# CederGroupHub/chgnet

Hardware: AMD Instinct MI355X
Metric: structures/s (energy+force+stress) on batched ~50-atom crystals (higher is better)
Workload: dtype f32; 1 GPU; 1024 x LiMnO2 5x1x1 (40 atoms, sigma=0.01 frac perturbation) per GPU, task efs; structures_per_gpu=1024, atoms=40960, directed_bonds=3535504, angles=4125764, bond_graph_nodes=213755, weights=random-init 0.3.0 architecture (tests/golden/weights_seed0.npz), parallelism=structures sharded over 1 GPU(s), RCCL all-gather of energies only, process_group_ranks=1, energies_in_all_gather=1024, comm=none (single rank)

## Files before the change

### chgnet_amd/csrc/engine_internal.h

```cpp
#pragma once

#include "chgnet_hip.h"

#include <hip/hip_runtime.h>

#include <algorithm>
#include <cmath>
#include <cstdint>
#include <cstdio>
#include <cstdlib>
#include <cstring>
#include <functional>
#include <map>
#include <mutex>
#include <string>
#include <unordered_map>
#include <vector>

#include "mfma_tile.h"
#include "mfma_split.h"
#include "kernels_conv.h"
#include "kernels_angle_w.h"
#include "kernels_angle_blk.h"
#include "kernels_embed.h"

using namespace chg;

constexpr int MAX_CONV = 8;
constexpr float F16_OPERAND_LIMIT = 65504.0f;
constexpr int FWD_WAVES = 8;

struct ACW { const float *w_cn, *w_bond, *b1, *q_bias, *q_shift; GatedW g; const float *w2c_t, *w2g_t, *w_out, *b_out, *w_out_t, *w_cn_t, *w_bond_t; };
struct BCW { const float *w_bij, *w_ang, *w_ctr, *b1; GatedW g; const float *w2c_t, *w2g_t, *w_out, *b_out, *w_out_t, *w_bij_t, *w_ang_t, *w_ctr_t; };
struct AUW { const float *w_bij, *w_ang, *w_ctr, *b1; GatedW g; const float *w_bij_t, *w_ang_t, *w_ctr_t; };

struct Weights {
  const float *atomref, *emb, *freq_ag, *freq_bg, *freq_ang, *w_bond_emb, *w_wag, *w_wbg, *w_ang_emb;
  ACW ac[MAX_CONV];
  BCW bc[MAX_CONV];
  AUW au[MAX_CONV];
  const float *site_w, *site_b, *ro_ln_g, *ro_ln_b, *mlp_w0, *mlp_b0, *mlp_w1, *mlp_b1, *mlp_w2, *mlp_b2, *mlp_w3, *mlp_b3;
  const float *mlp_w0_t, *mlp_w1_t, *mlp_w2_t;
};

struct ErrText {
  static std::unordered_map<const ErrText*, std::string>& texts() {
    thread_local std::unordered_map<const ErrText*, std::string> t;
    return t;
  }
  std::string& slot() const { return texts()[this]; }
  ErrText& operator=(const std::string& v) { slot() = v; return *this; }
  ErrText& operator=(const char* v) { slot() = v; return *this; }
  operator std::string() const { return slot(); }
  const char* c_str() const { return slot().c_str(); }
  ~ErrText() { texts().erase(this); }
};
inline std::string operator+(const char* a, const ErrText& b) { return std::string(a) + std::string(b); }
inline std::string operator+(const std::string& a, const ErrText& b) { return a + std::string(b); }
inline std::string operator+(const ErrText& a, const char* b) { return std::string(a) + b; }
inline std::string operator+(const ErrText& a, const std::string& b) { return std::string(a) + b; }

struct ProfEntry { std::string label; int64_t launches = 0; double ms = 0.0; };
struct PendingEvent { int entry; hipEvent_t start, stop; };

struct chg_engine {
  int device = 0;
  hipStream_t stream = nullptr;
  chg_model_desc desc{};
  float* d_weights = nullptr;
  Weights w{};
  float* d_images = nullptr;
  const float* p_elem = nullptr;
  const float* img_ac_fwd[2][MAX_CONV] = {};
  const float* img_ac_bwd_rm[MAX_CONV] = {};
  const float* img_angle[2][2 * MAX_CONV] = {};
  ErrText err;
  hipEvent_t t0 = nullptr, t1 = nullptr;
  bool profiling = false;
  std::vector<ProfEntry> prof;
  std::map<std::string, int> prof_index;
  std::vector<PendingEvent> pending;
  std::vector<hipEvent_t> event_pool;
  hipStream_t copy_stream = nullptr;
  std::mutex pool_mu;
  std::vector<std::pair<char*, size_t>> arena_pool;
  std::vector<std::pair<char*, size_t>> work_pool;
  std::vector<int> work_kind;
  bool use_graphs = true;
  bool force_wide = false;
  char* scratch = nullptr;
  size_t scratch_bytes = 0, scratch_wanted = 0;
  char* h_stage = nullptr;
  size_t h_stage_bytes = 0;
  char* h_out = nullptr;
  size_t h_out_bytes = 0;
  int num_cus = 256;
  bool spec_builds = true;
  int last_N = 0, last_Ed = 0, last_A = 0, last_Eb = 0;
  double last_r_atom = 0.0, last_r_bond = 0.0;
  long n_spec_builds = 0, n_spec_overflows = 0, n_cell_builds = 0, n_cell_fallbacks = 0;
  int graph_search = 0;
  int cell_min_atoms = 2048;
  size_t memory_limit = 0;
};

struct Train2;

struct chg_batch {
  int B = 0, N = 0, Ed = 0, Eu = 0, A = 0, Eb = 0, L = 0;
  char* arena = nullptr;
  size_t arena_bytes = 0;
  int *z, *atom_owner, *atom_off, *e_center, *e_nbr, *e_d2u, *e_owner, *e_rev, *p_center, *p_nbr, *u_u2d, *u_bnode, *bn_und, *a_ctr, *a_b1c, *a_b2c, *a_d1, *a_d2;
  float *frac, *lattice, *e_image;
  float* cart;
  f32x4 *ev, *eu;
  float *hb0, *wag, *wbgc;
  float* atom[MAX_CONV + 1];
  float* hbc[MAX_CONV + 1];
  float* ang[MAX_CONV];
  float* Pl[MAX_CONV];
  float* Ql[MAX_CONV];
  float* Rl[2 * MAX_CONV];
  float* Sl[2 * MAX_CONV];
  float* agg_l[MAX_CONV];
  float* aggB_l[MAX_CONV];
  float* GP_l[MAX_CONV];
  float* GR_l[2 * MAX_CONV];
  float* GS_l[2 * MAX_CONV];
  float* zsave_l[2 * MAX_CONV] = {};
  float *energy, *site_energy, *site_raw, *magmom, *crystal_fea, *force, *virial, *volume;
  float *Ga, *GA, *Gb, *Gwag, *Gwbgc, *Gang, *GQ, *Gagg, *Grk, *Gu;
  WinIndex win{};
  int *win_tmp = nullptr, *win_scan = nullptr;
  int win_grid = 64;
  bool win_built = false;
  bool canonical = false;
  bool win_index_ready = false;
  int win_team = 0;
  int blk_cap = 0;
  bool blk_ready = false;
  int *blk_a = nullptr, *blk_b1c = nullptr, *blk_b2c = nullptr, *blk_ctr = nullptr, *blk_desc = nullptr, *blk_tiles = nullptr;
  bool win_pending = false;
  bool zsave_now = false;
  int32_t route[6] = {}, graph_route[6] = {};
  size_t addr_span = 0;
  int p_table_done = -1;
  float *zero1, *zero1_end, *zero2, *zero2_end;
  float* zero2_keep_end = nullptr;
  uint32_t last_task = 0;
  bool seed1_adjoints = false;
  hipGraphExec_t graph_exec = nullptr;
  uint32_t graph_task = 0;
  int eager_calls = 0;
  std::map<std::string, std::pair<const float*, size_t>> named;
  std::map<std::string, std::pair<const int*, size_t>> named_i32;
  char* train_arena = nullptr;
  size_t train_bytes = 0;
  std::vector<int> h_atom_off;
  std::vector<double> h_volume;
  char* t2_arena = nullptr;
  size_t t2_bytes = 0;
  struct Train2* t2 = nullptr;
  float* t_mcot = nullptr;
  float h_g_b3 = 0.f;
  bool q_tables = false;
  bool wide_range = false;
  bool t_has_mcot = false;
  float *t_grad = nullptr, *t_cot = nullptr, *t_tmp = nullptr , *t_dumpG = nullptr, *t_dumpH = nullptr, *t_dumpZ = nullptr, *t_Xb = nullptr, *t_Xa = nullptr,
        *t_ro = nullptr;
};

#define HIP_TRY(eng, expr)                                                                          \
  do {                                                                                              \
    hipError_t _e = (expr);                                                                         \
    if (_e != hipSuccess) {                                                                         \
      (eng)->err = std::string(#expr) + ": " + hipGetErrorString(_e);                               \
      return CHG_EHIP;                                                                              \
    }                                                                                               \
  } while (0)

#define TRY(x)                   \
  do {                           \
    int _s = (x);                \
    if (_s != CHG_OK) return _s; \
  } while (0)

namespace chgh {

int prof_entry(chg_engine* eng, const char* label);
hipEvent_t get_event(chg_engine* eng);
int collect_profile(chg_engine* eng);

struct LaunchScope {
  chg_engine* eng;
  PendingEvent pe{};
  bool on;
  LaunchScope(chg_engine* e, const char* label) : eng(e), on(e->profiling) {
    if (on) {
      pe.entry = prof_entry(eng, label);
      pe.start = get_event(eng);
      pe.stop = get_event(eng);
      hipEventRecord(pe.start, eng->stream);
    }
  }
  ~LaunchScope() {
    if (on) {
      hipEventRecord(pe.stop, eng->stream);
      eng->pending.push_back(pe);
    }
  }
};


struct Carver {
  char* base;
  size_t pos = 0;
  template <class T>
  T* take(size_t n) {
    pos = (pos + 255) & ~size_t(255);
    T* p = base ? reinterpret_cast<T*>(base + pos) : nullptr;
    pos += std::max<size_t>(n, 1) * sizeof(T);
    return p;
  }
};

inline dim3 g1(int64_t n, int b = 256) { return dim3((unsigned)std::max<int64_t>(1, (n + b - 1) / b)); }
inline int wave_grid(chg_engine* eng, int64_t items) {
  return (int)std::max<int64_t>(1, std::min<int64_t>((items + 3) / 4, 16 * (int64_t)eng->num_cus));
}

template <class T>
int h2d(chg_engine* eng, T* dst, const T* src, size_t n, hipStream_t stream = nullptr) {
  if (n == 0) return CHG_OK;
  if (!src) { eng->err = "chg_batch_upload: null host array"; return CHG_EINVAL; }
  HIP_TRY(eng, hipMemcpyAsync(dst, src, n * sizeof(T), hipMemcpyHostToDevice, stream ? stream : eng->stream));
  return CHG_OK;
}
template <class T>
int d2h(chg_engine* eng, T* dst, const T* src, size_t n) {
  if (n == 0 || !dst) return CHG_OK;
  HIP_TRY(eng, hipMemcpyAsync(dst, src, n * sizeof(T), hipMemcpyDeviceToHost, eng->stream));
  return CHG_OK;
}

template <class K>
int set_lds(chg_engine* eng, K kernel, size_t bytes) {
  HIP_TRY(eng, hipFuncSetAttribute(reinterpret_cast<const void*>(kernel), hipFuncAttributeMaxDynamicSharedMemorySize, (int)bytes));
  return CHG_OK;
}

size_t layout_weights(const float* base, int L, Weights& w);
int grid_for(int rows, int max_blocks, int block_rows = BLOCK_ROWS);
int tile_grid(chg_engine* eng, int rows, int block_rows = BLOCK_ROWS);
int rows_gemm(chg_engine* eng, const char* label, int K, int NOUT, const float* X, int ldx, const int* in_idx, const float* Wt,
              const float* bias, const float* resid, int ldr, float* Y, int ldy, const int* out_idx, int rows, int accumulate);
int rows_gemm_out2(chg_engine* eng, const char* label, const float* X, const int* in_idx, const float* Wt, const float* Wt2,
                   const float* bias, float* Y, int ldy, int rows);
int rows_gemm_in2(chg_engine* eng, const char* label, const float* X, int ldx, const float* Wt, const float* Wt2, float* Y,
                  const int* out_idx, int rows, int accumulate);
int zero(chg_engine* eng, void* p, size_t bytes);
int build_images(chg_engine* eng);
int predict_set_lds(chg_engine* eng);
int atomconv_q_table(chg_engine* eng, chg_batch* b, int l);
AtomConvArgs atomconv_args(chg_engine* eng, chg_batch* b, int l);
AngleArgs angle_args(chg_batch* b, int slot, const float* ang, const float* w_ang, const GatedW& g, float* out);
int angle_table_grads(chg_engine* eng, chg_batch* b, int slot, const float* w_bij_t, const float* w_ctr_t);
BondEmbedTArgs bond_embed_args(chg_engine* eng, chg_batch* b);
AngleEmbedTArgs angle_embed_args(chg_engine* eng, chg_batch* b);
int run_predict(chg_engine* eng, chg_batch* b, uint32_t task);
void carve(chg_batch* b, char* base, size_t& total);
int prepare_windows(chg_engine* eng, chg_batch* b);
inline long team_min_angles() {
  static const long v = [] { const char* e = std::getenv("CHGNET_TEAM_MIN_ANGLES"); return e ? std::atol(e) : 131072L; }();
  return v;
}
inline long blk_max_angles() {
  static const long v = [] { const char* e = std::getenv("CHGNET_BLK_MAX_ANGLES"); return e ? std::atol(e) : (1L << 22); }();
  return v;
}
inline size_t blk_tile_bound(size_t A, size_t Eb, size_t N) { return (A + 14 * Eb + 9 * N) / 16 + 1; }
inline int upload_blk_cap(size_t N, size_t A, size_t Eb) {
  return (A > 0 && N + 1 <= 8192 && (long)A <= blk_max_angles()) ? (int)blk_tile_bound(A, Eb, N) : 0;
}
bool decide_windows(chg_engine* eng, chg_batch* b);
int ensure_windows(chg_engine* eng, chg_batch* b);
void register_names(chg_batch* b);

int train_set_lds(chg_engine* eng);
void free_train2(chg_batch* b);
void release_workspace(chg_engine* eng, char* p, size_t bytes, int kind);
int backward_impl(chg_engine* eng, chg_batch* b, const float* energy_cotangent, const float* magmom_cotangent, const float* force_cotangent,
                  const float* stress_cotangent, chg_comm* comm, float* grad_blob);

size_t scan_scratch_ints(int n);
int exclusive_scan_with(chg_engine* eng, int* scratch, const int* in, int* out, int n);
int acquire_arena(chg_engine* eng, chg_batch* b, size_t total);
int build_batch_on_device(chg_engine* eng, const chg_structs_host* h, double r_atom, double r_bond, double numerical_tol, chg_batch** out);

}

namespace chgh_wide {
int run_predict(chg_engine* eng, chg_batch* b, uint32_t task);
int predict_set_lds(chg_engine* eng);
int backward_compute(chg_engine* eng, chg_batch* b, const float* energy_cotangent, const float* magmom_cotangent, const float* force_cotangent,
                     const float* stress_cotangent);
int train_set_lds(chg_engine* eng);
int hvp_compute(chg_engine* eng, chg_batch* b, const float* direction, const float* strain, float* hvp, float* hvp_strain);
}

using namespace chgh;
```

### chgnet_amd/csrc/engine_predict.hip

```cpp
#include "engine_internal.h"

#include "kernels_geom.h"
#include "kernels_angle_fa.h"
#include "kernels_chain.h"

namespace chgh {


struct Cursor {
  const float* base;
  size_t pos = 0;
  const float* take(size_t n) {
    pos += (4 - pos % 4) % 4;
    const float* p = base + pos;
    pos += n;
    return p;
  }
};

void take_gated_tail(Cursor& c, GatedW& g, const float*& w2c_t, const float*& w2g_t) {
  g.w2c = c.take(D * D); g.b2c = c.take(D); g.w2g = c.take(D * D); g.b2g = c.take(D);
  w2c_t = c.take(D * D); w2g_t = c.take(D * D);
}
void take_ln(Cursor& c, GatedW& g) {
// ... 109 lines not shown
}

int rows_gemm(chg_engine* eng, const char* label, int K, int NOUT, const float* X, int ldx, const int* in_idx, const float* Wt,
              const float* bias, const float* resid, int ldr, float* Y, int ldy, const int* out_idx, int rows, int accumulate) {
  RowsGemm p{X, ldx, in_idx, Wt, bias, resid, ldr, Y, ldy, out_idx, rows, accumulate, nullptr, 0, 0, 0, 0};
  if (rows <= SMALL_GEMM_ROWS && K == 64 && (NOUT == 64 || NOUT == 128)) return launch_rows_gemm_cols<64, 1>(eng, label, p, NOUT, NOUT);
  if (rows <= SMALL_GEMM_ROWS && K == 128 && NOUT == 64) return launch_rows_gemm_cols<128, 1>(eng, label, p, NOUT, NOUT);
  if (K == 64 && NOUT == 64) return launch_rows_gemm<64, 64>(eng, label, p);
  if (K == 64 && NOUT == 128) return launch_rows_gemm<64, 128>(eng, label, p);
  if (K == 128 && NOUT == 64) return launch_rows_gemm<128, 64>(eng, label, p);
  eng->err = "rows_gemm: unsupported shape";
  return CHG_EINVAL;
}

int rows_gemm_out2(chg_engine* eng, const char* label, const float* X, const int* in_idx, const float* Wt, const float* Wt2,
                   const float* bias, float* Y, int ldy, int rows) {
  RowsGemm p{X, D, in_idx, Wt, bias, nullptr, 0, Y, ldy, nullptr, rows, 0, Wt2, 0, 2 * D, 0, 0};
  if (rows <= SMALL_GEMM_ROWS) return launch_rows_gemm_cols<64, 1>(eng, label, p, 4 * D, 2 * D);
  return launch_rows_gemm<64, 128, 2>(eng, label, p);
}
int rows_gemm_in2(chg_engine* eng, const char* label, const float* X, int ldx, const float* Wt, const float* Wt2, float* Y,
                  const int* out_idx, int rows, int accumulate) {
  RowsGemm p{X, ldx, nullptr, Wt, nullptr, nullptr, 0, Y, D, out_idx, rows, accumulate, Wt2, 2 * D, 0, 0, 0};
  if (rows <= SMALL_GEMM_ROWS) return launch_rows_gemm_cols<128, 2>(eng, label, p, D, D);
  return launch_rows_gemm<128, 64, 2>(eng, label, p);
}

struct MultiGemm {
  RowsGemmN g{};
  int max_rows = 0;
  void add(RowsGemm p, int n_out, int n_out_first) {
    p.col_blocks = n_out / SMALL_GEMM_COLS; p.blocks1 = n_out_first / SMALL_GEMM_COLS;
    g.p[g.n++] = p;
    max_rows = std::max(max_rows, p.rows);
  }
};
template <int K>
int launch_rows_gemm_multi(chg_engine* eng, const char* label, const MultiGemm& m) {
  int blocks = 0;
  for (int i = 0; i < m.g.n; ++i) blocks += m.g.p[i].col_blocks;
  LaunchScope ls(eng, label);
  hipLaunchKernelGGL((k_rows_gemm_multi<K, SMALL_GEMM_COLS>), dim3(grid_for(m.max_rows, 4 * eng->num_cus), blocks), dim3(BLOCK),
                     (rows_gemm_lds<K, SMALL_GEMM_COLS, (K == 128 ? 2 : 1)>()), eng->stream, m.g);
  HIP_TRY(eng, hipGetLastError());
  return CHG_OK;
}
static bool small_rows(int rows) { return rows > 0 && rows <= SMALL_GEMM_ROWS; }

int zero(chg_engine* eng, void* p, size_t bytes) {
  if (bytes == 0) return CHG_OK;
  LaunchScope ls(eng, "memset");
  HIP_TRY(eng, hipMemsetAsync(p, 0, bytes, eng->stream));
  return CHG_OK;
}





static bool addr32_mode(const chg_batch* b) {
  constexpr size_t HARD = (size_t)1 << 32;
  static const int forced = [] { const char* e = std::getenv("CHGNET_ADDR_MODE"); return e ? std::atoi(e) : 0; }();
  static const size_t limit = [] { const char* e = std::getenv("CHGNET_ADDR32_MAX_BYTES"); return e ? (size_t)std::strtoull(e, nullptr, 10) : HARD; }();
  if (b->addr_span == 0 || b->addr_span >= HARD || forced == 64) return false;
  return forced == 32 || b->addr_span < limit;
}

int build_images(chg_engine* eng) {
  const int L = eng->desc.n_conv;
  constexpr size_t AF = ac_fwd_image_floats(), AB = ac_bwd_rm_image_floats();
  constexpr size_t BF = AngleLds<true, false>::tiles, BB = AngleLds<true, true>::tiles, UF = AngleLds<false, false>::tiles,
                   UB = AngleLds<false, true>::tiles;
  static_assert(AF % 4 == 0 && AB % 4 == 0 && BF % 4 == 0 && BB % 4 == 0 && UF % 4 == 0 && UB % 4 == 0, "images are copied in 16-byte units");
  constexpr size_t PE = (size_t)94 * 4 * D;
  const size_t total = (size_t)L * (2 * AF + AB) + (size_t)(L - 1) * (BF + BB + UF + UB) + PE;
  if (!eng->d_images) {
    HIP_TRY(eng, hipMalloc(&eng->d_images, total * sizeof(float)));
    HIP_TRY(eng, hipMemsetAsync(eng->d_images, 0, total * sizeof(float), eng->stream));
  }
  float* at = eng->d_images;
  auto take = [&](size_t n) { float* p = at; at += n; return p; };
  for (int l = 0; l < L; ++l) {
    AtomConvArgs a{};
    a.gw = eng->w.ac[l].g; a.w_bond = eng->w.ac[l].w_bond;
    for (int qb = 0; qb < 2; ++qb) {
      a.q_bias = qb ? eng->w.ac[l].q_bias : nullptr;
      float* img = take(AF);
      eng->img_ac_fwd[qb][l] = img;
      hipLaunchKernelGGL(k_atomconv_image<>, dim3(1), dim3(BLOCK), 0, eng->stream, a, img);
    }
    float* img = take(AB);
    eng->img_ac_bwd_rm[l] = img;
    hipLaunchKernelGGL(k_atomconv_image_rm, dim3(1), dim3(BLOCK), 0, eng->stream, a, img);
  }
  for (int l = 0; l + 1 < L; ++l) {
    const BCW& bc = eng->w.bc[l];
    const AUW& au = eng->w.au[l];
    float* img;
    eng->img_angle[0][l] = img = take(BF);
    hipLaunchKernelGGL((k_angle_image<true, false>), dim3(1), dim3(BLOCK), 0, eng->stream, bc.w_ang, bc.g, img);
    eng->img_angle[1][l] = img = take(BB);
    hipLaunchKernelGGL((k_angle_image<true, true>), dim3(1), dim3(BLOCK), 0, eng->stream, bc.w_ang, bc.g, img);
    eng->img_angle[0][L + l] = img = take(UF);
    hipLaunchKernelGGL((k_angle_image<false, false>), dim3(1), dim3(BLOCK), 0, eng->stream, au.w_ang, au.g, img);
    eng->img_angle[1][L + l] = img = take(UB);
    hipLaunchKernelGGL((k_angle_image<false, true>), dim3(1), dim3(BLOCK), 0, eng->stream, au.w_ang, au.g, img);
  }
  {
    float* tab = take(PE);
    eng->p_elem = tab;
    const ACW& w0 = eng->w.ac[0];
    TRY(rows_gemm_out2(eng, "gemm_Pelem", eng->w.emb, nullptr, w0.w_cn, w0.w_cn + 2 * D * D, w0.b1, tab, 4 * D, 94));
  }
  HIP_TRY(eng, hipGetLastError());
  return CHG_OK;
}

static bool tiny_batch(const chg_batch* b) {
  static const bool on = [] { const char* e = std::getenv("CHGNET_TINY_FUSE"); return !e || std::atoi(e) != 0; }();
  return on && b->N <= SMALL_GEMM_ROWS && b->Ed <= (1 << 18) && b->A <= (1 << 19);
}

static RowsGemm atomconv_p_problem(chg_engine* eng, chg_batch* b, int l) {
  const ACW& w = eng->w.ac[l];
  return RowsGemm{b->atom[l], D, nullptr, w.w_cn, w.b1, nullptr, 0, b->Pl[l], 4 * D, nullptr, b->N, 0, w.w_cn + 2 * D * D, 0, 2 * D, 0, 0};
}

int atomconv_tables(chg_engine* eng, chg_batch* b, int l) {
  const ACW& w = eng->w.ac[l];
  if (b->p_table_done == l) return CHG_OK;
  return rows_gemm_out2(eng, "gemm_P", b->atom[l], nullptr, w.w_cn, w.w_cn + 2 * D * D, w.b1, b->Pl[l], 4 * D, b->N);
}

int atomconv_q_table(chg_engine* eng, chg_batch* b, int l) {
  const ACW& w = eng->w.ac[l];
  float* Q = b->Ql[l];
  if (b->Eu == 0) return CHG_OK;
  TRY(rows_gemm(eng, "gemm_Q", 64, 128, b->hb0, D, nullptr, w.w_bond, b->A > 0 ? w.q_bias : nullptr, nullptr, 0, Q, 2 * D, nullptr, b->Eu, 0));
  if (b->Eb > 0 && b->hbc[l] != b->hbc[0])
    TRY(rows_gemm(eng, "gemm_Qnode", 64, 128, b->hbc[l], D, nullptr, w.w_bond, nullptr, nullptr, 0, Q, 2 * D, b->bn_und, b->Eb, 0));
  return CHG_OK;
}

AtomConvArgs atomconv_args(chg_engine* eng, chg_batch* b, int l) {
  AtomConvArgs a{};
  a.P = b->Pl[l]; a.Q = b->Ql[l]; a.wag = b->wag;
  a.e_center = b->e_center; a.e_nbr = b->e_nbr; a.e_d2u = b->e_d2u; a.n_edges = b->Ed;
  a.gw = eng->w.ac[l].g;
  a.agg = b->agg_l[l]; a.GA = b->GA; a.GP = b->GP_l[l]; a.GQ = b->GQ; a.Gwag = b->Gwag;
  a.first_wag = l == b->L - 1;
  a.hb0 = b->hb0;
  a.hbc = (b->Eb > 0 && b->hbc[l] != b->hbc[0]) ? b->hbc[l] : nullptr;
  a.u_bnode = b->u_bnode;
  a.w_bond = eng->w.ac[l].w_bond;
  a.q_bias = b->A > 0 ? eng->w.ac[l].q_bias : nullptr;
  return a;
}

int atomconv_fwd_kernel(chg_engine* eng, chg_batch* b, int l, bool keep_q) {
  {
    LaunchScope ls(eng, "atomconv_fwd");
    const size_t lds = atomconv_lds<FWD_WAVES, false, true>();
    AtomConvArgs a = atomconv_args(eng, b, l);
    a.e_center = b->p_center;
    a.image = eng->img_ac_fwd[a.q_bias ? 1 : 0][l];
    a.e_nbr = b->p_nbr;
    a.Qout = keep_q ? b->Ql[l] : nullptr;
    if (addr32_mode(b)) hipLaunchKernelGGL((k_atomconv_fwd<FWD_WAVES, true>), dim3(tile_grid(eng, b->Ed, TILE_ROWS * FWD_WAVES)), dim3(64 * FWD_WAVES), lds, eng->stream, a);
    else hipLaunchKernelGGL((k_atomconv_fwd<FWD_WAVES>), dim3(tile_grid(eng, b->Ed, TILE_ROWS * FWD_WAVES)), dim3(64 * FWD_WAVES), lds, eng->stream, a);
    HIP_TRY(eng, hipGetLastError());
  }
  return CHG_OK;
}

int atomconv_fwd(chg_engine* eng, chg_batch* b, int l, bool keep_q) {
  const ACW& w = eng->w.ac[l];
  if (b->Ed > 0) {
    TRY(atomconv_tables(eng, b, l));
    TRY(atomconv_fwd_kernel(eng, b, l, keep_q));
  }
  return rows_gemm(eng, "gemm_out", 64, 64, b->agg_l[l], D, nullptr, w.w_out, w.b_out, b->atom[l], D, b->atom[l + 1], D, nullptr, b->N, 0);
}

constexpr size_t acb_fused_lds() { return sizeof(float) * ((size_t)ac_bwd_rm_image_floats() + WAVES * TILE_FLOATS); }

int atomconv_bwd_kernel(chg_engine* eng, chg_batch* b, int l) {
  {
    AtomConvArgs a = atomconv_args(eng, b, l);
    a.e_center = b->p_center;
    a.e_nbr = b->p_nbr;
    a.image = eng->img_ac_bwd_rm[l];
    a.Gb = b->Gb;
    a.gb_accumulate = l == b->L - 1 ? 0 : 1;
    LaunchScope ls(eng, "atomconv_bwd");
    if (addr32_mode(b)) hipLaunchKernelGGL((k_atomconv_bwd<false, true>), dim3(tile_grid(eng, b->Ed)), dim3(BLOCK), acb_fused_lds(), eng->stream, a);
    else hipLaunchKernelGGL(k_atomconv_bwd<false>, dim3(tile_grid(eng, b->Ed)), dim3(BLOCK), acb_fused_lds(), eng->stream, a);
    HIP_TRY(eng, hipGetLastError());
  }
  return CHG_OK;
}

int atomconv_bwd(chg_engine* eng, chg_batch* b, int l) {
  const ACW& w = eng->w.ac[l];
  if (b->Ed == 0) return CHG_OK;
  TRY(rows_gemm(eng, "gemm_Gagg", 64, 64, b->Ga, D, nullptr, w.w_out_t, nullptr, nullptr, 0, b->GA, D, nullptr, b->N, 0));
  TRY(atomconv_bwd_kernel(eng, b, l));
  if (l > 0) TRY(rows_gemm_in2(eng, "gemm_GP", b->GP_l[l], 4 * D, w.w_cn_t, w.w_cn_t + 2 * D * D, b->Ga, nullptr, b->N, 1));
  return CHG_OK;
}

int angle_tables(chg_engine* eng, chg_batch* b, int slot, const float* atom, const float* hbc, const float* w_bij, const float* w_ctr, const float* b1,
                 int p_layer = -1) {
  float *S = b->Sl[slot], *R = b->Rl[slot];
  if (small_rows(b->N) && small_rows(b->Eb)) {
    MultiGemm m;
    m.add(RowsGemm{atom, D, nullptr, w_ctr, b1, nullptr, 0, S, 2 * D, nullptr, b->N, 0, nullptr, 0, 0, 0, 0}, 2 * D, 2 * D);
    m.add(RowsGemm{hbc, D, nullptr, w_bij, nullptr, nullptr, 0, R, 4 * D, nullptr, b->Eb, 0, w_bij + 2 * D * D, 0, 2 * D, 0, 0}, 4 * D, 2 * D);
    if (p_layer >= 0 && b->Ed > 0) {
      m.add(atomconv_p_problem(eng, b, p_layer), 4 * D, 2 * D);
      b->p_table_done = p_layer;
    }
    return launch_rows_gemm_multi<64>(eng, m.g.n == 3 ? "gemm_SRP" : "gemm_SR", m);
  }
  TRY(rows_gemm(eng, "gemm_S", 64, 128, atom, D, nullptr, w_ctr, b1, nullptr, 0, S, 2 * D, nullptr, b->N, 0));
  return rows_gemm_out2(eng, "gemm_R", hbc, nullptr, w_bij, w_bij + 2 * D * D, nullptr, R, 4 * D, b->Eb);
}

AngleArgs angle_args(chg_batch* b, int slot, const float* ang, const float* w_ang, const GatedW& g, float* out) {
  AngleArgs a{};
  a.R = b->Rl[slot]; a.S = b->Sl[slot]; a.ang = ang; a.wbgc = b->wbgc;
  a.a_ctr = b->a_ctr; a.a_b1c = b->a_b1c; a.a_b2c = b->a_b2c; a.n_angles = b->A;
  a.w_ang = w_ang; a.gw = g; a.out = out; a.slot = slot;
  a.Gagg = b->Gagg; a.Gang = b->Gang; a.GR = b->GR_l[slot]; a.GS = b->GS_l[slot]; a.Gwbgc = b->Gwbgc;
  a.first_gang = slot == b->L - 2;
  a.skip_flag = b->win.flag;
  a.zsave = (b->zsave_now && (b->win_built || b->win_team > 0)) ? b->zsave_l[slot] : nullptr;
  return a;
}

static bool per_atom_forward() {
  static const bool on = [] { const char* e = std::getenv("CHGNET_PER_ATOM_FWD"); return !e || std::atoi(e) != 0; }();
  return on;
}

template <bool HIDDEN, bool BWD, int NW = WAVES>
int launch_angle(chg_engine* eng, const char* label, chg_batch* b, const AngleArgs& a) {
  LaunchScope ls(eng, label);
  AngleArgs plain = a;
  const bool index_from_builder = b->canonical && (b->win_index_ready || b->blk_ready);
  const bool a32 = addr32_mode(b);
  if (!BWD && !HIDDEN && b->win_built && per_atom_forward()) {
    AngleWArgs w{};
    w.a = a; w.w = b->win;
    w.a.image = eng->img_angle[0][a.slot];
    if (a32) hipLaunchKernelGGL(k_angleupd_fwd_a<true>, dim3(b->win_grid), dim3(BLOCK), angle_fa_lds(), eng->stream, w);
    else hipLaunchKernelGGL(k_angleupd_fwd_a<>, dim3(b->win_grid), dim3(BLOCK), angle_fa_lds(), eng->stream, w);
    HIP_TRY(eng, hipGetLastError());
    if (index_from_builder) return CHG_OK;
  } else if (BWD && b->blk_cap > 0) {
    AngleBlkArgs w{};
    w.a = a; w.a.image = eng->img_angle[1][a.slot];
    w.x.tiles = b->blk_tiles; w.x.a = b->blk_a; w.x.b1c = b->blk_b1c; w.x.b2c = b->blk_b2c; w.x.ctr = b->blk_ctr; w.x.desc = b->blk_desc;
    w.x.flag = b->canonical ? nullptr : b->win.flag;
    const int grid = std::max(1, std::min(eng->num_cus, (b->blk_cap + WAVES - 1) / WAVES));
    hipLaunchKernelGGL((k_angle_bwd_blk<HIDDEN>), dim3(grid), dim3(BLOCK), angle_blk_lds<HIDDEN>(), eng->stream, w);
    HIP_TRY(eng, hipGetLastError());
    if (index_from_builder) return CHG_OK;
  } else if (BWD && b->win_team > 0) {
    AngleBwdWArgs w = angle_bwd_w_args(a, b->win, b->N);
    w.image = eng->img_angle[1][a.slot];
    if (HIDDEN && w.zsave) hipLaunchKernelGGL((k_angle_bwd_w<HIDDEN, true, HIDDEN>), dim3(b->win_grid), dim3(BLOCK), angle_w_lds<HIDDEN>(), eng->stream, w);
    else
    hipLaunchKernelGGL((k_angle_bwd_w<HIDDEN, true>), dim3(b->win_grid), dim3(BLOCK), angle_w_lds<HIDDEN>(), eng->stream, w);
    HIP_TRY(eng, hipGetLastError());
    if (index_from_builder) return CHG_OK;
  } else if (BWD && b->win_built) {
    AngleBwdWArgs w = angle_bwd_w_args(a, b->win, b->N);
    w.image = eng->img_angle[1][a.slot];
    if (HIDDEN && w.zsave) {
      if (a32) hipLaunchKernelGGL((k_angle_bwd_w<HIDDEN, false, HIDDEN, true>), dim3(b->win_grid), dim3(BLOCK), angle_w_lds<HIDDEN>(), eng->stream, w);
      else hipLaunchKernelGGL((k_angle_bwd_w<HIDDEN, false, HIDDEN>), dim3(b->win_grid), dim3(BLOCK), angle_w_lds<HIDDEN>(), eng->stream, w);
    } else {
      if (a32) hipLaunchKernelGGL((k_angle_bwd_w<HIDDEN, false, false, true>), dim3(b->win_grid), dim3(BLOCK), angle_w_lds<HIDDEN>(), eng->stream, w);
      else hipLaunchKernelGGL((k_angle_bwd_w<HIDDEN>), dim3(b->win_grid), dim3(BLOCK), angle_w_lds<HIDDEN>(), eng->stream, w);
    }
    HIP_TRY(eng, hipGetLastError());
    if (index_from_builder) return CHG_OK;
  } else {
    plain.skip_flag = nullptr;
  }
  plain.image = eng->img_angle[BWD ? 1 : 0][a.slot];
  const size_t lds = angle_lds<HIDDEN, NW, BWD>();
  if (HIDDEN && !BWD && a32) hipLaunchKernelGGL((k_angle<HIDDEN, BWD, NW, false, HIDDEN && !BWD>), dim3(tile_grid(eng, b->A, TILE_ROWS * NW)), dim3(64 * NW), lds, eng->stream, plain);
  else hipLaunchKernelGGL((k_angle<HIDDEN, BWD, NW>), dim3(tile_grid(eng, b->A, TILE_ROWS * NW)), dim3(64 * NW), lds, eng->stream, plain);
  HIP_TRY(eng, hipGetLastError());
  return CHG_OK;
}

int bondconv_fwd(chg_engine* eng, chg_batch* b, int l) {
  const BCW& w = eng->w.bc[l];
  TRY(angle_tables(eng, b, l, b->atom[l + 1], b->hbc[l], w.w_bij, w.w_ctr, w.b1, l + 1));
  TRY((launch_angle<true, false>(eng, "bondconv_fwd", b, angle_args(b, l, b->ang[l], w.w_ang, w.g, b->aggB_l[l]))));
  return rows_gemm(eng, "gemm_out", 64, 64, b->aggB_l[l], D, nullptr, w.w_out, w.b_out, b->hbc[l], D, b->hbc[l + 1], D, nullptr, b->Eb, 0);
}

int angleupd_fwd(chg_engine* eng, chg_batch* b, int l) {
  const AUW& w = eng->w.au[l];
  TRY(angle_tables(eng, b, b->L + l, b->atom[l + 1], b->hbc[l + 1], w.w_bij, w.w_ctr, w.b1));
  return launch_angle<false, false, FWD_WAVES>(eng, "angleupd_fwd", b, angle_args(b, b->L + l, b->ang[l], w.w_ang, w.g, b->ang[l + 1]));
}

int angle_table_grads(chg_engine* eng, chg_batch* b, int slot, const float* w_bij_t, const float* w_ctr_t) {
  if (small_rows(b->N) && small_rows(b->Eb)) {
    MultiGemm m;
    m.add(RowsGemm{b->GR_l[slot], 4 * D, nullptr, w_bij_t, nullptr, nullptr, 0, b->Gb, D, b->bn_und, b->Eb, 1, w_bij_t + 2 * D * D, 2 * D, 0, 0, 0}, D, D);
    m.add(RowsGemm{b->GS_l[slot], 2 * D, nullptr, w_ctr_t, nullptr, nullptr, 0, b->Ga, D, nullptr, b->N, 1, nullptr, 0, 0, 0, 0}, D, D);
    return launch_rows_gemm_multi<128>(eng, "gemm_GRS", m);
  }
  TRY(rows_gemm_in2(eng, "gemm_GR", b->GR_l[slot], 4 * D, w_bij_t, w_bij_t + 2 * D * D, b->Gb, b->bn_und, b->Eb, 1));
  return rows_gemm(eng, "gemm_GS", 128, 64, b->GS_l[slot], 2 * D, nullptr, w_ctr_t, nullptr, nullptr, 0, b->Ga, D, nullptr, b->N, 1);
}

int bondconv_bwd(chg_engine* eng, chg_batch* b, int l) {
  const BCW& w = eng->w.bc[l];
  TRY(rows_gemm(eng, "gemm_Gagg", 64, 64, b->Gb, D, b->bn_und, w.w_out_t, nullptr, nullptr, 0, b->Gagg, D, nullptr, b->Eb, 0));
  TRY((launch_angle<true, true>(eng, "bondconv_bwd", b, angle_args(b, l, b->ang[l], w.w_ang, w.g, nullptr))));
  return angle_table_grads(eng, b, l, w.w_bij_t, w.w_ctr_t);
}

int angleupd_bwd(chg_engine* eng, chg_batch* b, int l) {
  const AUW& w = eng->w.au[l];
  TRY((launch_angle<false, true>(eng, "angleupd_bwd", b, angle_args(b, b->L + l, b->ang[l], w.w_ang, w.g, nullptr))));
  return angle_table_grads(eng, b, b->L + l, w.w_bij_t, w.w_ctr_t);
}

BondEmbedTArgs bond_embed_args(chg_engine* eng, chg_batch* b) {
  const Weights& w = eng->w;
  BondEmbedTArgs a{};
  a.ev = b->ev; a.u_u2d = b->u_u2d; a.u_bnode = b->u_bnode; a.n_und = b->Eu; a.bn_und = b->bn_und; a.n_nodes = b->Eb;
  a.freq_ag = w.freq_ag; a.freq_bg = w.freq_bg; a.w_emb = w.w_bond_emb; a.w_ag = w.w_wag; a.w_bg = w.w_wbg;
  a.rc_ag = eng->desc.atom_graph_cutoff; a.rc_bg = eng->desc.bond_graph_cutoff;
  const double p = eng->desc.cutoff_coeff;
  a.env = Envelope{(float)(-(p + 1) * (p + 2) / 2), (float)(p * (p + 2)), (float)(-p * (p + 1) / 2), eng->desc.cutoff_coeff};
  a.hb0 = b->hb0; a.wag = b->wag; a.wbgc = b->wbgc;
  a.hbc0 = b->Eb > 0 ? b->hbc[0] : nullptr;
  a.Gb = b->Gb; a.Gwag = b->Gwag; a.Gwbgc = b->Gwbgc; a.Grk = b->Grk;
  return a;
}

AngleEmbedTArgs angle_embed_args(chg_engine* eng, chg_batch* b) {
  AngleEmbedTArgs a{};
  a.eu = b->eu; a.a_d1 = b->a_d1; a.a_d2 = b->a_d2; a.n_angles = b->A;
  a.freq = eng->w.freq_ang; a.w_emb = eng->w.w_ang_emb;
  a.ang0 = b->ang[0]; a.Gang = b->Gang; a.Gu = b->Gu;
  return a;
}

struct ChainBuilder {
  ChainArgs a{};
  int max_rows = 0;
  ChainProb& add(int rows) {
    ChainProb& p = a.p[a.n++];
    p = ChainProb{};
    p.rows = rows;
    max_rows = std::max(max_rows, rows);
    return p;
  }
  static void term(ChainProb& p, const float* X, int ldx, const int* idx, const float* W, int K) { p.t[p.nterms++] = ChainTerm{X, idx, W, ldx, K}; }
  static void out(ChainProb& p, const float* W, const float* bias, float* Y, int ldy, int ncols) { p.o[p.nouts++] = ChainOut{W, bias, Y, ldy, ncols}; }
};
int launch_chain(chg_engine* eng, const char* label, ChainBuilder& cb) {
  int blocks = 0;
  for (int i = 0; i < cb.a.n; ++i) {
    ChainProb& p = cb.a.p[i];
    p.col_blocks = 0;
    for (int o = 0; o < p.nouts; ++o) p.col_blocks += p.o[o].ncols / D;
    p.serial_outs = (p.Y1 && p.Y1 == p.add) ? 1 : 0;
    if (p.serial_outs) {
      if (p.nouts > 1 || (p.nouts == 1 && p.o[0].ncols != D)) { eng->err = "launch_chain: an in-place problem takes one 64-column output"; return CHG_EINVAL; }
      p.col_blocks = 1;
    }
    p.col_blocks = std::max(1, p.col_blocks);
    blocks += p.col_blocks;
  }
  if (cb.max_rows <= 0 || blocks == 0) return CHG_OK;
  int row_blocks = 1;
  for (int i = 0; i < cb.a.n; ++i) {
    const int rows_per_wg = chain_tiles_per_wg(cb.a.p[i].nterms) * TILE_ROWS;
    row_blocks = std::max(row_blocks, (cb.a.p[i].rows + rows_per_wg - 1) / rows_per_wg);
  }
  LaunchScope ls(eng, label);
  hipLaunchKernelGGL(k_rows_chain, dim3(row_blocks, blocks), dim3(BLOCK), chain_lds(), eng->stream, cb.a);
  HIP_TRY(eng, hipGetLastError());
  return CHG_OK;
}

int forward_tiny(chg_engine* eng, chg_batch* b, bool want_grad, bool want_m) {
  const Weights& w = eng->w;
  const int L = b->L;
// ... 127 lines not shown
  if (b->A > 0 && !(tiny && b->Ed > 0)) {
    LaunchScope ls(eng, "angle_embed_fwd");
    hipLaunchKernelGGL((k_angle_embed_fwd_o4<0>), dim3(grid_for(b->A, EMBED_GRID_MULT * eng->num_cus)), dim3(BLOCK), angle_embed_lds(), st, angle_embed_args(eng, b));
  }
  if (!tiny) { LaunchScope ls(eng, "atom_embed");
    hipLaunchKernelGGL(k_atom_embed, g1((int64_t)b->N * (D / 4)), dim3(256), 0, st, b->z, w.emb, b->atom[0], b->N); }
  HIP_TRY(eng, hipGetLastError());

  if (!tiny) TRY(zero(eng, b->zero1, zero_bytes));
  static const bool chain_on = [] { const char* e = std::getenv("CHGNET_TINY_CHAIN"); return !e || std::atoi(e) != 0; }();
  const bool chained = tiny && chain_on && L >= 2 && b->Ed > 0 && b->A > 0 && b->Eb > 0 && b->p_table_done == 0;
  b->route[0] = tiny;
  b->route[1] = chained;
  b->route[2] = want_grad && b->zsave_l[0] && (b->win_built || b->win_team > 0);
  b->route[3] = b->win_built;
  b->route[4] = b->win_team > 0;
  b->route[5] = addr32_mode(b);
  if (chained) {
    TRY(forward_tiny(eng, b, want_grad, want_m));
  } else {
  for (int l = 0; l < L - 1; ++l) {
    TRY(atomconv_fwd(eng, b, l, want_grad));
    if (b->A > 0) {
      TRY(bondconv_fwd(eng, b, l));
      if (l < L - 2) TRY(angleupd_fwd(eng, b, l));
    }
  }
  if (want_m) {
    LaunchScope ls(eng, "magmom");
    hipLaunchKernelGGL(k_magmom, dim3(wave_grid(eng, b->N)), dim3(256), 0, st, b->atom[L - 1], w.site_w, w.site_b, b->magmom, b->N);
  }
  TRY(atomconv_fwd(eng, b, L - 1, want_grad));
  }

  {
    ReadoutArgs r{};
    r.atom = b->atom[L]; r.atom_owner = b->atom_owner; r.z = b->z; r.n_atoms = b->N;
    r.ln_g = w.ro_ln_g; r.ln_b = w.ro_ln_b; r.w0 = w.mlp_w0; r.b0 = w.mlp_b0; r.w1 = w.mlp_w1; r.b1 = w.mlp_b1;
    r.w2 = w.mlp_w2; r.b2 = w.mlp_b2; r.w3 = w.mlp_w3; r.b3 = w.mlp_b3; r.atomref = w.atomref;
    r.has_composition = eng->desc.has_composition; r.n_hidden = eng->desc.n_mlp_hidden;
    r.site_energy = b->site_energy; r.site_raw = b->site_raw; r.crystal_fea = b->crystal_fea;
    r.Ga = want_grad ? b->Ga : nullptr;
    const int tiles16 = (b->N + TILE_ROWS - 1) / TILE_ROWS;
    r.wpb = std::max(1, std::min(WAVES, (tiles16 + eng->num_cus - 1) / eng->num_cus));
    LaunchScope ls(eng, "readout");
    hipLaunchKernelGGL(k_readout<false>, dim3(grid_for(b->N, eng->num_cus, r.wpb * TILE_ROWS)), dim3(BLOCK), readout_lds(), st, r);
    HIP_TRY(eng, hipGetLastError());
  }

  if (want_grad) {
    if (chained) {
      TRY(reverse_tiny(eng, b));
    } else {
    TRY(atomconv_bwd(eng, b, L - 1));
    for (int l = L - 2; l >= 0; --l) {
      if (b->A > 0) {
        if (l < L - 2) TRY(angleupd_bwd(eng, b, l));
        TRY(bondconv_bwd(eng, b, l));
      }
      TRY(atomconv_bwd(eng, b, l));
    }
    }
    if (b->Ed > 0) {
      if (tiny) {
        EmbedAllArgs ea{bond_embed_args(eng, b), angle_embed_args(eng, b), grid_for(b->Eu, 2 * eng->num_cus),
                        b->Eb > 0 ? grid_for(b->Eb, 2 * eng->num_cus) : 0, b->A > 0 ? grid_for(b->A, EMBED_GRID_MULT * eng->num_cus) : 0};
        LaunchScope ls(eng, "embed_bwd");
        hipLaunchKernelGGL(k_embed_all<true>, dim3(ea.g_bond1 + ea.g_bond2 + ea.g_angle), dim3(BLOCK), bond_embed_lds(), st, ea);
      } else { LaunchScope ls(eng, "bond_embed_bwd");
        hipLaunchKernelGGL((k_bond_embed_t<true, false, 1>), dim3(grid_for(b->Eu, 2 * eng->num_cus)), dim3(BLOCK), bond_embed_lds(), st, bond_embed_args(eng, b));
        if (b->Eb > 0)
          hipLaunchKernelGGL((k_bond_embed_t<true, false, 2>), dim3(grid_for(b->Eb, 2 * eng->num_cus)), dim3(BLOCK), bond_embed_lds(), st, bond_embed_args(eng, b)); }
      if (b->A > 0 && !tiny) {
        LaunchScope ls(eng, "angle_embed_bwd");
        hipLaunchKernelGGL((k_angle_embed_t<true>), dim3(grid_for(b->A, EMBED_GRID_MULT * eng->num_cus)), dim3(BLOCK), angle_embed_lds(), st, angle_embed_args(eng, b));
      }
      ForceArgs f{};
      f.ev = b->ev; f.eu = b->eu; f.Gu = b->Gu; f.Grk = b->Grk;
      f.e_center = b->e_center; f.e_d2u = b->e_d2u; f.e_owner = b->e_owner; f.e_rev = b->e_rev; f.u_u2d = b->u_u2d;
      f.n_edges = b->Ed; f.force = b->force; f.virial = b->virial;
      LaunchScope ls(eng, "edge_force");
      hipLaunchKernelGGL(k_edge_force, g1(b->Ed, EF_EDGES_PER_BLOCK), dim3(256), 0, st, f);
    }
    HIP_TRY(eng, hipGetLastError());
  }
  {
    FinalizeArgs f{};
    f.lattice = b->lattice; f.atom_off = b->atom_off; f.n_struct = b->B;
    f.is_intensive = eng->desc.is_intensive; f.has_composition = eng->desc.has_composition; f.want_stress = want_s;
    f.site_raw = b->site_raw; f.z = b->z; f.atomref = eng->w.atomref; f.energy_out = b->energy; f.virial = b->virial; f.volume = b->volume;
    LaunchScope ls(eng, "finalize");
    hipLaunchKernelGGL(k_finalize, g1((int64_t)b->B * 64), dim3(256), 0, st, f);
    HIP_TRY(eng, hipGetLastError());
  }
  b->last_task = task;
  b->seed1_adjoints = want_grad;
  b->q_tables = want_grad;
  return CHG_OK;
}


void carve(chg_batch* b, char* base, size_t& total) {
  Carver c{base};
  const size_t B = b->B, N = b->N, Ed = b->Ed, Eu = b->Eu, A = b->A, Eb = b->Eb;
  const int L = b->L;
  b->z = c.take<int>(N); b->atom_owner = c.take<int>(N); b->atom_off = c.take<int>(B + 1);
  b->e_center = c.take<int>(Ed); b->e_nbr = c.take<int>(Ed); b->e_d2u = c.take<int>(Ed); b->e_owner = c.take<int>(Ed);
  b->e_rev = c.take<int>(Ed); b->p_center = c.take<int>(Ed); b->p_nbr = c.take<int>(Ed);
  b->u_u2d = c.take<int>(Eu); b->u_bnode = c.take<int>(Eu); b->bn_und = c.take<int>(Eb);
  b->a_ctr = c.take<int>(A); b->a_b1c = c.take<int>(A); b->a_b2c = c.take<int>(A); b->a_d1 = c.take<int>(A); b->a_d2 = c.take<int>(A);
  b->frac = c.take<float>(3 * N); b->lattice = c.take<float>(9 * B); b->e_image = c.take<float>(3 * Ed);
  b->cart = c.take<float>(3 * N); b->ev = c.take<f32x4>(Ed); b->eu = c.take<f32x4>(Ed);
  b->hb0 = c.take<float>(Eu * D); b->wag = c.take<float>(Eu * D); b->wbgc = c.take<float>(Eb * D);
  for (int l = 0; l <= L; ++l) b->atom[l] = c.take<float>(N * D);
  for (int l = 0; l < L; ++l) b->hbc[l] = (A > 0 || l == 0) ? c.take<float>(Eb * D) : nullptr;
  for (int l = 0; l < L - 1; ++l) b->ang[l] = c.take<float>(A * D);
  for (int l = 0; l < L; ++l) { b->Pl[l] = c.take<float>(N * 4 * D); b->Ql[l] = c.take<float>(Eu * 2 * D); }
  for (int t = 0; t < 2 * L; ++t) { b->Rl[t] = c.take<float>(Eb * 4 * D); b->Sl[t] = c.take<float>(N * 2 * D); }
  static const bool zsave_on = [] { const char* e = std::getenv("CHGNET_ZSAVE"); return !e || std::atoi(e) != 0; }();
  for (int t = 0; t < 2 * L; ++t)
    b->zsave_l[t] = (zsave_on && t < L - 1 && A > ((size_t)1 << 19)) ? c.take<float>((A + TILE_ROWS) * 2 * D) : nullptr;
  b->site_energy = c.take<float>(N); b->site_raw = c.take<float>(N); b->volume = c.take<float>(B);
  b->zero1 = c.take<float>(0);
  for (int l = 0; l < L; ++l) b->agg_l[l] = c.take<float>(N * D);
  for (int l = 0; l < L - 1; ++l) b->aggB_l[l] = c.take<float>(Eb * D);
  b->crystal_fea = c.take<float>(B * D);
  b->zero1_end = c.take<float>(0);
  b->zero2 = c.take<float>(0);
  b->force = c.take<float>(3 * N); b->virial = c.take<float>(9 * B); b->energy = c.take<float>(B); b->magmom = c.take<float>(N);
  b->zero2_keep_end = c.take<float>(0);
  b->Gwbgc = c.take<float>(Eb * D);
  b->Gu = c.take<float>(4 * Ed);
  b->Grk = c.take<float>(Eu);
  for (int l = 0; l < L; ++l) b->GP_l[l] = c.take<float>(N * 4 * D);
  for (int t = 0; t < 2 * L; ++t) {
    const bool used = (t < L - 1) || (t >= L && t < 2 * L - 2);
    b->GR_l[t] = used ? c.take<float>(Eb * 4 * D) : nullptr;
    b->GS_l[t] = used ? c.take<float>(N * 2 * D) : nullptr;
  }
  b->zero2_end = c.take<float>(0);
  b->Gb = c.take<float>(Eu * D); b->Gwag = c.take<float>(Eu * D); b->Gang = c.take<float>(A * D);
  b->Ga = c.take<float>(N * D); b->GA = c.take<float>(N * D);
  b->GQ = c.take<float>(Eu * 2 * D);
  b->Gagg = c.take<float>(Eb * D);
  {
    WinIndex& w = b->win;
    w.flag = c.take<int>(4); w.na = c.take<int>(N + 1); w.boff = c.take<int>(N + 1); w.aoff = c.take<int>(N + 1); w.toff = c.take<int>(N + 1); w.toff4 = c.take<int>(N + 1);
    w.head = c.take<int>(Ed); w.rank = c.take<int>(Ed); w.list = c.take<int>(A ? N * WIN_LIST : 0);
    w.q_a = c.take<int>(A); w.q_ctr = c.take<int>(A); w.q_b1c = c.take<int>(A); w.q_b2c = c.take<int>(A); w.q_ab1 = c.take<int>(A); w.q_ab2 = c.take<int>(A);
    w.abbond = c.take<int>(2 * Eb);
    w.rows = c.take<int4>(A); w.atoms = c.take<int4>(A ? N : 0);
    w.wave_head = c.take<int>(A ? WIN_MAX_GRID * WAVES : 0); w.next_atom = c.take<int>(A ? N : 0); w.xatom = c.take<int>(WIN_MAX_GRID / 8 + 1);
    b->win_tmp = c.take<int>(N + 1);
    b->win_scan = c.take<int>(scan_scratch_ints((int)N + 1));
  }
  {
    const size_t slots = (size_t)b->blk_cap * TILE_ROWS;
    b->blk_a = c.take<int>(slots); b->blk_b1c = c.take<int>(slots); b->blk_b2c = c.take<int>(slots); b->blk_ctr = c.take<int>(slots);
    b->blk_desc = c.take<int>(b->blk_cap);
    b->blk_tiles = c.take<int>(b->blk_cap ? 4 : 0);
  }
  if (A == 0) for (int l = 1; l < L; ++l) b->hbc[l] = b->hbc[0];
  {
    auto tab = [](size_t rows, size_t ld) { return rows * ld * sizeof(float); };
    size_t span = std::max({tab(N, 4 * D) , tab(Eu, 2 * D) , tab(Eb, 4 * D) , tab(A, D) ,
                            b->zsave_l[0] ? tab(A + TILE_ROWS, 2 * D) : 0 ,
                            A * sizeof(int4) });
    for (int l = 0; l < L; ++l) {
      if (!b->hbc[l]) continue;
      span = b->hbc[l] < b->hb0 ? ~size_t(0) : std::max(span, (size_t)(b->hbc[l] - b->hb0) * sizeof(float) + tab(Eb, D));
    }
    b->addr_span = span;
  }
  total = (c.pos + 255) & ~size_t(255);
}

int ensure_windows(chg_engine* eng, chg_batch* b) {
  if (!b->win_pending) return CHG_OK;
  b->win_pending = false;
  return prepare_windows(eng, b);
}

bool decide_windows(chg_engine* eng, chg_batch* b) {
  b->win_built = false;
  b->win_team = 0;
  b->win_grid = std::max(64, std::min(eng->num_cus / 64 * 64, WIN_MAX_GRID));
  const char* min_env = std::getenv("CHGNET_WIN_MIN_ATOMS_PER_WAVE");
  const long min_atoms = min_env ? std::atol(min_env) : WIN_MIN_ATOMS_PER_WAVE;
  if (b->A == 0) return false;
  if ((long)b->N < min_atoms * b->win_grid * WAVES) {
    const long team_min = team_min_angles();
    if (team_min < 0 || b->A < team_min || b->N + 1 > 8192) return false;
    const int cus = std::max(1, std::min(eng->num_cus, WIN_MAX_GRID));
    const long tiles_max = (long)b->A / TILE_ROWS + b->N;
    b->win_team = WAVES;
    b->win_grid = (int)std::max<long>(1, std::min<long>(cus, (tiles_max + WAVES - 1) / WAVES));
    return true;
  }
  if (scan_scratch_ints(b->N + 1) > (size_t)(1u << 17)) return false;
  b->win_built = true;
  return true;
}

int prepare_windows(chg_engine* eng, chg_batch* b) {
  hipStream_t st = eng->stream;
  WinIndex& w = b->win;
  if (b->blk_cap > 0) {
    b->win_built = false; b->win_team = 0;
    if (b->blk_ready) return CHG_OK;
    b->win_grid = std::max(1, std::min(eng->num_cus, WIN_MAX_GRID));
    hipLaunchKernelGGL(k_win_clear, g1(std::max(b->Ed, b->N + 1)), dim3(256), 0, st, w, b->N, b->Ed, b->win_grid);
    hipLaunchKernelGGL(k_win_heads, g1(b->A), dim3(256), 0, st, b->a_d1, b->a_ctr, b->A, b->Ed, b->N, w);
    hipLaunchKernelGGL(k_win_scan2, dim3(1), dim3(1024), 0, st, b->N, w);
    hipLaunchKernelGGL(k_win_ranks, g1(b->A), dim3(256), 0, st, b->a_d1, b->a_ctr, b->a_b1c, b->A, b->N, w);
    hipLaunchKernelGGL(k_win_rows, g1(b->A), dim3(256), 0, st, b->a_ctr, b->a_b1c, b->a_b2c, b->a_d1, b->a_d2, b->A, b->N, b->Ed, w);
    const size_t slots = (size_t)b->blk_cap * TILE_ROWS;
    HIP_TRY(eng, hipMemsetAsync(b->blk_a, 0xFF, sizeof(int) * slots, st));
    HIP_TRY(eng, hipMemsetAsync(b->blk_b1c, 0, (size_t)((char*)(b->blk_ctr + slots) - (char*)b->blk_b1c), st));
    hipLaunchKernelGGL(k_blk_from_q, g1(b->A), dim3(256), 0, st, b->A, b->N, w, b->blk_a, b->blk_b1c, b->blk_b2c, b->blk_ctr, b->blk_desc, b->blk_tiles, b->blk_cap);
    HIP_TRY(eng, hipGetLastError());
    b->blk_ready = true;
    return CHG_OK;
  }
  const bool ready = b->win_index_ready;
  if (!ready && !decide_windows(eng, b)) return CHG_OK;
  if (b->win_team > 0) {
    if (ready) return CHG_OK;
    hipLaunchKernelGGL(k_win_clear, g1(std::max(b->Ed, b->N + 1)), dim3(256), 0, st, w, b->N, b->Ed, b->win_grid);
    hipLaunchKernelGGL(k_win_heads, g1(b->A), dim3(256), 0, st, b->a_d1, b->a_ctr, b->A, b->Ed, b->N, w);
    hipLaunchKernelGGL(k_win_scan2, dim3(1), dim3(1024), 0, st, b->N, w);
    hipLaunchKernelGGL(k_win_ranks, g1(b->A), dim3(256), 0, st, b->a_d1, b->a_ctr, b->a_b1c, b->A, b->N, w);
    hipLaunchKernelGGL(k_win_rows, g1(b->A), dim3(256), 0, st, b->a_ctr, b->a_b1c, b->a_b2c, b->a_d1, b->a_d2, b->A, b->N, b->Ed, w);
    HIP_TRY(eng, hipGetLastError());
    return CHG_OK;
  }
  if (!ready) {
    HIP_TRY(eng, hipMemsetAsync(w.flag, 0, sizeof(int) * 4, st));
    HIP_TRY(eng, hipMemsetAsync(w.na, 0, sizeof(int) * ((size_t)b->N + 1), st));
    HIP_TRY(eng, hipMemsetAsync(w.head, 0xFF, sizeof(int) * (size_t)b->Ed, st));
    HIP_TRY(eng, hipMemsetAsync(w.rank, 0xFF, sizeof(int) * (size_t)b->Ed, st));
    hipLaunchKernelGGL(k_win_init, dim3(1), dim3(1), 0, st, w, b->win_grid);
    hipLaunchKernelGGL(k_win_heads, g1(b->A), dim3(256), 0, st, b->a_d1, b->a_ctr, b->A, b->Ed, b->N, w);
    TRY(exclusive_scan_with(eng, b->win_scan, w.na, w.boff, b->N + 1));
    hipLaunchKernelGGL(k_win_counts, g1((int64_t)b->N + 1), dim3(256), 0, st, b->N, w, b->win_tmp);
    TRY(exclusive_scan_with(eng, b->win_scan, b->win_tmp, w.aoff, b->N + 1));
    hipLaunchKernelGGL(k_win_ranks, g1(b->A), dim3(256), 0, st, b->a_d1, b->a_ctr, b->a_b1c, b->A, b->N, w);
    hipLaunchKernelGGL(k_win_rows, g1(b->A), dim3(256), 0, st, b->a_ctr, b->a_b1c, b->a_b2c, b->a_d1, b->a_d2, b->A, b->N, b->Ed, w);
  }
  hipLaunchKernelGGL(k_win_groups, g1(b->win_grid / 8 + 1), dim3(256), 0, st, b->N, b->A, b->win_grid / 8, w);
  hipLaunchKernelGGL(k_win_schedule, dim3(b->win_grid / 8), dim3(64), 0, st, b->win_grid, w);
  hipLaunchKernelGGL(k_win_atoms, g1(b->N), dim3(256), 0, st, b->N, w);
  if (ready) hipLaunchKernelGGL(k_win_pack, g1(b->A), dim3(256), 0, st, b->A, w);
  HIP_TRY(eng, hipGetLastError());
  return CHG_OK;
}

void register_names(chg_batch* b) {
  auto& m = b->named;
  m.clear();
  const size_t N = b->N, Ed = b->Ed, Eu = b->Eu, A = b->A, Eb = b->Eb, B = b->B;
  m["cart"] = {b->cart, 3 * N};
  m["ev"] = {reinterpret_cast<const float*>(b->ev), 4 * Ed};
  m["eu"] = {reinterpret_cast<const float*>(b->eu), 4 * Ed};
  m["hb0"] = {b->hb0, Eu * D}; m["wag"] = {b->wag, Eu * D}; m["wbgc"] = {b->wbgc, Eb * D};
  for (int l = 0; l <= b->L; ++l) m["atom" + std::to_string(l)] = {b->atom[l], N * D};
  for (int l = 0; l < b->L; ++l) m["hbc" + std::to_string(l)] = {b->hbc[l], Eb * D};
  for (int l = 0; l < b->L - 1; ++l) m["ang" + std::to_string(l)] = {b->ang[l], A * D};
  for (int l = 0; l < b->L; ++l) { m["P" + std::to_string(l)] = {b->Pl[l], N * 4 * D}; m["Q" + std::to_string(l)] = {b->Ql[l], Eu * 2 * D}; }
  m["agg"] = {b->agg_l[b->L - 1], N * D}; m["aggB"] = {b->aggB_l[0], Eb * D};
  m["Ga"] = {b->Ga, N * D}; m["GA"] = {b->GA, N * D}; m["Gb"] = {b->Gb, Eu * D}; m["Gwag"] = {b->Gwag, Eu * D};
  m["Gwbgc"] = {b->Gwbgc, Eb * D}; m["Gang"] = {b->Gang, A * D}; m["GP"] = {b->GP_l[0], N * 4 * D}; m["GQ"] = {b->GQ, Eu * 2 * D};
  m["GR"] = {b->GR_l[0], Eb * 4 * D}; m["GS"] = {b->GS_l[0], N * 2 * D}; m["Grk"] = {b->Grk, Eu}; m["Gu"] = {b->Gu, 4 * Ed};
  m["virial"] = {b->virial, 9 * B}; m["volume"] = {b->volume, B};
  m["frac"] = {b->frac, 3 * N}; m["lattice"] = {b->lattice, 9 * B}; m["e_image"] = {b->e_image, 3 * Ed};
  auto& mi = b->named_i32;
  mi.clear();
  mi["z"] = {b->z, N}; mi["atom_owner"] = {b->atom_owner, N}; mi["atom_off"] = {b->atom_off, B + 1};
  mi["e_center"] = {b->e_center, Ed}; mi["e_nbr"] = {b->e_nbr, Ed}; mi["e_d2u"] = {b->e_d2u, Ed}; mi["e_owner"] = {b->e_owner, Ed};
  mi["e_rev"] = {b->e_rev, Ed}; mi["p_center"] = {b->p_center, Ed}; mi["p_nbr"] = {b->p_nbr, Ed};
  mi["u_u2d"] = {b->u_u2d, Eu}; mi["u_bnode"] = {b->u_bnode, Eu}; mi["bn_und"] = {b->bn_und, Eb};
  mi["a_ctr"] = {b->a_ctr, A}; mi["a_b1c"] = {b->a_b1c, A}; mi["a_b2c"] = {b->a_b2c, A}; mi["a_d1"] = {b->a_d1, A}; mi["a_d2"] = {b->a_d2, A};
  mi["win_flag"] = {b->win.flag, 4}; mi["win_q_a"] = {b->win.q_a, A}; mi["win_q_ctr"] = {b->win.q_ctr, A}; mi["win_na"] = {b->win.na, N + 1};
  mi["win_aoff"] = {b->win.aoff, N + 1}; mi["win_q_ab1"] = {b->win.q_ab1, A}; mi["win_q_ab2"] = {b->win.q_ab2, A};
  mi["win_next_atom"] = {b->win.next_atom, A ? N : 0};
  mi["blk_tiles"] = {b->blk_tiles, b->blk_cap ? (size_t)1 : 0}; mi["blk_a"] = {b->blk_a, (size_t)b->blk_cap * TILE_ROWS};
  mi["blk_b1c"] = {b->blk_b1c, (size_t)b->blk_cap * TILE_ROWS}; mi["blk_b2c"] = {b->blk_b2c, (size_t)b->blk_cap * TILE_ROWS};
  mi["blk_ctr"] = {b->blk_ctr, (size_t)b->blk_cap * TILE_ROWS}; mi["blk_desc"] = {b->blk_desc, (size_t)b->blk_cap};
  mi["win_wave_head"] = {b->win.wave_head, A ? (size_t)WIN_MAX_GRID * WAVES : 0}; mi["win_xatom"] = {b->win.xatom, (size_t)WIN_MAX_GRID / 8 + 1};
}


int predict_set_lds(chg_engine* eng) {
  int s;
  if ((s = set_lds(eng, k_rows_gemm<64, 64>, rows_gemm_lds<64, 64>()))) return s;
  if ((s = set_lds(eng, k_rows_gemm<64, 128>, rows_gemm_lds<64, 128>()))) return s;
  if ((s = set_lds(eng, k_rows_gemm<128, 64>, rows_gemm_lds<128, 64>()))) return s;
  if ((s = set_lds(eng, k_rows_gemm<64, SMALL_GEMM_COLS, 1>, (rows_gemm_lds<64, SMALL_GEMM_COLS, 1>())))) return s;
  if ((s = set_lds(eng, k_rows_gemm_multi<64, SMALL_GEMM_COLS>, (rows_gemm_lds<64, SMALL_GEMM_COLS, 1>())))) return s;
  if ((s = set_lds(eng, k_rows_gemm_multi<128, SMALL_GEMM_COLS>, (rows_gemm_lds<128, SMALL_GEMM_COLS, 2>())))) return s;
  if ((s = set_lds(eng, k_rows_gemm<128, SMALL_GEMM_COLS, 1>, (rows_gemm_lds<128, SMALL_GEMM_COLS, 1>())))) return s;
  if ((s = set_lds(eng, k_rows_gemm<128, SMALL_GEMM_COLS, 2>, (rows_gemm_lds<128, SMALL_GEMM_COLS, 2>())))) return s;
  if ((s = set_lds(eng, (k_rows_gemm<64, 128, 2>), (rows_gemm_lds<64, 128, 2>())))) return s;
  if ((s = set_lds(eng, (k_rows_gemm<128, 64, 2>), (rows_gemm_lds<128, 64, 2>())))) return s;
  if ((s = set_lds(eng, k_atomconv_fwd<FWD_WAVES>, (atomconv_lds<FWD_WAVES, false, true>())))) return s;
  if ((s = set_lds(eng, k_atomconv_bwd<false>, acb_fused_lds()))) return s;
  if ((s = set_lds(eng, k_angleupd_fwd_a<>, angle_fa_lds()))) return s;
  if ((s = set_lds(eng, (k_atomconv_fwd<FWD_WAVES, true>), (atomconv_lds<FWD_WAVES, false, true>())))) return s;
  if ((s = set_lds(eng, (k_atomconv_bwd<false, true>), acb_fused_lds()))) return s;
  if ((s = set_lds(eng, k_angleupd_fwd_a<true>, angle_fa_lds()))) return s;
  if ((s = set_lds(eng, (k_angle_bwd_w<true, false, false, true>), angle_w_lds<true>()))) return s;
  if ((s = set_lds(eng, (k_angle_bwd_w<true, false, true, true>), angle_w_lds<true>()))) return s;
  if ((s = set_lds(eng, (k_angle_bwd_w<false, false, false, true>), angle_w_lds<false>()))) return s;
  if ((s = set_lds(eng, (k_angle<true, false, WAVES, false, true>), angle_lds<true>()))) return s;
  if ((s = set_lds(eng, k_angle_bwd_blk<true>, angle_blk_lds<true>()))) return s;
  if ((s = set_lds(eng, k_angle_bwd_blk<false>, angle_blk_lds<false>()))) return s;
  if ((s = set_lds(eng, k_angle_bwd_w<true>, angle_w_lds<true>()))) return s;
  if ((s = set_lds(eng, k_angle_bwd_w<false>, angle_w_lds<false>()))) return s;
  if ((s = set_lds(eng, (k_angle_bwd_w<true, true>), angle_w_lds<true>()))) return s;
  if ((s = set_lds(eng, (k_angle_bwd_w<true, false, true>), angle_w_lds<true>()))) return s;
  if ((s = set_lds(eng, (k_angle_bwd_w<true, true, true>), angle_w_lds<true>()))) return s;
  if ((s = set_lds(eng, (k_angle_bwd_w<false, true>), angle_w_lds<false>()))) return s;
  if ((s = set_lds(eng, k_angle<true, false>, angle_lds<true>()))) return s;
  if ((s = set_lds(eng, k_angle<true, true>, (angle_lds<true, WAVES, true>())))) return s;
  if ((s = set_lds(eng, k_angle<false, true>, (angle_lds<false, WAVES, true>())))) return s;
  if ((s = set_lds(eng, k_angle<false, false, FWD_WAVES>, (angle_lds<false, FWD_WAVES>())))) return s;
  if ((s = set_lds(eng, k_readout<false>, readout_lds()))) return s;
  if ((s = set_lds(eng, (k_bond_embed_t<false, false, 2>), bond_embed_lds()))) return s;
  if ((s = set_lds(eng, (k_bond_embed_t<true, false, 1>), bond_embed_lds()))) return s;
  if ((s = set_lds(eng, (k_bond_embed_t<true, false, 2>), bond_embed_lds()))) return s;
  if ((s = set_lds(eng, k_angle_embed_fwd_o4<0>, angle_embed_lds()))) return s;
  if ((s = set_lds(eng, k_bond_embed_fwd_o4<1>, bond_embed_lds()))) return s;
  if ((s = set_lds(eng, k_angle_embed_t<true>, angle_embed_lds()))) return s;
  if ((s = set_lds(eng, k_rows_chain, chain_lds()))) return s;
  if ((s = set_lds(eng, k_embed_all<false>, bond_embed_lds()))) return s;
  if ((s = set_lds(eng, k_embed_all<true>, bond_embed_lds()))) return s;
  return CHG_OK;
}


}
```

### chgnet_amd/csrc/kernels_angle_fa.h

```cpp
#pragma once

#include "kernels_angle_w.h"

namespace chg {

constexpr int FA_NSL = 15;
constexpr int FA_RS = 4 * D + 4;
constexpr size_t angle_fa_lds() { return sizeof(float) * (size_t)(AngleLds<false, false>::tiles + WAVES * FA_NSL * FA_RS); }

struct FaRows { f32x4 r[FA_NSL]; f32x4 s; };

template <bool A32 = false>
__device__ __forceinline__ void fa_request(FaRows& q, const AngleArgs& p, int c, int n, int bkv, int lane) {
#pragma unroll
  for (int k = 0; k < FA_NSL; ++k)
    if (k < n) q.r[k] = *grow<f32x4, A32>(p.R, (unsigned)__builtin_amdgcn_readlane(bkv, k), 4 * D, 4 * lane);
  q.s = lane < 32 ? *grow<f32x4, A32>(p.S, (unsigned)c, 2 * D, 4 * lane) : zero4();
}
__device__ __forceinline__ void fa_commit(const FaRows& q, float* tab, int n, int lane) {
#pragma unroll
  for (int k = 0; k < FA_NSL; ++k)
    if (k < n) *reinterpret_cast<f32x4*>(tab + k * FA_RS + 4 * lane) = q.r[k] + q.s;
}

template <bool A32 = false>
__global__ __launch_bounds__(BLOCK) CHG_TWO_WAVES void k_angleupd_fwd_a(AngleWArgs pw) {
  const AngleArgs& p = pw.a;
  const WinIndex& w = pw.w;
  if (w.flag[0] != 1) return;
  extern __shared__ __attribute__((aligned(16))) float smem[];
  using L = AngleLds<false, false>;
  const h16x8* Wang = reinterpret_cast<const h16x8*>(smem);
  const float* vecs = smem + L::vecs;
  const int tid = threadIdx.x, lane = tid & 63, j = lane & 15, g = lane >> 4;
  const int wave = __builtin_amdgcn_readfirstlane(tid >> 6);
  float* tab = smem + L::tiles + wave * (FA_NSL * FA_RS);

  int c_cur = w.wave_head[blockIdx.x * WAVES + wave];
  int n_raw = 0, ab_raw = 0, r_raw = 0, c_nx = -1;
  if (c_cur >= 0) { n_raw = w.na[c_cur]; ab_raw = w.boff[c_cur]; r_raw = w.aoff[c_cur]; c_nx = w.next_atom[c_cur]; }
  stage_image<L::tiles / 4, BLOCK>(smem, p.image, tid);
  __syncthreads();
  if (c_cur < 0) return;
  int n_nraw = 0, ab_nraw = 0, r_nraw = 0, c_n2 = -1;
  if (c_nx >= 0) { n_nraw = w.na[c_nx]; ab_nraw = w.boff[c_nx]; r_nraw = w.aoff[c_nx]; c_n2 = w.next_atom[c_nx]; }
  FaRows rows;
  int aA, q1A, q2A;
  V64 xn;
  {
    const int c = __builtin_amdgcn_readfirstlane(c_cur), n = __builtin_amdgcn_readfirstlane(n_raw);
    const int ab0 = __builtin_amdgcn_readfirstlane(ab_raw), r0 = __builtin_amdgcn_readfirstlane(r_raw);
    const int bkv = w.abbond[ab0 + min(lane, n - 1)];
    const int ra = min(r0 + j, r0 + n * (n - 1) - 1);
    aA = w.q_a[ra]; q1A = w.q_ab1[ra]; q2A = w.q_ab2[ra];
    fa_request<A32>(rows, p, c, min(n, FA_NSL), bkv, lane);
    read_dl_g<VT, A32>(p.ang, (unsigned)aA, D, g, xn.t);
  }
  V64 y_prev;
  CHG_EV(ft) y_prev.t[ft] = zero4();
  int a_prev = 0, nvalid_prev = 0;

  for (int c = __builtin_amdgcn_readfirstlane(c_cur); c >= 0; c = __builtin_amdgcn_readfirstlane(c_cur)) {
    const int n = __builtin_amdgcn_readfirstlane(n_raw), ab0 = __builtin_amdgcn_readfirstlane(ab_raw);
    const int r_begin = __builtin_amdgcn_readfirstlane(r_raw), r_end = r_begin + n * (n - 1);
    __builtin_amdgcn_wave_barrier();
    fa_commit(rows, tab, min(n, FA_NSL), lane);
    __builtin_amdgcn_wave_barrier();
    const int c_next = __builtin_amdgcn_readfirstlane(c_nx);
    int bkv_n = 0, aA_n = 0, q1A_n = 0, q2A_n = -1;
    int n1 = 0, ab1 = 0, rb1 = 0;
    int n_n2raw = 0, ab_n2raw = 0, r_n2raw = 0, c_n3 = -1;
    if (c_next >= 0) {
      n1 = __builtin_amdgcn_readfirstlane(n_nraw); ab1 = __builtin_amdgcn_readfirstlane(ab_nraw); rb1 = __builtin_amdgcn_readfirstlane(r_nraw);
      bkv_n = w.abbond[ab1 + min(lane, n1 - 1)];
      const int ra = min(rb1 + j, rb1 + n1 * (n1 - 1) - 1);
      aA_n = w.q_a[ra]; q1A_n = w.q_ab1[ra]; q2A_n = w.q_ab2[ra];
      if (c_n2 >= 0) { n_n2raw = w.na[c_n2]; ab_n2raw = w.boff[c_n2]; r_n2raw = w.aoff[c_n2]; c_n3 = w.next_atom[c_n2]; }
    }
    int a_t = aA, q1_t = q1A, q2_t = q2A;
    int a_n, q1_n, q2_n;
    {
      const int rr = min(r_begin + TILE_ROWS + j, r_end - 1);
      a_n = w.q_a[rr]; q1_n = w.q_ab1[rr]; q2_n = w.q_ab2[rr];
    }
    for (int row0 = r_begin; row0 < r_end; row0 += TILE_ROWS) {
      const int nvalid = min(TILE_ROWS, r_end - row0);
      asm volatile("" ::: "memory");
      const V64 x = xn;
      const int a = a_t, r1 = q1_t - ab0, r2 = q2_t < 0 ? -1 : q2_t - ab0;
      const bool last = row0 + TILE_ROWS >= r_end;
      const int a_ld = last ? (c_next >= 0 ? aA_n : a) : a_n;
      read_dl_g<VT, A32>(p.ang, (unsigned)a_ld, D, g, xn.t);
      const int rr2 = min(row0 + 2 * TILE_ROWS + j, r_end - 1);
      const int a_n2 = w.q_a[rr2], q1_n2 = w.q_ab1[rr2], q2_n2 = w.q_ab2[rr2];
      f32x4 z[2 * VT];
#pragma unroll
      for (int fo = 0; fo < 2 * VT; ++fo) z[fo] = zero4();
      gemm_split<VT, 2 * VT, false, true>(z, Wang, 2 * D, x.t, j, g);
      asm volatile("" ::: "memory");
      if (j < nvalid_prev) write_dl_g<VT, A32>(p.out, (unsigned)a_prev, D, g, y_prev.t);
      asm volatile("" ::: "memory");
      const bool in_lds = r1 < FA_NSL && r2 >= 0 && r2 < FA_NSL;
      if (__builtin_amdgcn_ballot_w64(!in_lds) == 0) {
        const float* t1 = tab + r1 * FA_RS + 4 * g;
        const float* t2 = tab + r2 * FA_RS + 2 * D + 4 * g;
#pragma unroll
        for (int fo = 0; fo < 2 * VT; ++fo)
          z[fo] += *reinterpret_cast<const f32x4*>(t1 + 16 * fo) + *reinterpret_cast<const f32x4*>(t2 + 16 * fo);
      } else {
        const int row = min(row0 + j, r_end - 1);
        const float* g1 = grow<float, A32>(p.R, (unsigned)w.q_b1c[row], 4 * D, 4 * g);
        const float* g2 = grow<float, A32>(p.R, (unsigned)w.q_b2c[row], 4 * D, 2 * D + 4 * g);
        const float* gs = grow<float, A32>(p.S, (unsigned)c, 2 * D, 4 * g);
#pragma unroll
        for (int fo = 0; fo < 2 * VT; ++fo)
          z[fo] += (*reinterpret_cast<const f32x4*>(g1 + 16 * fo) + *reinterpret_cast<const f32x4*>(gs + 16 * fo)) +
                   *reinterpret_cast<const f32x4*>(g2 + 16 * fo);
      }
      if (row0 == r_begin && c_next >= 0) fa_request<A32>(rows, p, c_next, min(n1, FA_NSL), bkv_n, lane);
      V64 zc{{z[0], z[1], z[2], z[3]}}, zg{{z[4], z[5], z[6], z[7]}};
      GatedState st;
      V64 y;
      gated_forward<false, false, false, 1>(zc, zg, nullptr, nullptr, vecs, j, g, st, y);
      CHG_EV(ft) y_prev.t[ft] = y.t[ft] + x.t[ft];
      a_prev = a; nvalid_prev = nvalid;
      a_t = a_n; q1_t = q1_n; q2_t = q2_n; a_n = a_n2; q1_n = q1_n2; q2_n = q2_n2;
    }
    c_cur = c_next; n_raw = n_nraw; ab_raw = ab_nraw; r_raw = r_nraw;
    c_nx = c_n2; n_nraw = n_n2raw; ab_nraw = ab_n2raw; r_nraw = r_n2raw; c_n2 = c_n3;
    aA = aA_n; q1A = q1A_n; q2A = q2A_n;
  }
  if (j < nvalid_prev) write_dl_g<VT, A32>(p.out, (unsigned)a_prev, D, g, y_prev.t);
}

}
```

### chgnet_amd/csrc/kernels_angle_w.h

```cpp
#pragma once

#include "blk_shape.h"
#include "kernels_conv.h"

namespace chg {

constexpr int TS64 = D + PAD;
constexpr int TILE64_FLOATS = TILE_ROWS * TS64;
constexpr int WIN_LIST = 32;
constexpr int WIN_MAX_GRID = 1024;
constexpr int WIN_MIN_ATOMS_PER_WAVE = 3;

struct WinIndex {
  int* flag;
  int *wave_head, *next_atom;
  int* xatom;
  int *na, *boff, *aoff;
  int* toff;
  int* toff4;
  int *head, *rank;
  int* list;
  int *q_a, *q_ctr, *q_b1c, *q_b2c, *q_ab1, *q_ab2;
  int* abbond;
  int4* rows;
// ... 46 lines not shown
  const int h = w.head[d1];
  if (h < 0 || a_ctr[h] != c) { w.flag[0] = 0; return; }
  const int n = w.na[c], q = a - h, r = w.rank[d1];
  const long row = (long)w.aoff[c] + (long)r * (n - 1) + q;
  if (q < 0 || q >= n - 1 || row < 0 || row >= A) { w.flag[0] = 0; return; }
  int r2 = -1;
  if (d2 >= 0 && d2 < Ed) {
    const int h2 = w.head[d2];
    if (h2 >= 0 && a_ctr[h2] == c) r2 = w.rank[d2];
  }
  w.q_a[row] = a; w.q_ctr[row] = c; w.q_b1c[row] = a_b1c[a]; w.q_b2c[row] = a_b2c[a];
  w.q_ab1[row] = w.boff[c] + r;
  w.q_ab2[row] = r2 >= 0 ? w.boff[c] + r2 : -1;
  w.rows[row] = make_int4(a, a_b1c[a], a_b2c[a], r2);
}

static __global__ void k_win_pack(int A, WinIndex w) {
  const int row = blockIdx.x * blockDim.x + threadIdx.x;
  if (row >= A) return;
  const int ab2 = w.q_ab2[row];
  w.rows[row] = make_int4(w.q_a[row], w.q_b1c[row], w.q_b2c[row], ab2 < 0 ? -1 : ab2 - w.boff[w.q_ctr[row]]);
}

static __global__ void k_win_clear(WinIndex w, int N, int Ed, int grid) {
  const int i = blockIdx.x * blockDim.x + threadIdx.x, stride = gridDim.x * blockDim.x;
  for (int k = i; k <= N; k += stride) w.na[k] = 0;
  for (int k = i; k < Ed; k += stride) { w.head[k] = -1; w.rank[k] = -1; }
  if (i == 0) { w.flag[0] = 1; w.flag[1] = 0; w.flag[2] = 0; w.flag[3] = grid; }
}

static __global__ __launch_bounds__(1024) void k_win_scan2(int N, WinIndex w) {
  __shared__ int tot_b[16], tot_a[16], tot_t[16], tot_4[16];
  const int tid = threadIdx.x, lane = tid & 63, wave = tid >> 6;
  const int n = N + 1, per = (n + 1023) / 1024;
  const int b = min(tid * per, n), e = min(b + per, n);
  int sb = 0, sa = 0, st = 0, s4 = 0;
  for (int k = b; k < e; ++k) {
    const int v = k < N ? w.na[k] : 0;
    int ps, qs;
    sb += v; sa += v * (v - 1); st += (v * (v - 1) + TILE_ROWS - 1) / TILE_ROWS; s4 += blk_shape_of(v, ps, qs);
  }
  int ib = sb, ia = sa, it = st, i4 = s4;
#pragma unroll
  for (int off = 1; off < 64; off <<= 1) {
    const int ub = __shfl_up(ib, off), ua = __shfl_up(ia, off), ut = __shfl_up(it, off), u4 = __shfl_up(i4, off);
    if (lane >= off) { ib += ub; ia += ua; it += ut; i4 += u4; }
  }
  if (lane == 63) { tot_b[wave] = ib; tot_a[wave] = ia; tot_t[wave] = it; tot_4[wave] = i4; }
  __syncthreads();
  int rb = ib - sb, ra = ia - sa, rt = it - st, r4 = i4 - s4;
  for (int q = 0; q < wave; ++q) { rb += tot_b[q]; ra += tot_a[q]; rt += tot_t[q]; r4 += tot_4[q]; }
  for (int k = b; k < e; ++k) {
    const int v = k < N ? w.na[k] : 0;
    int ps, qs;
    w.boff[k] = rb; w.aoff[k] = ra; w.toff[k] = rt; w.toff4[k] = r4;
    rb += v; ra += v * (v - 1); rt += (v * (v - 1) + TILE_ROWS - 1) / TILE_ROWS; r4 += blk_shape_of(v, ps, qs);
  }
}

constexpr int WIN_GROUP_WAVES = 64;

static __global__ void k_win_groups(int N, int A, int ngroups, WinIndex w) {
  const int i = blockIdx.x * blockDim.x + threadIdx.x;
  if (i > ngroups) return;
  if (i == ngroups) { w.xatom[i] = N; return; }
  const long target = (long)A * i / ngroups;
  int lo = 0, hi = N;
  while (lo < hi) {
    const int mid = (lo + hi) >> 1;
    if (w.aoff[mid + 1] > target) hi = mid; else lo = mid + 1;
  }
  w.xatom[i] = lo;
}

__device__ __forceinline__ unsigned wave_min_u32(unsigned v) {
#define CHG_DPP_MIN(ctrl) v = min(v, (unsigned)__builtin_amdgcn_update_dpp((int)v, (int)v, (ctrl), 0xF, 0xF, false))
  CHG_DPP_MIN(0xB1);
  CHG_DPP_MIN(0x4E);
  CHG_DPP_MIN(0x141);
  CHG_DPP_MIN(0x140);
#undef CHG_DPP_MIN
  const auto r = __builtin_amdgcn_permlane16_swap(v, v, false, false);
  const unsigned s = min((unsigned)r[0], (unsigned)r[1]);
  const auto q = __builtin_amdgcn_permlane32_swap(s, s, false, false);
  return min((unsigned)q[0], (unsigned)q[1]);
}

static __global__ __launch_bounds__(64) void k_win_schedule(int grid, WinIndex w) {
  const int gi = blockIdx.x, lane = threadIdx.x;
  const int spx = grid >> 6;
  const int x = gi / spx, sub = gi - x * spx;
  const int head_slot = ((((sub << 3) + (lane / WAVES)) << 3) + x) * WAVES + (lane % WAVES);
  if (w.flag[0] != 1) { w.wave_head[head_slot] = -1; return; }
  const int c0 = w.xatom[gi], c1 = w.xatom[gi + 1];
  unsigned load = 0;
  int head = -1, tail = -1;
  for (int cb = c0; cb < c1; cb += 64) {
    const int nn = w.na[min(cb + lane, c1 - 1)];
    const int m = min(64, c1 - cb);
    for (int i = 0; i < m; ++i) {
      const int n = __builtin_amdgcn_readlane(nn, i);
      if (n < 2) continue;
      const unsigned cost = (unsigned)(n * (n - 1) + TILE_ROWS - 1) / TILE_ROWS + 1;
      const unsigned best = wave_min_u32((load << 6) | (unsigned)lane);
      if ((int)(best & 63u) == lane) {
        const int c = cb + i;
        load += cost;
        w.next_atom[c] = -1;
        if (tail < 0) head = c; else w.next_atom[tail] = c;
        tail = c;
      }
    }
  }
  w.wave_head[head_slot] = head;
}

static __global__ void k_win_atoms(int N, WinIndex w) {
  const int c = blockIdx.x * blockDim.x + threadIdx.x;
  if (c < N) w.atoms[c] = make_int4(w.na[c], w.aoff[c], w.boff[c], w.next_atom[c]);
}

struct AngleWArgs {
  AngleArgs a;
  WinIndex w;
  int n_atoms;
};

struct AngleBwdWArgs {
  const int* flag;
  const float* image;
  const float* w_ang;
  GatedW gw;
  const float *R, *S, *ang, *wbgc, *Gagg, *zsave;
  float *Gang, *GR, *GS, *Gwbgc;
  int first_gang;
  const int4* rows;
  const int* abbond;
  const int4* atoms;
  const int* wave_head;
  const int *toff, *na, *aoff, *boff, *q_a, *q_b1c, *q_b2c, *q_ab2;
  int n_atoms;
};
inline AngleBwdWArgs angle_bwd_w_args(const AngleArgs& a, const WinIndex& w, int n_atoms) {
  AngleBwdWArgs k{};
  k.flag = w.flag; k.image = a.image; k.w_ang = a.w_ang; k.gw = a.gw;
  k.R = a.R; k.S = a.S; k.ang = a.ang; k.wbgc = a.wbgc; k.Gagg = a.Gagg; k.zsave = a.zsave;
  k.Gang = a.Gang; k.GR = a.GR; k.GS = a.GS; k.Gwbgc = a.Gwbgc; k.first_gang = a.first_gang;
  k.rows = w.rows; k.abbond = w.abbond; k.atoms = w.atoms; k.wave_head = w.wave_head;
  k.toff = w.toff; k.na = w.na; k.aoff = w.aoff; k.boff = w.boff; k.q_a = w.q_a; k.q_b1c = w.q_b1c; k.q_b2c = w.q_b2c; k.q_ab2 = w.q_ab2;
  k.n_atoms = n_atoms;
  return k;
}

template <class T, bool A32 = false>
__device__ __forceinline__ T index_load(const T* __restrict__ base, int i) {
  if constexpr (A32) return *reinterpret_cast<const T*>(reinterpret_cast<const char*>(base) + (unsigned)i * (unsigned)sizeof(T));
  else return base[i];
}
__device__ __forceinline__ int4 index_load_uniform(const int4* base, int i) {
#if defined(__HIP_DEVICE_COMPILE__)
  typedef const int __attribute__((address_space(4))) * ConstInt;
  ConstInt q = (ConstInt)(unsigned long long)(base + i);
  return make_int4(q[0], q[1], q[2], q[3]);
#else
  return base[i];
#endif
}

template <bool HIDDEN> constexpr int win_ns() { return HIDDEN ? 13 : 14; }
template <bool HIDDEN> constexpr int win_pst() { return 2 * D; }
constexpr size_t WIN_RM_ANG = rm_image_bytes(2 * D, D), WIN_RM_W2 = rm_image_bytes(D, D);

template <bool HIDDEN>
constexpr size_t angle_w_lds() {
  const size_t weights = HIDDEN ? WIN_RM_ANG + 2 * WIN_RM_W2 : 16 * (size_t)(2 * IMG128);
  return weights + sizeof(float) * (VEC_SLOTS * D + WAVES * TILE64_FLOATS + WAVES * win_ns<HIDDEN>() * win_pst<HIDDEN>());
}

struct Gather64 { f32x4 a[TILE_ROWS / 4], b[TILE_ROWS / 4], c[TILE_ROWS / 4]; };
template <bool A32 = false>
__device__ __forceinline__ void gather64_issue(Gather64& gr, const float* __restrict__ t0, int i0, int ld0, const float* __restrict__ t1, int i1,
                                               int ld1, const float* __restrict__ t2, int i2, int ld2, int lane, int c0 = 0, int c1 = 0, int c2 = 0) {
  const int sub = lane >> 4, t = lane & 15;
  int r0[TILE_ROWS / 4], r1[TILE_ROWS / 4], r2[TILE_ROWS / 4];
#pragma unroll
  for (int it = 0; it < TILE_ROWS / 4; ++it) {
    const int rr = 4 * it + sub;
    r0[it] = __shfl(i0, rr); r1[it] = __shfl(i1, rr); r2[it] = __shfl(i2, rr);
  }
#pragma unroll
  for (int it = 0; it < TILE_ROWS / 4; ++it) {
    gr.a[it] = *grow<f32x4, A32>(t0, (unsigned)r0[it], ld0, c0 + 4 * t);
    gr.b[it] = *grow<f32x4, A32>(t1, (unsigned)r1[it], ld1, c1 + 4 * t);
    gr.c[it] = *grow<f32x4, A32>(t2, (unsigned)r2[it], ld2, c2 + 4 * t);
  }
}
__device__ __forceinline__ void gather64_commit(const Gather64& gr, float* tile, int lane) {
  const int sub = lane >> 4, t = lane & 15;
#pragma unroll
  for (int it = 0; it < TILE_ROWS / 4; ++it)
    *reinterpret_cast<f32x4*>(tile + (4 * it + sub) * TS64 + 4 * t) = (gr.a[it] + gr.b[it]) + gr.c[it];
}

struct Cols64 { float v[TILE_ROWS]; };
__device__ __forceinline__ void to_columns(const V64& x, float* T, float* Trow, int g, int lane, Cols64& c) {
  write_dl<VT>(Trow, g, x.t);
  __builtin_amdgcn_wave_barrier();
#pragma unroll
  for (int rr = 0; rr < TILE_ROWS; ++rr) c.v[rr] = T[rr * TS64 + lane];
  __builtin_amdgcn_wave_barrier();
}
__device__ __forceinline__ int fresh_uniform(int v) {
  asm volatile("" : "+s"(v));
  return v;
}
__device__ __forceinline__ unsigned run_starts64(int key, int cur, int nvalid, int lane) {
  const int prev = __builtin_amdgcn_update_dpp(cur, key, 0x111 , 0xF, 0xF, false);
  return (unsigned)__builtin_amdgcn_ballot_w64(key != prev && lane < nvalid);
}
template <int NB, bool A32 = false>
__device__ __forceinline__ void run_sum64(const Cols64 (&c)[NB], int nvalid, int key, unsigned starts, float (&sum)[NB], int& cur, float* __restrict__ dst,
                                          int ld, int col) {
  nvalid = fresh_uniform(nvalid);
#pragma unroll
  for (int rr = 0; rr < TILE_ROWS; ++rr) {
    if (rr < nvalid) {
      if (starts & (1u << rr)) {
        if (cur >= 0) {
          float* d = grow<float, A32>(dst, (unsigned)cur, ld, col);
#pragma unroll
          for (int q = 0; q < NB; ++q) atomicAdd(d + q * D, sum[q]);
        }
#pragma unroll
        for (int q = 0; q < NB; ++q) sum[q] = 0.f;
        cur = __builtin_amdgcn_readlane(key, rr);
      }
#pragma unroll
      for (int q = 0; q < NB; ++q) sum[q] += c[q].v[rr];
    }
  }
}
template <int NB, bool A32 = false>
__device__ __forceinline__ void run_flush64(float (&sum)[NB], int& cur, float* __restrict__ dst, int ld, int col) {
  if (cur >= 0) {
    float* d = grow<float, A32>(dst, (unsigned)cur, ld, col);
#pragma unroll
    for (int q = 0; q < NB; ++q) atomicAdd(d + q * D, sum[q]);
  }
#pragma unroll
  for (int q = 0; q < NB; ++q) sum[q] = 0.f;
  cur = -1;
}
template <bool A32 = false>
__device__ __forceinline__ void row_add64(const Cols64& c, int nvalid, float* __restrict__ base, int row, int ld, int lane) {
  nvalid = fresh_uniform(nvalid);
#pragma unroll
  for (int rr = 0; rr < TILE_ROWS; ++rr)
    if (rr < nvalid) atomicAdd(grow<float, A32>(base, (unsigned)__builtin_amdgcn_readlane(row, rr), ld, lane), c.v[rr]);
}
template <int NB>
__device__ __forceinline__ void private_add(const Cols64 (&c)[NB], int nvalid, int slot, float* pacc, float* dump, int lane) {
  nvalid = fresh_uniform(nvalid);
#pragma unroll
  for (int rr = 0; rr < TILE_ROWS; rr += 2) {
    const int sa = __builtin_amdgcn_readlane(slot, rr), sb = __builtin_amdgcn_readlane(slot, rr + 1);
    float* pa = (rr < nvalid && sa >= 0) ? pacc + sa * (NB * D) : dump;
    float* pb = (rr + 1 < nvalid && sb >= 0) ? pacc + sb * (NB * D) : dump + NB * D;
    float a[NB], b[NB];
#pragma unroll
    for (int q = 0; q < NB; ++q) { a[q] = pa[q * D + lane]; b[q] = pb[q * D + lane]; }
#pragma unroll
    for (int q = 0; q < NB; ++q) { pa[q * D + lane] = a[q] + c[q].v[rr]; pb[q * D + lane] = b[q] + c[q].v[rr + 1]; }
  }
}

template <bool HIDDEN, bool TEAM = false, bool ZS = false, bool A32 = false>
__global__ __launch_bounds__(BLOCK) CHG_TWO_WAVES void k_angle_bwd_w(AngleBwdWArgs pw) {
  const AngleBwdWArgs& p = pw;
  const AngleBwdWArgs& w = pw;
  if (w.flag[0] != 1) return;
  extern __shared__ __attribute__((aligned(16))) float smem[];
  constexpr int NS = win_ns<HIDDEN>(), PST = win_pst<HIDDEN>();
  constexpr int MODE = HIDDEN ? 2 : 1;
  float* Wang = smem;
  float* WangT = HIDDEN ? Wang : Wang + 4 * IMG128;
  float* W2c = HIDDEN ? Wang + WIN_RM_ANG / 4 : WangT + 4 * IMG128;
  float* W2g = W2c + (HIDDEN ? WIN_RM_W2 / 4 : 0);
  float* vecs = W2g + (HIDDEN ? WIN_RM_W2 / 4 : 0);
  float* tiles = vecs + VEC_SLOTS * D;
  float* paccs = tiles + WAVES * TILE64_FLOATS;
  const int tid = threadIdx.x, lane = tid & 63, j = lane & 15, g = lane >> 4;
  const int wave = __builtin_amdgcn_readfirstlane(tid >> 6);
  static_assert((size_t)AngleLds<HIDDEN, true>::tiles * sizeof(float) == (HIDDEN ? WIN_RM_ANG + 2 * WIN_RM_W2 : 16 * (size_t)(2 * IMG128)) + sizeof(float) * VEC_SLOTS * D,
                "the per-atom adjoints share the weight image of k_angle<HIDDEN, true>");
  if (p.image) {
    stage_image<AngleLds<HIDDEN, true>::tiles / 4, BLOCK>(smem, p.image, tid);
  } else if (HIDDEN) {
    stage_rm(reinterpret_cast<_Float16*>(Wang), p.w_ang, 2 * D, D, tid, BLOCK);
    stage_rm(reinterpret_cast<_Float16*>(W2c), p.gw.w2c, D, D, tid, BLOCK);
    stage_rm(reinterpret_cast<_Float16*>(W2g), p.gw.w2g, D, D, tid, BLOCK);
    stage_gated_vecs(vecs, p.gw, HIDDEN, tid);
  } else {
    stage_split<false>(reinterpret_cast<h16x8*>(Wang), p.w_ang, 2 * D, D, tid, BLOCK);
    stage_split<true>(reinterpret_cast<h16x8*>(WangT), p.w_ang, 2 * D, D, tid, BLOCK);
    stage_gated_vecs(vecs, p.gw, HIDDEN, tid);
  }
  for (int q = tid; q < WAVES * NS * PST; q += BLOCK) paccs[q] = 0.f;
  __syncthreads();
  float* T = tiles + wave * TILE64_FLOATS;
  float* Trow = T + j * TS64;
  float* pacc = paccs + wave * NS * PST;
// ... 219 lines not shown
```

### chgnet_amd/csrc/kernels_conv.h

```cpp
#pragma once

#include "mfma_tile.h"
#include "mfma_split.h"

namespace chg {

constexpr int TS = 2 * D + PAD;
constexpr int WS = D + PAD;
constexpr int TILE_FLOATS = TILE_ROWS * TS;
constexpr int VEC_SLOTS = 6;
constexpr int IMG64 = 1024, IMG128 = 2048;
constexpr int angle_split(bool hidden, bool bwd) { return (hidden && bwd) ? 2 : 1; }

struct GatedW {
  const float *w2c, *b2c, *w2g, *b2g, *ln1_g, *ln1_b, *ln2_g, *ln2_b;
};

__device__ __forceinline__ void stage_gated_vecs(float* vecs, const GatedW& gw, bool hidden, int tid) {
  if (hidden) {
    stage_vector(vecs + 0 * D, gw.b2c, D, tid);
    stage_vector(vecs + 1 * D, gw.b2g, D, tid);
  }
  stage_vector(vecs + 2 * D, gw.ln1_g, D, tid);
  stage_vector(vecs + 3 * D, gw.ln1_b, D, tid);
// ... 225 lines not shown
      rows_of(tb, nvalid_n, in_n, out_n);
      if (nvalid_n > 0) issue_x(in_n, vn);
    }
    for (int tile = tb; tile < te; ++tile) {
      const int nvalid = nvalid_n, out_row = out_n;
      if (nvalid <= 0) break;
#pragma unroll
      for (int it = 0; it < NV; ++it) *reinterpret_cast<f32x4*>(T + (RPS * it + subx) * XS + 4 * tx) = vn[it];
      __builtin_amdgcn_wave_barrier();
      f32x4 x[KT];
      read_dl<KT>(T + j * XS, g, x);
      __builtin_amdgcn_wave_barrier();
      if (tile + 1 < te) {
        rows_of(tile + 1, nvalid_n, in_n, out_n);
        if (nvalid_n > 0) issue_x(in_n, vn);
      } else {
        nvalid_n = 0;
      }
      const bool rmw = p.accumulate || p.resid;
      f32x4 old[NO];
      if (rmw) {
#pragma unroll
        for (int it = 0; it < NO; ++it) {
          const int r = __shfl(out_row, RPO * it + suby);
          old[it] = zero4();
          if (RPO * it + suby < nvalid) {
            if (p.accumulate) old[it] = *reinterpret_cast<const f32x4*>(p.Y + (size_t)r * p.ldy + 4 * ty);
            if (p.resid) old[it] += *reinterpret_cast<const f32x4*>(p.resid + (size_t)r * p.ldr + 4 * ty);
          }
        }
      }
      f32x4 acc[NFT];
      read_dl<NFT>(bias, g, acc);
      contract(acc, 0, x);
      write_dl<NFT>(T + j * XS, g, acc);
      __builtin_amdgcn_wave_barrier();
      f32x4 ov[NO];
      int orow[NO];
#pragma unroll
      for (int it = 0; it < NO; ++it) {
        const int rr = RPO * it + suby;
        orow[it] = __shfl(out_row, rr);
        ov[it] = *reinterpret_cast<const f32x4*>(T + rr * XS + 4 * ty);
        if (rmw) ov[it] += old[it];
      }
#pragma unroll
      for (int it = 0; it < NO; ++it) asm volatile("" : "+v"(ov[it]));
#pragma unroll
      for (int it = 0; it < NO; ++it)
        if (RPO * it + suby < nvalid) *reinterpret_cast<f32x4*>(p.Y + (size_t)orow[it] * p.ldy + 4 * ty) = ov[it];
      __builtin_amdgcn_wave_barrier();
    }
    return;
  }
  for (int tile = tb; tile < te; ++tile) {
    const int row0 = tile * BLOCK_ROWS + wave * TILE_ROWS;
    const int nvalid = min(TILE_ROWS, p.rows - row0);
    if (nvalid <= 0) continue;
    const int rr_ = row0 + (j < nvalid ? j : 0);
    const int in_row = p.in_idx ? p.in_idx[rr_] : rr_;
    const int out_row = p.out_idx ? p.out_idx[rr_] : rr_;
    constexpr int LPR = K / 4, RPS = 64 / LPR;
    constexpr int LPO = NOUT / 4, RPO = 64 / LPO;
    f32x4 x[KT];
    f32x4 acc[NFT];
    read_dl<NFT>(bias, g, acc);
#pragma unroll
    for (int part = 0; part < PARTS; ++part) {
      if (part == 0 || split_in) {
        const float* X = p.X + (part ? p.x2_off : 0);
        const int sub = lane / LPR, t = lane % LPR;
        f32x4 v[TILE_ROWS / RPS];
#pragma unroll
        for (int it = 0; it < TILE_ROWS / RPS; ++it) {
          const int r = __shfl(in_row, RPS * it + sub);
          v[it] = *reinterpret_cast<const f32x4*>(X + (size_t)r * p.ldx + 4 * t);
        }
#pragma unroll
        for (int it = 0; it < TILE_ROWS / RPS; ++it) *reinterpret_cast<f32x4*>(T + (RPS * it + sub) * XS + 4 * t) = v[it];
        __builtin_amdgcn_wave_barrier();
        read_dl<KT>(T + j * XS, g, x);
        __builtin_amdgcn_wave_barrier();
      }
      if (part == 1 && !split_in) {
#pragma unroll
        for (int ft = 0; ft < NFT; ++ft) acc[ft] = zero4();
      }
      contract(acc, part, x);
      if (part == PARTS - 1 || !split_in) {
        write_dl<NFT>(T + j * XS, g, acc);
        __builtin_amdgcn_wave_barrier();
        float* Y = p.Y + (part ? p.y2_off : 0);
        const int sub = lane / LPO, t = lane % LPO;
        constexpr int NOI = TILE_ROWS / RPO;
        f32x4 ov[NOI];
        f32x4* odst[NOI];
#pragma unroll
        for (int it = 0; it < NOI; ++it) {
          const int r = __shfl(out_row, RPO * it + sub);
          odst[it] = reinterpret_cast<f32x4*>(Y + (size_t)r * p.ldy + 4 * t);
          ov[it] = zero4();
          if (p.resid) ov[it] = *reinterpret_cast<const f32x4*>(p.resid + (size_t)r * p.ldr + 4 * t);
          if (p.accumulate) ov[it] += *odst[it];
        }
#pragma unroll
        for (int it = 0; it < NOI; ++it) {
          ov[it] += *reinterpret_cast<const f32x4*>(T + (RPO * it + sub) * XS + 4 * t);
          asm volatile("" : "+v"(ov[it]));
        }
#pragma unroll
        for (int it = 0; it < NOI; ++it)
          if (RPO * it + sub < nvalid) *odst[it] = ov[it];
        __builtin_amdgcn_wave_barrier();
      }
    }
  }
}

template <int K, int NOUT, int PARTS = 1>
__global__ __launch_bounds__(BLOCK) CHG_TWO_WAVES void k_rows_gemm(RowsGemm p) {
  rows_gemm_body<K, NOUT, PARTS>(p, blockIdx.y);
}

struct RowsGemmN { RowsGemm p[3]; int n; };
template <int K, int NOUT>
__global__ __launch_bounds__(BLOCK) CHG_TWO_WAVES void k_rows_gemm_multi(RowsGemmN g) {
  int y = blockIdx.y;
#pragma unroll
  for (int i = 0; i < 3; ++i) {
    if (i >= g.n) return;
    if (y < g.p[i].col_blocks) {
      if (K == 128 && g.p[i].x2_off > 0) rows_gemm_body<K, NOUT, (K == 128 ? 2 : 1)>(g.p[i], y);
      else rows_gemm_body<K, NOUT, 1>(g.p[i], y);
      return;
    }
    y -= g.p[i].col_blocks;
  }
}

template <int K, int NOUT, int PARTS = 1>
constexpr size_t rows_gemm_lds() {
  return sizeof(float) * (PARTS * NOUT * (K + PAD) + NOUT + WAVES * TILE_ROWS * ((K > NOUT ? K : NOUT) + PAD));
}

struct AtomConvArgs {
  const float* P;
  const float* Q;
  const float* wag;
  const int *e_center, *e_nbr, *e_d2u;
  int n_edges;
  GatedW gw;
  const float *hb0, *hbc;
  const int* u_bnode;
  const float *w_bond, *q_bias;
  float* Qout;
  const float* image;
  float* agg;
  const float* GA;
  float* GP;
  float* GQ;
  float* Gwag;
  int first_wag;
  float* Gb;
  int gb_accumulate;
  float* dumpG;
  float* dumpH;
  float* g_ln;
};

constexpr int AC_VEC_SLOTS = VEC_SLOTS + 2;
template <int NW = WAVES, bool BWD = false, bool FUSEQ = false>
constexpr size_t atomconv_lds() {
  if (FUSEQ) return 16 * (size_t)(2 * IMG64 + IMG128) + sizeof(float) * (AC_VEC_SLOTS * D + NW * TILE_FLOATS);
  return 16 * (size_t)(BWD ? 4 : 2) * IMG64 + sizeof(float) * (VEC_SLOTS * D + NW * TILE_FLOATS);
}

constexpr int ac_fwd_image_floats() { return 4 * (2 * IMG64 + IMG128) + AC_VEC_SLOTS * D; }
__device__ __forceinline__ void atomconv_fwd_stage(float* base, const AtomConvArgs& p, int tid, int nthreads) {
  h16x8* I2c = reinterpret_cast<h16x8*>(base);
  h16x8* I2g = I2c + IMG64;
  h16x8* Ib = I2g + IMG64;
  float* vecs = reinterpret_cast<float*>(Ib + IMG128);
  stage_split<false>(I2c, p.gw.w2c, D, D, tid, nthreads);
  stage_split<false>(I2g, p.gw.w2g, D, D, tid, nthreads);
  stage_split<false>(Ib, p.w_bond, 2 * D, D, tid, nthreads);
  stage_gated_vecs(vecs, p.gw, true, tid);
  for (int q = tid; q < 2 * D; q += nthreads) vecs[VEC_SLOTS * D + q] = p.q_bias ? p.q_bias[q] : 0.f;
}
__device__ __forceinline__ void atomconv_bwd_stage(float* base, const AtomConvArgs& p, int tid, int nthreads) {
  h16x8* I2c = reinterpret_cast<h16x8*>(base);
  h16x8* I2g = I2c + IMG64;
  h16x8* I2cT = I2g + IMG64;
  h16x8* I2gT = I2cT + IMG64;
  float* vecs = reinterpret_cast<float*>(I2gT + IMG64);
  stage_split<false>(I2c, p.gw.w2c, D, D, tid, nthreads);
  stage_split<false>(I2g, p.gw.w2g, D, D, tid, nthreads);
  stage_split<true>(I2cT, p.gw.w2c, D, D, tid, nthreads);
  stage_split<true>(I2gT, p.gw.w2g, D, D, tid, nthreads);
  stage_gated_vecs(vecs, p.gw, true, tid);
}
constexpr int AC_RM_IMG = (int)(rm_image_bytes(D, D) / 4);
constexpr int ac_bwd_rm_image_floats() { return 2 * AC_RM_IMG + VEC_SLOTS * D + 4 * IMG128; }
__device__ __forceinline__ void atomconv_bwd_stage_rm(float* base, const AtomConvArgs& p, int tid, int nthreads) {
  stage_rm(reinterpret_cast<_Float16*>(base), p.gw.w2c, D, D, tid, nthreads);
  stage_rm(reinterpret_cast<_Float16*>(base + AC_RM_IMG), p.gw.w2g, D, D, tid, nthreads);
  float* vecs = base + 2 * AC_RM_IMG;
  stage_gated_vecs(vecs, p.gw, true, tid);
  stage_split<true>(reinterpret_cast<h16x8*>(vecs + VEC_SLOTS * D), p.w_bond, 2 * D, D, tid, nthreads);
}
template <int UNUSED = 0>
__global__ __launch_bounds__(BLOCK) void k_atomconv_image(AtomConvArgs p, float* out) { atomconv_fwd_stage(out, p, threadIdx.x, BLOCK); }
static __global__ __launch_bounds__(BLOCK) void k_atomconv_image_rm(AtomConvArgs p, float* out) { atomconv_bwd_stage_rm(out, p, threadIdx.x, BLOCK); }

__device__ __forceinline__ int bond_node(const AtomConvArgs& p, int k) { return p.hbc ? p.u_bnode[k] : -1; }
template <bool A32 = false>
__device__ __forceinline__ long bond_row_offset(const AtomConvArgs& p, int k, int bn) {
  if constexpr (A32) return (long)(bn >= 0 ? (unsigned)(p.hbc - p.hb0) + (unsigned)bn * D : (unsigned)k * D);
  else return bn >= 0 ? (p.hbc - p.hb0) + (long)bn * D : (long)k * D;
}

template <int NW, bool A32 = false>
__global__ __launch_bounds__(64 * NW) CHG_TWO_WAVES void k_atomconv_fwd(AtomConvArgs p) {
  extern __shared__ __attribute__((aligned(16))) float smem[];
  h16x8* I2c = reinterpret_cast<h16x8*>(smem);
  h16x8* I2g = I2c + IMG64;
  h16x8* Ib = I2g + IMG64;
  float* vecs = reinterpret_cast<float*>(Ib + IMG128);
  float* tiles = vecs + AC_VEC_SLOTS * D;
  const float* W2c = reinterpret_cast<const float*>(I2c);
  const float* W2g = reinterpret_cast<const float*>(I2g);
  const int tid = threadIdx.x, wave = tid >> 6, lane = tid & 63, j = lane & 15, g = lane >> 4;
  float* T = tiles + wave * TILE_FLOATS;
  float* Trow = T + j * TS;
  const int ntiles = (p.n_edges + TILE_ROWS - 1) / TILE_ROWS;
  const TileSeq ts = wave_tile_seq<true>(ntiles, NW, wave);
  const int tstride = TILE_ROWS;
  auto row_of = [&](int v) { return max(0, min(ts.at(v) * tstride + j, p.n_edges - 1)); };
  GatherPH gr;
  V64 wv_nx;
  int c_nx = 0, n_nx = 0, c_n2 = 0, n_n2 = 0;
  int bn_nx = -1, bn_n2 = -1;
  if (ts.count > 0) {
    const int r0 = row_of(0);
    c_nx = p.e_center[r0]; n_nx = p.e_nbr[r0];
    bn_nx = bond_node(p, r0 >> 1);
    gather_issue_ph<A32>(gr, p.P, c_nx, p.P + 2 * D, n_nx, 4 * D, 4 * D, p.hb0, bond_row_offset<A32>(p, r0 >> 1, bn_nx), lane);
    read_dl_g<VT, A32>(p.wag, (unsigned)(r0 >> 1), D, g, wv_nx.t);
    const int r1 = row_of(1);
    c_n2 = p.e_center[r1]; n_n2 = p.e_nbr[r1];
    bn_n2 = bond_node(p, r1 >> 1);
  }
  stage_image<ac_fwd_image_floats() / 4, 64 * NW>(smem, p.image, tid);
  __syncthreads();
  for (int v = 0; v < ts.count; ++v) {
    const int row0 = ts.at(v) * tstride;
    const int nvalid = min(TILE_ROWS, p.n_edges - row0);
    const int c = c_nx;
    const bool node = bn_nx >= 0;
    const V64 wv = wv_nx;
    gather_commit_h(gr, T, TS, lane);
    __builtin_amdgcn_wave_barrier();
    V64 x;
    read_dl<VT>(Trow, g, x.t);
    __builtin_amdgcn_wave_barrier();
    gather_commit_p(gr, T, TS, lane);
    __builtin_amdgcn_wave_barrier();
    c_nx = c_n2; n_nx = n_n2; bn_nx = bn_n2;
    if (v + 1 < ts.count) {
      const int r1 = row_of(v + 1);
      gather_issue_ph<A32>(gr, p.P, c_nx, p.P + 2 * D, n_nx, 4 * D, 4 * D, p.hb0, bond_row_offset<A32>(p, r1 >> 1, bn_nx), lane);
      read_dl_g<VT, A32>(p.wag, (unsigned)(r1 >> 1), D, g, wv_nx.t);
      const int r2 = row_of(v + 2);
      c_n2 = p.e_center[r2]; n_n2 = p.e_nbr[r2];
      bn_n2 = bond_node(p, r2 >> 1);
    }
    f32x4 z[2 * VT];
    if (!node) {
      read_dl<2 * VT>(vecs + VEC_SLOTS * D, g, z);
    } else {
#pragma unroll
      for (int ft = 0; ft < 2 * VT; ++ft) z[ft] = f32x4{0.f, 0.f, 0.f, 0.f};
    }
    gemm_split<VT, 2 * VT, false, true>(z, Ib, 2 * D, x.t, j, g);
    if (p.Qout && !(j & 1) && j < nvalid) {
      write_dl_g<2 * VT, A32>(p.Qout, (unsigned)((row0 + j) >> 1), 2 * D, g, z);
    }
    {
      f32x4 ps[2 * VT];
      read_dl<2 * VT>(Trow, g, ps);
#pragma unroll
      for (int ft = 0; ft < 2 * VT; ++ft) z[ft] += ps[ft];
    }
    V64 zc{{z[0], z[1], z[2], z[3]}}, zg{{z[4], z[5], z[6], z[7]}};
    GatedState s;
    V64 y;
    gated_forward<true, false, false, 1, true>(zc, zg, W2c, W2g, vecs, j, g, s, y);
    gather_take(gr);
    asm volatile("" : "+v"(c_n2), "+v"(n_n2), "+v"(bn_n2));
    CHG_EV(ft) asm volatile("" : "+v"(wv_nx.t[ft]));
    __builtin_amdgcn_wave_barrier();
    V64 m;
    CHG_EV(ft) m.t[ft] = y.t[ft] * wv.t[ft];
    write_dl<VT>(Trow, g, m.t);
    __builtin_amdgcn_wave_barrier();
    {
      float acc1 = 0.f, acc2 = 0.f;
      int cur1 = __builtin_amdgcn_readlane(c, 0), cur2 = __builtin_amdgcn_readlane(c, 1);
#pragma unroll
      for (int b = 0; b < TILE_ROWS / 2; ++b) {
        if (2 * b < nvalid) {
          const int c1 = __builtin_amdgcn_readlane(c, 2 * b), c2 = __builtin_amdgcn_readlane(c, 2 * b + 1);
          if (c1 != cur1) {
            tile_atomic_add(grow<float, A32>(p.agg, (unsigned)cur1, D, lane), acc1);
            acc1 = 0.f;
            cur1 = c1;
          }
          if (c2 != cur2) {
            tile_atomic_add(grow<float, A32>(p.agg, (unsigned)cur2, D, lane), acc2);
            acc2 = 0.f;
            cur2 = c2;
          }
          acc1 += T[(2 * b) * TS + lane];
          acc2 += T[(2 * b + 1) * TS + lane];
        }
      }
      tile_atomic_add(grow<float, A32>(p.agg, (unsigned)cur1, D, lane), acc1);
      tile_atomic_add(grow<float, A32>(p.agg, (unsigned)cur2, D, lane), acc2);
    }
    __builtin_amdgcn_wave_barrier();
  }
}

template <bool STORE_GQ = true, bool A32 = false>
__device__ __forceinline__ void acbwd_scatter(const float* T, int c, int nvalid, int k0, const AtomConvArgs& p, int lane) {
  float a1[4] = {0.f, 0.f, 0.f, 0.f}, a2[4] = {0.f, 0.f, 0.f, 0.f};
  int cur1 = __builtin_amdgcn_readlane(c, 0), cur2 = __builtin_amdgcn_readlane(c, 1);
#pragma unroll
  for (int b = 0; b < TILE_ROWS / 2; ++b) {
    if (2 * b < nvalid) {
      const float e0 = T[(2 * b) * TS + lane], e1 = T[(2 * b) * TS + 64 + lane];
      const float o0 = T[(2 * b + 1) * TS + lane], o1 = T[(2 * b + 1) * TS + 64 + lane];
      if (STORE_GQ) {
        float* q = p.GQ + (size_t)(k0 + b) * 2 * D + lane;
        q[0] = e0 + o0;
        q[64] = e1 + o1;
      }
      const int c1 = __builtin_amdgcn_readlane(c, 2 * b), c2 = __builtin_amdgcn_readlane(c, 2 * b + 1);
      if (c1 != cur1) {
        float* d = grow<float, A32>(p.GP, (unsigned)cur1, 4 * D, lane);
        tile_atomic_add(d, a1[0]); tile_atomic_add(d + 64, a1[1]); tile_atomic_add(d + 128, a1[2]); tile_atomic_add(d + 192, a1[3]);
        a1[0] = a1[1] = a1[2] = a1[3] = 0.f;
        cur1 = c1;
      }
      if (c2 != cur2) {
        float* d = grow<float, A32>(p.GP, (unsigned)cur2, 4 * D, lane);
        tile_atomic_add(d, a2[0]); tile_atomic_add(d + 64, a2[1]); tile_atomic_add(d + 128, a2[2]); tile_atomic_add(d + 192, a2[3]);
        a2[0] = a2[1] = a2[2] = a2[3] = 0.f;
        cur2 = c2;
      }
      a1[0] += e0; a1[1] += e1; a1[2] += o0; a1[3] += o1;
      a2[0] += o0; a2[1] += o1; a2[2] += e0; a2[3] += e1;
    }
  }
  float* d1 = grow<float, A32>(p.GP, (unsigned)cur1, 4 * D, lane);
  tile_atomic_add(d1, a1[0]); tile_atomic_add(d1 + 64, a1[1]); tile_atomic_add(d1 + 128, a1[2]); tile_atomic_add(d1 + 192, a1[3]);
  float* d2 = grow<float, A32>(p.GP, (unsigned)cur2, 4 * D, lane);
  tile_atomic_add(d2, a2[0]); tile_atomic_add(d2 + 64, a2[1]); tile_atomic_add(d2 + 128, a2[2]); tile_atomic_add(d2 + 192, a2[3]);
}

template <bool TRAIN, bool A32 = false>
__global__ __launch_bounds__(BLOCK) CHG_TWO_WAVES void k_atomconv_bwd(AtomConvArgs p) {
  constexpr bool FUSE_GQ = !TRAIN;
  constexpr int NW = WAVES;
  constexpr bool RM = FUSE_GQ;
  extern __shared__ __attribute__((aligned(16))) float smem[];
  constexpr int HMODE = RM ? 2 : 1;
  float* vecs = RM ? smem + 2 * AC_RM_IMG : smem + 4 * 4 * IMG64;
  const h16x8* IbT = reinterpret_cast<const h16x8*>(vecs + VEC_SLOTS * D);
  float* tiles = vecs + VEC_SLOTS * D + (FUSE_GQ ? 4 * IMG128 : 0);
  const float* W2c = smem;
  const float* W2g = RM ? smem + AC_RM_IMG : smem + 4 * IMG64;
  const float* W2cT = RM ? W2c : smem + 2 * 4 * IMG64;
  const float* W2gT = RM ? W2g : smem + 3 * 4 * IMG64;
  const int tid = threadIdx.x, lane = tid & 63, j = lane & 15, g = lane >> 4;
  const int wave = __builtin_amdgcn_readfirstlane(tid >> 6);
  float* T = tiles + wave * TILE_FLOATS;
  float* Trow = T + j * TS;
  const int ntiles = (p.n_edges + TILE_ROWS - 1) / TILE_ROWS;
  const TileSeq ts = wave_tile_seq<!TRAIN>(ntiles, NW, wave);
  const int last_row = p.n_edges - 1;
  int c, n, k;
  {
    const int row = max(0, min(ts.at(0) * TILE_ROWS + j, last_row));
    c = p.e_center[row]; n = p.e_nbr[row]; k = row >> 1;
    GatherRegs gr;
    gather_issue128<A32>(gr, p.P, c, p.P + 2 * D, n, p.Q, k, 4 * D, 4 * D, 2 * D, lane);
    if (TRAIN) atomconv_bwd_stage(smem, p, tid, 64 * NW);
    else stage_image<ac_bwd_rm_image_floats() / 4, 64 * NW>(smem, p.image, tid);
    gather_commit128(gr, T, TS, lane);
  }
  __syncthreads();
  TrainTile tt{};
  tt.T = T; tt.lane = lane;
  for (int v = 0; v < ts.count; ++v) {
    const int row0 = ts.at(v) * TILE_ROWS;
    const int nvalid = min(TILE_ROWS, p.n_edges - row0);
    if (TRAIN) {
      tt.nvalid = nvalid;
      tt.hrow = j < nvalid ? p.dumpH + (size_t)(row0 + j) * 2 * D : nullptr;
      tt.grow = j < nvalid ? p.dumpG + (size_t)(row0 + j) * 2 * D : nullptr;
    }
    int cn, nn, kn;
    {
      const int row = max(0, min(ts.at(v + 1) * TILE_ROWS + j, last_row));
      cn = p.e_center[row]; nn = p.e_nbr[row]; kn = row >> 1;
    }
    V64 wv, gm;
    read_dl_g<VT, A32>(p.wag, (unsigned)k, D, g, wv.t);
    read_dl_g<VT, A32>(p.GA, (unsigned)c, D, g, gm.t);
    const int k0 = row0 >> 1, nb = nvalid >> 1;
    float* gwag_rows = grow<float, A32>(p.Gwag, (unsigned)k0, D, lane);
    float prev[TILE_ROWS / 2];
#pragma unroll
    for (int b = 0; b < TILE_ROWS / 2; ++b) prev[b] = p.first_wag ? 0.f : gwag_rows[(size_t)min(b, nb - 1) * D];
    __builtin_amdgcn_wave_barrier();
    V64 zc, zg;
    read_dl<VT>(Trow, g, zc.t);
    read_dl<VT>(Trow + D, g, zg.t);
    GatedState s;
    V64 y;
    gated_forward<true, false, TRAIN, HMODE>(zc, zg, W2c, W2g, vecs, j, g, s, y, &tt);
    asm volatile("" : "+v"(cn), "+v"(nn));
    V64 gy, gw, gzc, gzg;
    CHG_EV(ft) {
      gw.t[ft] = gm.t[ft] * y.t[ft];
      gy.t[ft] = gm.t[ft] * wv.t[ft];
    }
    __builtin_amdgcn_wave_barrier();
    write_dl<VT>(Trow, g, gw.t);
    __builtin_amdgcn_wave_barrier();
    {
      float* dst = gwag_rows;
#pragma unroll
      for (int b = 0; b < TILE_ROWS / 2; ++b) prev[b] += T[(2 * b) * TS + lane] + T[(2 * b + 1) * TS + lane];
      if (nvalid == TILE_ROWS) {
#pragma unroll
        for (int b = 0; b < TILE_ROWS / 2; ++b) dst[(size_t)b * D] = prev[b];
      } else {
#pragma unroll
        for (int b = 0; b < TILE_ROWS / 2; ++b)
          if (b < nb) dst[(size_t)b * D] = prev[b];
      }
    }
    gated_backward<true, false, TRAIN, HMODE>(gy, zc, zg, W2cT, W2gT, vecs, j, g, s, gzc, gzg, &tt);
    if (FUSE_GQ) {
      float* gb_row = grow<float, A32>(p.Gb, (unsigned)(k0 + (j >> 1)), D, 4 * g);
      const bool owner = !(j & 1) && j < nvalid;
      V64 old = zero64();
      if (p.gb_accumulate && owner) {
        CHG_EV(ft) old.t[ft] = *reinterpret_cast<const f32x4*>(gb_row + 16 * ft);
      }
      f32x4 gz[2 * VT] = {gzc.t[0], gzc.t[1], gzc.t[2], gzc.t[3], gzg.t[0], gzg.t[1], gzg.t[2], gzg.t[3]};
      V64 gq = zero64();
      gemm_split<2 * VT, VT, true>(gq.t, IbT, D, gz, j, g);
      CHG_EW(ft, r) gq.t[ft][r] += __shfl_xor(gq.t[ft][r], 1);
      CHG_EV(ft) gq.t[ft] += old.t[ft];
      CHG_EV(ft) asm volatile("" : "+v"(gq.t[ft]));
      if (owner) {
        CHG_EV(ft) *reinterpret_cast<f32x4*>(gb_row + 16 * ft) = gq.t[ft];
      }
    }
    __builtin_amdgcn_wave_barrier();
    write_dl<VT>(Trow, g, gzc.t);
    write_dl<VT>(Trow + D, g, gzg.t);
    __builtin_amdgcn_wave_barrier();
    if (v + 1 < ts.count) {
      GatherRegs gr;
      gather_issue128<A32>(gr, p.P, cn, p.P + 2 * D, nn, p.Q, kn, 4 * D, 4 * D, 2 * D, lane);
      acbwd_scatter<!FUSE_GQ, A32>(T, c, nvalid, k0, p, lane);
      __builtin_amdgcn_wave_barrier();
      gather_commit128(gr, T, TS, lane);
    } else {
      acbwd_scatter<!FUSE_GQ, A32>(T, c, nvalid, k0, p, lane);
    }
    c = cn; n = nn; k = kn;
  }
  if (TRAIN) {
#pragma unroll
    for (int q = 0; q < 4; ++q) atomicAdd(p.g_ln + q * D + lane, tt.ln[q]);
  }
}

struct AngleArgs {
  const float* R;
  const float* S;
  const float* ang;
  const float* wbgc;
  const int *a_ctr, *a_b1c, *a_b2c;
  int n_angles;
  const float* w_ang;
  GatedW gw;
  const float* image;
  int slot;
  float* out;
  const float* Gagg;
  float* Gang;
  float* GR;
  float* GS;
  float* Gwbgc;
  int first_gang;
  const int* skip_flag;
  float* zsave;
  float* dumpG;
  float* dumpH;
  float* dumpZ;
  float* g_ln;
};

template <bool HIDDEN, int NW = WAVES, bool BWD = false>
constexpr size_t angle_lds() {
  if (angle_split(HIDDEN, BWD) == 2) return rm_image_bytes(2 * D, D) + 2 * rm_image_bytes(D, D) + sizeof(float) * (VEC_SLOTS * D + NW * TILE_FLOATS);
  return 16 * (size_t)((BWD ? 2 : 1) * IMG128 + (HIDDEN ? 2 * IMG64 : 0)) + sizeof(float) * (VEC_SLOTS * D + NW * TILE_FLOATS);
}


template <bool HIDDEN, bool BWD>
struct AngleLds {
  static constexpr int SPLIT = angle_split(HIDDEN, BWD);
  static constexpr int wangT = SPLIT == 2 ? 0 : 4 * IMG128;
  static constexpr int w2c = SPLIT == 2 ? (int)(rm_image_bytes(2 * D, D) / 4) : wangT + (BWD ? 4 * IMG128 : 0);
  static constexpr int w2 = HIDDEN ? (SPLIT == 2 ? (int)(rm_image_bytes(D, D) / 4) : 4 * IMG64) : 0;
  static constexpr int w2g = w2c + w2;
  static constexpr int vecs = w2g + w2;
  static constexpr int tiles = vecs + VEC_SLOTS * D;
};
template <bool HIDDEN, bool BWD>
__device__ __forceinline__ void angle_stage(float* base, const float* __restrict__ w_ang, const GatedW& gw, int tid, int nthreads) {
  using L = AngleLds<HIDDEN, BWD>;
  float* Wang = base;
  float* WangT = base + L::wangT;
  float* W2c = base + L::w2c;
  float* W2g = base + L::w2g;
  if (L::SPLIT == 2) {
    stage_rm(reinterpret_cast<_Float16*>(Wang), w_ang, 2 * D, D, tid, nthreads);
    stage_rm(reinterpret_cast<_Float16*>(W2c), gw.w2c, D, D, tid, nthreads);
    stage_rm(reinterpret_cast<_Float16*>(W2g), gw.w2g, D, D, tid, nthreads);
  } else {
    stage_split<false>(reinterpret_cast<h16x8*>(Wang), w_ang, 2 * D, D, tid, nthreads);
    if (BWD) stage_split<true>(reinterpret_cast<h16x8*>(WangT), w_ang, 2 * D, D, tid, nthreads);
    if (HIDDEN) {
      stage_split<false>(reinterpret_cast<h16x8*>(W2c), gw.w2c, D, D, tid, nthreads);
      stage_split<false>(reinterpret_cast<h16x8*>(W2g), gw.w2g, D, D, tid, nthreads);
    }
  }
  stage_gated_vecs(base + L::vecs, gw, HIDDEN, tid);
}
template <bool HIDDEN, bool BWD>
__global__ __launch_bounds__(BLOCK) void k_angle_image(const float* w_ang, GatedW gw, float* out) {
  angle_stage<HIDDEN, BWD>(out, w_ang, gw, threadIdx.x, BLOCK);
}

template <bool HIDDEN, bool BWD, int NW = WAVES, bool TRAIN = false, bool A32 = false>
__global__ __launch_bounds__(64 * NW) CHG_TWO_WAVES void k_angle(AngleArgs p) {
  static_assert(!TRAIN || BWD, "TRAIN is a variant of the adjoint kernels");
  if (!TRAIN && p.skip_flag && *p.skip_flag == 1) return;
  extern __shared__ __attribute__((aligned(16))) float smem[];
  constexpr int SPLIT = angle_split(HIDDEN, BWD);
  using L = AngleLds<HIDDEN, BWD>;
  float* Wang = smem;
  float* WangT = smem + L::wangT;
  float* W2c = smem + L::w2c;
  float* W2g = smem + L::w2g;
  float* vecs = smem + L::vecs;
  float* tiles = smem + L::tiles;
  const int tid = threadIdx.x, wave = tid >> 6, lane = tid & 63, j = lane & 15, g = lane >> 4;
  float* T = tiles + wave * TILE_FLOATS;
  float* Trow = T + j * TS;
  const int ntiles = (p.n_angles + TILE_ROWS - 1) / TILE_ROWS;
  const TileSeq ts = wave_tile_seq<!TRAIN>(ntiles, NW, wave);
  const int tstride = TILE_ROWS;
  auto row_of = [&](int v) { return max(0, min(ts.at(v) * tstride + j, p.n_angles - 1)); };
  constexpr bool PIPE = !BWD;
  int ctr_nx, b1_nx, b2_nx;
  int ctr_n2 = 0, b1_n2 = 0, b2_n2 = 0;
  GatherRegs gr_p;
  V64 x_p;
  {
    const int a0 = row_of(0);
    ctr_nx = p.a_ctr[a0]; b1_nx = p.a_b1c[a0]; b2_nx = p.a_b2c[a0];
    if (PIPE) {
      gather_issue128<A32>(gr_p, p.R, b1_nx, p.R + 2 * D, b2_nx, p.S, ctr_nx, 4 * D, 4 * D, 2 * D, lane);
      read_dl_g<VT, A32>(p.ang, (unsigned)a0, D, g, x_p.t);
      if (1 < ts.count) {
        const int a1 = row_of(1);
        ctr_n2 = p.a_ctr[a1]; b1_n2 = p.a_b1c[a1]; b2_n2 = p.a_b2c[a1];
      }
    }
  }
  if (TRAIN) angle_stage<HIDDEN, BWD>(smem, p.w_ang, p.gw, tid, 64 * NW);
  else stage_image<L::tiles / 4, 64 * NW>(smem, p.image, tid);
  __syncthreads();
  TrainTile tt{};
  tt.T = T; tt.lane = lane;
  for (int v = 0; v < ts.count; ++v) {
    int lane_t = lane;
    if (BWD && HIDDEN) asm volatile("" : "+v"(lane_t));
    const int row0 = ts.at(v) * tstride;
    const int nvalid = min(TILE_ROWS, p.n_angles - row0);
    const int ctr = ctr_nx, b1 = b1_nx, b2 = b2_nx;
    if (TRAIN) {
      tt.nvalid = nvalid;
      tt.hrow = (HIDDEN && j < nvalid) ? p.dumpH + (size_t)(row0 + j) * 2 * D : nullptr;
      tt.grow = j < nvalid ? p.dumpG + (size_t)(row0 + j) * 2 * D : nullptr;
    }
    if (!PIPE && v + 1 < ts.count) {
      const int a1 = row_of(v + 1);
      ctr_nx = p.a_ctr[a1]; b1_nx = p.a_b1c[a1]; b2_nx = p.a_b2c[a1];
    }
    if (nvalid <= 0) continue;
    const bool valid = j < nvalid;
    const int a = row0 + (valid ? j : 0);
    V64 x;
    f32x4 z[2 * VT];
    if (PIPE) {
      gather_commit128(gr_p, T, TS, lane_t);
      x = x_p;
      __builtin_amdgcn_wave_barrier();
      read_dl<2 * VT>(Trow, g, z);
      if (v + 1 < ts.count) {
        const int a1 = row_of(v + 1);
        gather_issue128<A32>(gr_p, p.R, b1_n2, p.R + 2 * D, b2_n2, p.S, ctr_n2, 4 * D, 4 * D, 2 * D, lane_t);
        int lane_here;
        asm volatile("v_mbcnt_lo_u32_b32 %0, -1, 0\n\tv_mbcnt_hi_u32_b32 %0, -1, %0" : "=v"(lane_here));
        read_dl_g<VT, A32>(p.ang, (unsigned)a1, D, lane_here >> 4, x_p.t);
        ctr_nx = ctr_n2; b1_nx = b1_n2; b2_nx = b2_n2;
        if (v + 2 < ts.count) {
          const int a2 = max(0, min(ts.at(v + 2) * tstride + (lane_here & 15), p.n_angles - 1));
          ctr_n2 = p.a_ctr[a2]; b1_n2 = p.a_b1c[a2]; b2_n2 = p.a_b2c[a2];
        }
      }
    } else {
      gather_rows64<A32>(T, TS, p.ang, a, lane_t);
      __builtin_amdgcn_wave_barrier();
      read_dl<VT>(Trow, g, x.t);
      __builtin_amdgcn_wave_barrier();
      gather_sum128<A32>(T, TS, p.R, b1, p.R + 2 * D, b2, p.S, ctr, 4 * D, 4 * D, 2 * D, lane_t);
      __builtin_amdgcn_wave_barrier();
      read_dl<2 * VT>(Trow, g, z);
    }
    Rows64 gy_rows;
    if (BWD && !HIDDEN) rows64_issue<A32>(gy_rows, p.Gang, a, lane_t);
    if (SPLIT == 2) gemm_rm<VT, 2 * VT, false, false>(z, reinterpret_cast<const _Float16*>(Wang), 2 * D, D, x.t, j, g, lane_t);
    else gemm_split<VT, 2 * VT, false, !BWD>(z, reinterpret_cast<const h16x8*>(Wang), 2 * D, x.t, j, g);
    if (BWD && !HIDDEN) {
      __builtin_amdgcn_sched_group_barrier(0x020, 4, 0);
      __builtin_amdgcn_sched_group_barrier(0x008, 128, 0);
    }
    if (!BWD && p.zsave) write_dl_g_nt<2 * VT, A32>(p.zsave, (unsigned)(valid ? a : p.n_angles + j), 2 * D, g, z);
    V64 zc{{z[0], z[1], z[2], z[3]}}, zg{{z[4], z[5], z[6], z[7]}};
    GatedState s;
    V64 y;
    constexpr bool SLIM = HIDDEN && BWD;
    gated_forward<HIDDEN, SLIM, TRAIN, SPLIT, !BWD>(zc, zg, W2c, W2g, vecs, j, g, s, y, &tt);
    __builtin_amdgcn_wave_barrier();
    V64 w1, w2;
    if (HIDDEN) {
      read_dl_g<VT, A32>(p.wbgc, (unsigned)b1, D, g, w1.t);
      read_dl_g<VT, A32>(p.wbgc, (unsigned)b2, D, g, w2.t);
    }
    if (!BWD) {
      CHG_EV(ft) {
        if (HIDDEN) y.t[ft] = y.t[ft] * (w1.t[ft] * w2.t[ft]);
        else y.t[ft] = y.t[ft] + x.t[ft];
      }
      write_dl<VT>(Trow, g, y.t);
      __builtin_amdgcn_wave_barrier();
      if (HIDDEN) seg_colsum_atomic<D, A32>(T, TS, valid ? b1 : -1, nvalid, p.out, D, lane_t);
      else scatter_rows64<false, A32>(T, TS, p.out, a, nvalid, lane_t);
    } else {
      V64 gy, gzc, gzg;
      if (HIDDEN) {
        V64 g1, g2, gu;
        read_dl_g<VT, A32>(p.Gagg, (unsigned)b1, D, g, gu.t);
        CHG_EV(ft) {
          const f32x4 gyu = gu.t[ft] * y.t[ft];
          g1.t[ft] = gyu * w2.t[ft];
          g2.t[ft] = gyu * w1.t[ft];
          gy.t[ft] = gu.t[ft] * w1.t[ft] * w2.t[ft];
        }
        write_dl<VT>(Trow, g, g1.t);
        write_dl<VT>(Trow + D, g, g2.t);
        __builtin_amdgcn_wave_barrier();
        seg_colsum_atomic<D, A32>(T, TS, valid ? b1 : -1, nvalid, p.Gwbgc, D, lane_t);
        row_atomic_add<D, A32>(T + D, TS, valid ? b2 : -1, nvalid, p.Gwbgc, D, lane_t);
      } else {
        rows64_commit(gy_rows, T, TS, lane_t);
        __builtin_amdgcn_wave_barrier();
        read_dl<VT>(Trow, g, gy.t);
      }
      __builtin_amdgcn_wave_barrier();
      gated_backward<HIDDEN, SLIM, TRAIN, SPLIT>(gy, zc, zg, W2c, W2g, vecs, j, g, s, gzc, gzg, &tt);
      f32x4 gz[2 * VT] = {gzc.t[0], gzc.t[1], gzc.t[2], gzc.t[3], gzg.t[0], gzg.t[1], gzg.t[2], gzg.t[3]};
      if (TRAIN && HIDDEN && valid) write_dl_g<2 * VT>(p.dumpZ, (unsigned)a, 2 * D, g, gz);
      V64 ga = zero64();
      if (HIDDEN) {
        Rows64 gang_old;
        if (p.first_gang) {
#pragma unroll
          for (int it = 0; it < TILE_ROWS / 4; ++it) gang_old.v[it] = zero4();
        } else {
          rows64_issue<A32>(gang_old, p.Gang, a, lane_t);
        }
        gemm_rm<2 * VT, VT, true, true>(ga.t, reinterpret_cast<const _Float16*>(Wang), 2 * D, D, gz, j, g, lane_t);
        write_dl<VT>(Trow, g, ga.t);
        __builtin_amdgcn_wave_barrier();
        scatter_rows64_add<false, A32>(T, TS, p.Gang, a, nvalid, lane_t, gang_old);
      } else {
        gemm_split<2 * VT, VT, true>(ga.t, reinterpret_cast<const h16x8*>(WangT), D, gz, j, g);
        write_dl<VT>(Trow, g, ga.t);
        __builtin_amdgcn_wave_barrier();
        scatter_rows64<true, A32>(T, TS, p.Gang, a, nvalid, lane_t);
      }
      __builtin_amdgcn_wave_barrier();
      write_dl<2 * VT>(Trow, g, gz);
      __builtin_amdgcn_wave_barrier();
      seg_colsum_atomic<2 * D, A32>(T, TS, valid ? b1 : -1, nvalid, p.GR, 4 * D, lane_t);
      row_atomic_add<2 * D, A32>(T, TS, valid ? b2 : -1, nvalid, p.GR + 2 * D, 4 * D, lane_t);
      seg_colsum_atomic<2 * D, A32>(T, TS, valid ? ctr : -1, nvalid, p.GS, 2 * D, lane_t);
    }
    __builtin_amdgcn_wave_barrier();
  }
  if (TRAIN) {
#pragma unroll
    for (int q = 0; q < 4; ++q) atomicAdd(p.g_ln + q * D + lane, tt.ln[q]);
  }
}

struct ReadoutArgs {
  const float* atom;
  const int* atom_owner;
  const int* z;
  int n_atoms;
  const float *ln_g, *ln_b, *w0, *b0, *w1, *b1, *w2, *b2, *w3, *b3, *atomref;
  int has_composition;
  int n_hidden;
  float* site_energy;
  float* site_raw;
  float* crystal_fea;
  float* Ga;
  int wpb;
  const float* cot;
  float* dump;
};

enum { RO_X0 = 0, RO_S1, RO_S2, RO_S3C, RO_G1, RO_G2, RO_G3, RO_GX, RO_GXX, RO_NDUMP };

constexpr size_t readout_lds() { return sizeof(float) * (3 * D * WS + 6 * D + WAVES * TILE_FLOATS); }

template <bool TRAIN>
__global__ __launch_bounds__(BLOCK) CHG_TWO_WAVES void k_readout(ReadoutArgs p) {
  extern __shared__ __attribute__((aligned(16))) float smem[];
  float* W0 = smem;
  float* W1 = W0 + D * WS;
  float* W2 = W1 + D * WS;
  float* vecs = W2 + D * WS;
  float* tiles = vecs + 6 * D;
  const int tid = threadIdx.x, wave = tid >> 6, lane = tid & 63, j = lane & 15, g = lane >> 4;
  stage_weights(W0, p.w0, D, D, tid);
  stage_weights(W1, p.w1, D, D, tid);
  stage_weights(W2, p.w2, D, D, tid);
  stage_vector(vecs + 0 * D, p.ln_g, D, tid);
  stage_vector(vecs + 1 * D, p.ln_b, D, tid);
  stage_vector(vecs + 2 * D, p.b0, D, tid);
  stage_vector(vecs + 3 * D, p.b1, D, tid);
  stage_vector(vecs + 4 * D, p.b2, D, tid);
  stage_vector(vecs + 5 * D, p.w3, D, tid);
  __syncthreads();
  float* T = tiles + wave * TILE_FLOATS;
  float* Trow = T + j * TS;
  const float b3 = p.b3[0];
  const int wpb = p.wpb > 0 ? p.wpb : WAVES, block_rows = wpb * TILE_ROWS;
  const int ntiles = (p.n_atoms + block_rows - 1) / block_rows;
  int tb, te;
  tile_range(ntiles, tb, te);
  if (wave >= wpb) return;
  for (int tile = tb; tile < te; ++tile) {
    const int row0 = tile * block_rows + wave * TILE_ROWS;
    const int nvalid = min(TILE_ROWS, p.n_atoms - row0);
    if (nvalid <= 0) continue;
    const bool valid = j < nvalid;
    const int i = row0 + (valid ? j : 0);
    const int owner = p.atom_owner[i];
    gather_rows64(T, TS, p.atom, i, lane);
    __builtin_amdgcn_wave_barrier();
    V64 xh, x0;
    read_dl<VT>(Trow, g, xh.t);
    const float rstd = ln_normalize(xh);
    const V64 gam = param64(vecs + 0 * D, g), bet = param64(vecs + 1 * D, g);
    CHG_EW(ft, r) x0.t[ft][r] = xh.t[ft][r] * gam.t[ft][r] + bet.t[ft][r];
    __builtin_amdgcn_wave_barrier();
    write_dl<VT>(Trow, g, x0.t);
    __builtin_amdgcn_wave_barrier();
    if (!TRAIN) seg_colsum_atomic<D>(T, TS, valid ? owner : -1, nvalid, p.crystal_fea, D, lane);
    V64 l1 = param64(vecs + 2 * D, g), l2 = param64(vecs + 3 * D, g), l3 = param64(vecs + 4 * D, g), sv;
    const size_t plane = (size_t)p.n_atoms * D;
    float* drow = TRAIN ? p.dump + (size_t)i * D : nullptr;
    const bool dump = TRAIN && valid;
    const float cot = TRAIN ? p.cot[owner] : 1.0f;
    if (dump) write_dl<VT>(drow + RO_X0 * plane, g, x0.t);
    gemm_dl<VT, VT>(l1.t, W0, WS, x0.t, j, g);
    CHG_EW(ft, r) sv.t[ft][r] = siluf_(l1.t[ft][r]);
    if (dump) write_dl<VT>(drow + RO_S1 * plane, g, sv.t);
    gemm_dl<VT, VT>(l2.t, W1, WS, sv.t, j, g);
    CHG_EW(ft, r) sv.t[ft][r] = siluf_(l2.t[ft][r]);
    if (dump) write_dl<VT>(drow + RO_S2 * plane, g, sv.t);
    const bool three = p.n_hidden != 2;
    if (three) gemm_dl<VT, VT>(l3.t, W2, WS, sv.t, j, g);
    else l3 = l2;
    const V64 w3 = param64(vecs + 5 * D, g);
    float site = 0.f;
    CHG_EW(ft, r) site += w3.t[ft][r] * siluf_(l3.t[ft][r]);
    site = quad_sum(site) + b3;
    if (!TRAIN && valid && g == 0) {
      const float ref = p.has_composition ? p.atomref[p.z[i] - 1] : 0.f;
      p.site_energy[i] = site + ref;
      p.site_raw[i] = site;
    }
    if (dump) {
      CHG_EW(ft, r) sv.t[ft][r] = cot * siluf_(l3.t[ft][r]);
      write_dl<VT>(drow + RO_S3C * plane, g, sv.t);
// ... 34 lines not shown
```

### chgnet_amd/csrc/mfma_tile.h

```cpp
#pragma once

#include <hip/hip_runtime.h>
#include <stdint.h>


namespace chg {

typedef float f32x4 __attribute__((ext_vector_type(4)));

constexpr int D = 64;
constexpr int TILE_ROWS = 16;
constexpr int WAVES = 8;
constexpr int BLOCK = 64 * WAVES;
constexpr int BLOCK_ROWS = TILE_ROWS * WAVES;
constexpr int PAD = 4;
constexpr int VT = 4;
constexpr float LN_EPS = 1e-5f;
constexpr int MFMA_R = 4;

struct V64 { f32x4 t[VT]; };

__device__ __forceinline__ int dfeat(int ft, int r, int g) { return 16 * ft + 4 * g + r; }

__device__ __forceinline__ f32x4 zero4() { return f32x4{0.f, 0.f, 0.f, 0.f}; }
__device__ __forceinline__ V64 zero64() { return V64{{zero4(), zero4(), zero4(), zero4()}}; }

__device__ __forceinline__ float sigmoidf_(float x) {
  return __builtin_amdgcn_rcpf(1.0f + __builtin_amdgcn_exp2f(-1.4426950408889634f * x));
}
__device__ __forceinline__ float siluf_(float x) { return x * sigmoidf_(x); }
__device__ __forceinline__ float dsiluf_(float x) {
  const float s = sigmoidf_(x);
  return s * (1.0f + x * (1.0f - s));
}

typedef float f32x2 __attribute__((ext_vector_type(2)));
__device__ __forceinline__ f32x2 sigmoid2(f32x2 x) {
  f32x2 t = x * -1.4426950408889634f;
  t[0] = __builtin_amdgcn_exp2f(t[0]); t[1] = __builtin_amdgcn_exp2f(t[1]);
  t = t + 1.0f;
  t[0] = __builtin_amdgcn_rcpf(t[0]); t[1] = __builtin_amdgcn_rcpf(t[1]);
  return t;
}
__device__ __forceinline__ f32x4 sigmoid4(f32x4 x) {
  const f32x2 lo = sigmoid2(f32x2{x[0], x[1]}), hi = sigmoid2(f32x2{x[2], x[3]});
  return f32x4{lo[0], lo[1], hi[0], hi[1]};
}
__device__ __forceinline__ float hsum4(f32x4 v) { return (v[0] + v[1]) + (v[2] + v[3]); }
#define CHG_EV(ft) _Pragma("unroll") for (int ft = 0; ft < VT; ++ft)

#define CHG_EW(ft, r) _Pragma("unroll") for (int ft = 0; ft < VT; ++ft) _Pragma("unroll") for (int r = 0; r < 4; ++r)

template <class T, bool A32 = false>
__device__ __forceinline__ const T* grow(const float* __restrict__ base, unsigned r, int ld, int c) {
  if constexpr (A32) return reinterpret_cast<const T*>(reinterpret_cast<const char*>(base) + (r * (unsigned)(4 * ld) + (unsigned)(4 * c)));
  else return reinterpret_cast<const T*>(base + (size_t)r * ld + c);
}
template <class T, bool A32 = false>
__device__ __forceinline__ T* grow(float* __restrict__ base, unsigned r, int ld, int c) {
  if constexpr (A32) return reinterpret_cast<T*>(reinterpret_cast<char*>(base) + (r * (unsigned)(4 * ld) + (unsigned)(4 * c)));
  else return reinterpret_cast<T*>(base + (size_t)r * ld + c);
}
template <int NT>
__device__ __forceinline__ void read_dl(const float* row, int g, f32x4 (&x)[NT]) {
#pragma unroll
  for (int ft = 0; ft < NT; ++ft) x[ft] = *reinterpret_cast<const f32x4*>(row + 16 * ft + 4 * g);
}
template <int NT>
__device__ __forceinline__ void write_dl(float* row, int g, const f32x4 (&x)[NT]) {
#pragma unroll
  for (int ft = 0; ft < NT; ++ft) *reinterpret_cast<f32x4*>(row + 16 * ft + 4 * g) = x[ft];
}

template <int NT, bool A32 = false>
__device__ __forceinline__ void read_dl_g(const float* __restrict__ base, unsigned r, int ld, int g, f32x4 (&x)[NT]) {
#pragma unroll
  for (int ft = 0; ft < NT; ++ft) x[ft] = *grow<f32x4, A32>(base, r, ld, 16 * ft + 4 * g);
}
template <int NT, bool A32 = false>
__device__ __forceinline__ void write_dl_g(float* __restrict__ base, unsigned r, int ld, int g, const f32x4 (&x)[NT]) {
#pragma unroll
  for (int ft = 0; ft < NT; ++ft) *grow<f32x4, A32>(base, r, ld, 16 * ft + 4 * g) = x[ft];
}

template <int NT, bool A32 = false>
__device__ __forceinline__ void read_dl_g_nt(const float* __restrict__ base, unsigned r, int ld, int g, f32x4 (&x)[NT]) {
#pragma unroll
  for (int ft = 0; ft < NT; ++ft) x[ft] = __builtin_nontemporal_load(grow<f32x4, A32>(base, r, ld, 16 * ft + 4 * g));
}
template <int NT, bool A32 = false>
__device__ __forceinline__ void write_dl_g_nt(float* __restrict__ base, unsigned r, int ld, int g, const f32x4 (&x)[NT]) {
#pragma unroll
  for (int ft = 0; ft < NT; ++ft) __builtin_nontemporal_store(x[ft], grow<f32x4, A32>(base, r, ld, 16 * ft + 4 * g));
}

template <int KT, int NFT>
__device__ __forceinline__ void gemm_dl(f32x4 (&acc)[NFT], const float* W, int ws, const f32x4 (&x)[KT], int i, int g) {
  const float* wbase = W + i * ws + 4 * g;
#pragma unroll
  for (int kt = 0; kt < KT; ++kt) {
    f32x4 w[NFT];
#pragma unroll
    for (int fo = 0; fo < NFT; ++fo) w[fo] = *reinterpret_cast<const f32x4*>(wbase + 16 * fo * ws + 16 * kt);
#pragma unroll
    for (int r = 0; r < MFMA_R; ++r)
#pragma unroll
      for (int fo = 0; fo < NFT; ++fo) acc[fo] = __builtin_amdgcn_mfma_f32_16x16x4f32(w[fo][r], x[kt][r], acc[fo], 0, 0, 0);
  }
}

template <int NFT>
__device__ __forceinline__ void gemm_t_load(float (&a)[4][NFT], const float* W, int ws, int kt, int i, int g) {
#pragma unroll
  for (int r = 0; r < 4; ++r) {
    const float* wrow = W + dfeat(kt, r, g) * ws + i;
#pragma unroll
    for (int fo = 0; fo < NFT; ++fo) a[r][fo] = wrow[16 * fo];
  }
}
template <int NFT>
__device__ __forceinline__ void gemm_t_touch(float (&a)[4][NFT]) {
#pragma unroll
  for (int r = 0; r < 4; ++r)
#pragma unroll
    for (int fo = 0; fo < NFT; ++fo) asm volatile("" : "+v"(a[r][fo]));
}
template <int KT, int NFT>
__device__ __forceinline__ void gemm_dl_t(f32x4 (&acc)[NFT], const float* W, int ws, const f32x4 (&x)[KT], int i, int g) {
  float a[2][4][NFT];
  gemm_t_load<NFT>(a[0], W, ws, 0, i, g);
#pragma unroll
  for (int kt = 0; kt < KT; ++kt) {
    if (kt + 1 < KT) gemm_t_load<NFT>(a[(kt + 1) & 1], W, ws, kt + 1, i, g);
    gemm_t_touch<NFT>(a[kt & 1]);
#pragma unroll
    for (int r = 0; r < MFMA_R; ++r)
#pragma unroll
      for (int fo = 0; fo < NFT; ++fo) acc[fo] = __builtin_amdgcn_mfma_f32_16x16x4f32(a[kt & 1][r][fo], x[kt][r], acc[fo], 0, 0, 0);
  }
}

__device__ __forceinline__ float quad_sum(float v) {
  const unsigned u = __float_as_uint(v);
  const auto r = __builtin_amdgcn_permlane16_swap(u, u, false, false);
  const float s = __uint_as_float(r[0]) + __uint_as_float(r[1]);
  const unsigned w = __float_as_uint(s);
  const auto q = __builtin_amdgcn_permlane32_swap(w, w, false, false);
  return __uint_as_float(q[0]) + __uint_as_float(q[1]);
}

__device__ __forceinline__ float ln_normalize(V64& c) {
  f32x4 s4 = (c.t[0] + c.t[1]) + (c.t[2] + c.t[3]);
  const float mu = quad_sum(hsum4(s4)) * (1.0f / 64.0f);
  f32x4 v4 = zero4();
  CHG_EV(ft) {
    c.t[ft] = c.t[ft] - mu;
    v4 += c.t[ft] * c.t[ft];
  }
  const float rstd = __builtin_amdgcn_rsqf(quad_sum(hsum4(v4)) * (1.0f / 64.0f) + LN_EPS);
  CHG_EV(ft) c.t[ft] = c.t[ft] * rstd;
  return rstd;
}

__device__ __forceinline__ void ln_backward(V64& gy, const V64& gamma, const V64& xhat, float rstd) {
  f32x4 s1 = zero4(), s2 = zero4();
  CHG_EV(ft) {
    gy.t[ft] = gy.t[ft] * gamma.t[ft];
    s1 += gy.t[ft];
    s2 += gy.t[ft] * xhat.t[ft];
  }
  const float m1 = quad_sum(hsum4(s1)) * (1.0f / 64.0f);
  const float m2 = quad_sum(hsum4(s2)) * (1.0f / 64.0f);
  CHG_EV(ft) gy.t[ft] = (gy.t[ft] - m1 - xhat.t[ft] * m2) * rstd;
}

__device__ __forceinline__ void stage_weights(float* dst, const float* __restrict__ src, int rows, int K, int tid) {
  const int ws = K + PAD;
  const int k4 = K / 4;
  for (int idx = tid; idx < rows * k4; idx += (int)blockDim.x) {
    const int rr = idx / k4, c4 = idx - rr * k4;
    *reinterpret_cast<f32x4*>(dst + rr * ws + 4 * c4) = *reinterpret_cast<const f32x4*>(src + rr * K + 4 * c4);
  }
}
__device__ __forceinline__ void stage_vector(float* dst, const float* __restrict__ src, int n, int tid) {
  for (int idx = tid; idx < n; idx += (int)blockDim.x) dst[idx] = src[idx];
}

template <int N16, int NT, int CHUNK = 16>
__device__ __forceinline__ void stage_image(float* dst, const float* __restrict__ src, int tid) {
  constexpr int IT = (N16 + NT - 1) / NT;
#pragma unroll
  for (int u0 = 0; u0 < IT; u0 += CHUNK) {
    f32x4 v[CHUNK];
#pragma unroll
    for (int u = 0; u < CHUNK; ++u) {
      const int idx = tid + (u0 + u) * NT;
      if (u0 + u < IT && idx < N16) v[u] = reinterpret_cast<const f32x4*>(src)[idx];
    }
#pragma unroll
    for (int u = 0; u < CHUNK; ++u) {
      const int idx = tid + (u0 + u) * NT;
      if (u0 + u < IT && idx < N16) reinterpret_cast<f32x4*>(dst)[idx] = v[u];
    }
  }
}

__device__ __forceinline__ void wave_tile_range(int n_wave_tiles, int waves_per_block, int wave, int& begin, int& end) {
  const int G = gridDim.x, b = blockIdx.x;
  int lb = b;
  if ((G & 7) == 0) lb = (b & 7) * (G >> 3) + (b >> 3);
  const long W = (long)G * waves_per_block, lw = (long)lb * waves_per_block + wave;
  begin = (int)(lw * n_wave_tiles / W);
  end = (int)((lw + 1) * n_wave_tiles / W);
}

constexpr int INTERLEAVE_MIN_TILES = 6;
struct TileSeq {
  int first, stride, count;
  __device__ __forceinline__ int at(int v) const { return first + v * stride; }
};
template <bool INTERLEAVE>
__device__ __forceinline__ TileSeq wave_tile_seq(int n_wave_tiles, int waves_per_block, int wave) {
  const int G = gridDim.x, b = blockIdx.x;
  TileSeq s;
  if (INTERLEAVE && (G & 7) == 0 && (long)n_wave_tiles >= (long)INTERLEAVE_MIN_TILES * G * waves_per_block) {
    const int x = b & 7, WX = (G >> 3) * waves_per_block, lw = (b >> 3) * waves_per_block + wave;
    const int xb = (int)((long)n_wave_tiles * x / 8), xe = (int)((long)n_wave_tiles * (x + 1) / 8);
    s.first = xb + lw;
    s.stride = WX;
    s.count = xe - xb > lw ? (xe - xb - lw + WX - 1) / WX : 0;
    return s;
  }
  int tb, te;
  wave_tile_range(n_wave_tiles, waves_per_block, wave, tb, te);
  s.first = tb; s.stride = 1; s.count = te - tb;
  return s;
}

__device__ __forceinline__ int xcc_id() { return (int)(__builtin_amdgcn_s_getreg(20 | (3 << 11)) & 7u); }

__device__ __forceinline__ void tile_range_of(int ntiles, int G, int b, int& begin, int& end) {
  int lb = b;
  if ((G & 7) == 0) lb = (b & 7) * (G >> 3) + (b >> 3);
  const int per = ntiles / G, rem = ntiles - per * G;
  begin = lb * per + (lb < rem ? lb : rem);
  end = begin + per + (lb < rem ? 1 : 0);
}
__device__ __forceinline__ void tile_range(int ntiles, int& begin, int& end) { tile_range_of(ntiles, gridDim.x, blockIdx.x, begin, end); }

#define CHG_TWO_WAVES __attribute__((amdgpu_waves_per_eu(2, 2)))

__device__ __forceinline__ void tile_atomic_add(float* p, float v) {
  atomicAdd(p, v);
}

template <int W, bool A32 = false>
__device__ __forceinline__ void seg_colsum_atomic(const float* tile, int stride, int key, int nvalid, float* __restrict__ dst,
                                                  int ldd, int lane) {
  constexpr int NC = W / 64;
  float acc[NC];
#pragma unroll
  for (int c = 0; c < NC; ++c) acc[c] = 0.f;
  int cur = __builtin_amdgcn_readlane(key, 0);
#pragma unroll
  for (int rr = 0; rr < TILE_ROWS; ++rr) {
    const int kk = __builtin_amdgcn_readlane(key, rr);
    if (kk != cur) {
      if (cur >= 0) {
#pragma unroll
        for (int c = 0; c < NC; ++c) tile_atomic_add(grow<float, A32>(dst, (unsigned)cur, ldd, 64 * c + lane), acc[c]);
      }
#pragma unroll
      for (int c = 0; c < NC; ++c) acc[c] = 0.f;
      cur = kk;
    }
#pragma unroll
    for (int c = 0; c < NC; ++c) acc[c] += tile[rr * stride + 64 * c + lane];
  }
  if (cur >= 0) {
#pragma unroll
    for (int c = 0; c < NC; ++c) tile_atomic_add(grow<float, A32>(dst, (unsigned)cur, ldd, 64 * c + lane), acc[c]);
  }
}

template <int W, bool A32 = false>
__device__ __forceinline__ void row_atomic_add(const float* tile, int stride, int key, int nvalid, float* __restrict__ dst,
                                               int ldd, int lane) {
#pragma unroll
  for (int rr = 0; rr < TILE_ROWS; ++rr) {
    const int kk = __builtin_amdgcn_readlane(key, rr);
    if (kk >= 0) {
#pragma unroll
      for (int c = 0; c < W / 64; ++c) tile_atomic_add(grow<float, A32>(dst, (unsigned)kk, ldd, 64 * c + lane), tile[rr * stride + 64 * c + lane]);
    }
  }
}

template <bool A32 = false>
__device__ __forceinline__ void gather_sum128(float* tile, int stride, const float* __restrict__ t0, int i0,
                                              const float* __restrict__ t1, int i1, const float* __restrict__ t2, int i2,
                                              int ld0, int ld1, int ld2, int lane) {
  const int hw = lane >> 5, t = lane & 31;
  int r0[TILE_ROWS / 2], r1[TILE_ROWS / 2], r2[TILE_ROWS / 2];
#pragma unroll
  for (int it = 0; it < TILE_ROWS / 2; ++it) {
    const int rr = 2 * it + hw;
    r0[it] = __shfl(i0, rr); r1[it] = __shfl(i1, rr); r2[it] = __shfl(i2, rr);
  }
  f32x4 a[TILE_ROWS / 2], b[TILE_ROWS / 2], c[TILE_ROWS / 2];
#pragma unroll
  for (int it = 0; it < TILE_ROWS / 2; ++it) {
    a[it] = *grow<f32x4, A32>(t0, (unsigned)r0[it], ld0, 4 * t);
    b[it] = *grow<f32x4, A32>(t1, (unsigned)r1[it], ld1, 4 * t);
    c[it] = *grow<f32x4, A32>(t2, (unsigned)r2[it], ld2, 4 * t);
  }
#pragma unroll
  for (int it = 0; it < TILE_ROWS / 2; ++it) {
    const int rr = 2 * it + hw;
    *reinterpret_cast<f32x4*>(tile + rr * stride + 4 * t) = (a[it] + b[it]) + c[it];
  }
}

struct GatherRegs { f32x4 a[TILE_ROWS / 2], b[TILE_ROWS / 2], c[TILE_ROWS / 2]; };
__device__ __forceinline__ void gather_take(GatherRegs& gr);

template <bool A32 = false>
__device__ __forceinline__ void gather_issue128(GatherRegs& gr, const float* __restrict__ t0, int i0, const float* __restrict__ t1,
                                                int i1, const float* __restrict__ t2, int i2, int ld0, int ld1, int ld2, int lane) {
  const int hw = lane >> 5, t = lane & 31;
  int r0[TILE_ROWS / 2], r1[TILE_ROWS / 2], r2[TILE_ROWS / 2];
#pragma unroll
  for (int it = 0; it < TILE_ROWS / 2; ++it) {
    const int rr = 2 * it + hw;
    r0[it] = __shfl(i0, rr); r1[it] = __shfl(i1, rr); r2[it] = __shfl(i2, rr);
  }
#pragma unroll
  for (int it = 0; it < TILE_ROWS / 2; ++it) {
    gr.a[it] = *grow<f32x4, A32>(t0, (unsigned)r0[it], ld0, 4 * t);
    gr.b[it] = *grow<f32x4, A32>(t1, (unsigned)r1[it], ld1, 4 * t);
    gr.c[it] = *grow<f32x4, A32>(t2, (unsigned)r2[it], ld2, 4 * t);
  }
}
__device__ __forceinline__ void gather_commit128(const GatherRegs& gr, float* tile, int stride, int lane) {
  const int hw = lane >> 5, t = lane & 31;
#pragma unroll
  for (int it = 0; it < TILE_ROWS / 2; ++it)
    *reinterpret_cast<f32x4*>(tile + (2 * it + hw) * stride + 4 * t) = (gr.a[it] + gr.b[it]) + gr.c[it];
}

struct GatherPH { f32x4 a[TILE_ROWS / 2], b[TILE_ROWS / 2], h[TILE_ROWS / 4]; };
__device__ __forceinline__ void gather_take(GatherPH& gr) {
#pragma unroll
  for (int it = 0; it < TILE_ROWS / 2; ++it) asm volatile("" : "+v"(gr.a[it]), "+v"(gr.b[it]));
#pragma unroll
  for (int it = 0; it < TILE_ROWS / 4; ++it) asm volatile("" : "+v"(gr.h[it]));
}
__device__ __forceinline__ void gather_take(GatherRegs& gr) {
#pragma unroll
  for (int it = 0; it < TILE_ROWS / 2; ++it) asm volatile("" : "+v"(gr.a[it]), "+v"(gr.b[it]), "+v"(gr.c[it]));
}
template <bool A32 = false>
__device__ __forceinline__ void gather_issue_ph(GatherPH& gr, const float* __restrict__ t0, int i0, const float* __restrict__ t1, int i1, int ld0,
                                                int ld1, const float* __restrict__ hbase, long hoff, int lane) {
  const int hw = lane >> 5, t = lane & 31, sub = lane >> 4, t16 = lane & 15;
  int r0[TILE_ROWS / 2], r1[TILE_ROWS / 2];
  long ho[TILE_ROWS / 4];
#pragma unroll
  for (int it = 0; it < TILE_ROWS / 2; ++it) {
    const int rr = 2 * it + hw;
    r0[it] = __shfl(i0, rr); r1[it] = __shfl(i1, rr);
  }
  const int hlo = (int)(hoff & 0xffffffffL), hhi = (int)(hoff >> 32);
#pragma unroll
  for (int it = 0; it < TILE_ROWS / 4; ++it) {
    const int rr = 4 * it + sub;
    if constexpr (A32) ho[it] = (long)(unsigned)__shfl(hlo, rr);
    else ho[it] = ((long)__shfl(hhi, rr) << 32) | (unsigned)__shfl(hlo, rr);
  }
#pragma unroll
  for (int it = 0; it < TILE_ROWS / 2; ++it) {
    gr.a[it] = *grow<f32x4, A32>(t0, (unsigned)r0[it], ld0, 4 * t);
    gr.b[it] = *grow<f32x4, A32>(t1, (unsigned)r1[it], ld1, 4 * t);
  }
#pragma unroll
  for (int it = 0; it < TILE_ROWS / 4; ++it) {
    if constexpr (A32) gr.h[it] = *reinterpret_cast<const f32x4*>(reinterpret_cast<const char*>(hbase) + (4u * (unsigned)ho[it] + 16u * (unsigned)t16));
    else gr.h[it] = *reinterpret_cast<const f32x4*>(hbase + ho[it] + 4 * t16);
  }
}
__device__ __forceinline__ void gather_commit_p(const GatherPH& gr, float* tile, int stride, int lane) {
  const int hw = lane >> 5, t = lane & 31;
#pragma unroll
  for (int it = 0; it < TILE_ROWS / 2; ++it) *reinterpret_cast<f32x4*>(tile + (2 * it + hw) * stride + 4 * t) = gr.a[it] + gr.b[it];
}
__device__ __forceinline__ void gather_commit_h(const GatherPH& gr, float* tile, int stride, int lane) {
  const int sub = lane >> 4, t = lane & 15;
#pragma unroll
  for (int it = 0; it < TILE_ROWS / 4; ++it) *reinterpret_cast<f32x4*>(tile + (4 * it + sub) * stride + 4 * t) = gr.h[it];
}

struct Rows64 { f32x4 v[TILE_ROWS / 4]; };
template <bool A32 = false>
__device__ __forceinline__ void rows64_issue(Rows64& rr, const float* __restrict__ src, int idx, int lane) {
  const int sub = lane >> 4, t = lane & 15;
  int r[TILE_ROWS / 4];
#pragma unroll
  for (int it = 0; it < TILE_ROWS / 4; ++it) r[it] = __shfl(idx, 4 * it + sub);
#pragma unroll
  for (int it = 0; it < TILE_ROWS / 4; ++it) rr.v[it] = *grow<f32x4, A32>(src, (unsigned)r[it], D, 4 * t);
}
__device__ __forceinline__ void rows64_commit(const Rows64& rr, float* tile, int stride, int lane) {
  const int sub = lane >> 4, t = lane & 15;
#pragma unroll
  for (int it = 0; it < TILE_ROWS / 4; ++it) *reinterpret_cast<f32x4*>(tile + (4 * it + sub) * stride + 4 * t) = rr.v[it];
}
template <bool OPAQUE = false, bool A32 = false>
__device__ __forceinline__ void scatter_rows64_add(const float* tile, int stride, float* __restrict__ dst, int idx, int nvalid, int lane,
                                                   const Rows64& old) {
  const int sub = lane >> 4, t = lane & 15;
  f32x4 v[TILE_ROWS / 4];
  int r[TILE_ROWS / 4];
#pragma unroll
  for (int it = 0; it < TILE_ROWS / 4; ++it) {
    const int rr = 4 * it + sub;
    r[it] = __shfl(idx, rr);
    v[it] = old.v[it] + *reinterpret_cast<const f32x4*>(tile + rr * stride + 4 * t);
  }
#pragma unroll
  for (int it = 0; it < TILE_ROWS / 4; ++it) asm volatile("" : "+v"(v[it]));
#pragma unroll
  for (int it = 0; it < TILE_ROWS / 4; ++it) {
    int lim = nvalid - 4 * it;
    if (OPAQUE) asm volatile("" : "+v"(lim));
    if (sub < lim) *grow<f32x4, A32>(dst, (unsigned)r[it], D, 4 * t) = v[it];
  }
}

template <bool A32 = false>
// ... 36 lines not shown
```

Baseline: 40900 structures/s.

## Pack edge and angle index arrays into int4 records and use ballot-based segment sums

Adds one-time kernels that pack per-edge (center, neighbor, bond node) and per-angle (center, bond1, bond2) indices into int4 records, so the atom-conv and angle kernels fetch one vector load per row instead of several scalar gathers. The windowed angle kernel now reads packed per-atom headers and row records, and derives the first-bond slot arithmetically from the row position. The segmented column-sum atomics now find segment boundaries with a DPP shift plus ballot instead of a serial readlane compare chain. This costs extra device memory for the record arrays and a one-time build pass per batch, and the float-based slot division could misround for some group sizes.

```diff
diff --git a/chgnet_amd/csrc/engine_internal.h b/chgnet_amd/csrc/engine_internal.h
--- a/chgnet_amd/csrc/engine_internal.h
+++ b/chgnet_amd/csrc/engine_internal.h
@@ -130,6 +130,8 @@
   float* zsave_l[2 * MAX_CONV] = {};
   float *energy, *site_energy, *site_raw, *magmom, *crystal_fea, *force, *virial, *volume;
   float *Ga, *GA, *Gb, *Gwag, *Gwbgc, *Gang, *GQ, *Gagg, *Grk, *Gu;
+  int4 *pair_rec = nullptr, *ang_rec = nullptr;
+  bool index_records_ready = false;
   WinIndex win{};
   int *win_tmp = nullptr, *win_scan = nullptr;
   int win_grid = 64;
@@ -283,6 +285,7 @@
   return (A > 0 && N + 1 <= 8192 && (long)A <= blk_max_angles()) ? (int)blk_tile_bound(A, Eb, N) : 0;
 }
 bool decide_windows(chg_engine* eng, chg_batch* b);
+int ensure_index_records(chg_engine* eng, chg_batch* b);
 int ensure_windows(chg_engine* eng, chg_batch* b);
 void register_names(chg_batch* b);
 
diff --git a/chgnet_amd/csrc/engine_predict.hip b/chgnet_amd/csrc/engine_predict.hip
--- a/chgnet_amd/csrc/engine_predict.hip
+++ b/chgnet_amd/csrc/engine_predict.hip
@@ -285,6 +285,7 @@
   a.hb0 = b->hb0;
   a.hbc = (b->Eb > 0 && b->hbc[l] != b->hbc[0]) ? b->hbc[l] : nullptr;
   a.u_bnode = b->u_bnode;
+  a.rec = b->pair_rec;
   a.w_bond = eng->w.ac[l].w_bond;
   a.q_bias = b->A > 0 ? eng->w.ac[l].q_bias : nullptr;
   return a;
@@ -292,6 +293,7 @@
 
 int atomconv_fwd_kernel(chg_engine* eng, chg_batch* b, int l, bool keep_q) {
   {
+    TRY(ensure_index_records(eng, b));
     LaunchScope ls(eng, "atomconv_fwd");
     const size_t lds = atomconv_lds<FWD_WAVES, false, true>();
     AtomConvArgs a = atomconv_args(eng, b, l);
@@ -325,6 +327,7 @@
     a.image = eng->img_ac_bwd_rm[l];
     a.Gb = b->Gb;
     a.gb_accumulate = l == b->L - 1 ? 0 : 1;
+    TRY(ensure_index_records(eng, b));
     LaunchScope ls(eng, "atomconv_bwd");
     if (addr32_mode(b)) hipLaunchKernelGGL((k_atomconv_bwd<false, true>), dim3(tile_grid(eng, b->Ed)), dim3(BLOCK), acb_fused_lds(), eng->stream, a);
     else hipLaunchKernelGGL(k_atomconv_bwd<false>, dim3(tile_grid(eng, b->Ed)), dim3(BLOCK), acb_fused_lds(), eng->stream, a);
@@ -362,7 +365,7 @@
 AngleArgs angle_args(chg_batch* b, int slot, const float* ang, const float* w_ang, const GatedW& g, float* out) {
   AngleArgs a{};
   a.R = b->Rl[slot]; a.S = b->Sl[slot]; a.ang = ang; a.wbgc = b->wbgc;
-  a.a_ctr = b->a_ctr; a.a_b1c = b->a_b1c; a.a_b2c = b->a_b2c; a.n_angles = b->A;
+  a.a_ctr = b->a_ctr; a.a_b1c = b->a_b1c; a.a_b2c = b->a_b2c; a.rec = b->ang_rec; a.n_angles = b->A;
   a.w_ang = w_ang; a.gw = g; a.out = out; a.slot = slot;
   a.Gagg = b->Gagg; a.Gang = b->Gang; a.GR = b->GR_l[slot]; a.GS = b->GS_l[slot]; a.Gwbgc = b->Gwbgc;
   a.first_gang = slot == b->L - 2;
@@ -378,6 +381,7 @@
 
 template <bool HIDDEN, bool BWD, int NW = WAVES>
 int launch_angle(chg_engine* eng, const char* label, chg_batch* b, const AngleArgs& a) {
+  if (HIDDEN && !BWD) TRY(ensure_index_records(eng, b));
   LaunchScope ls(eng, label);
   AngleArgs plain = a;
   const bool index_from_builder = b->canonical && (b->win_index_ready || b->blk_ready);
@@ -811,6 +815,7 @@
     w.rows = c.take<int4>(A); w.atoms = c.take<int4>(A ? N : 0);
     w.wave_head = c.take<int>(A ? WIN_MAX_GRID * WAVES : 0); w.next_atom = c.take<int>(A ? N : 0); w.xatom = c.take<int>(WIN_MAX_GRID / 8 + 1);
     b->win_tmp = c.take<int>(N + 1);
+    b->pair_rec = c.take<int4>(Ed); b->ang_rec = c.take<int4>(A);
     b->win_scan = c.take<int>(scan_scratch_ints((int)N + 1));
   }
   {
@@ -824,7 +829,8 @@
     auto tab = [](size_t rows, size_t ld) { return rows * ld * sizeof(float); };
     size_t span = std::max({tab(N, 4 * D) , tab(Eu, 2 * D) , tab(Eb, 4 * D) , tab(A, D) ,
                             b->zsave_l[0] ? tab(A + TILE_ROWS, 2 * D) : 0 ,
-                            A * sizeof(int4) });
+                            A * sizeof(int4) ,
+                            Ed * sizeof(int4) });
     for (int l = 0; l < L; ++l) {
       if (!b->hbc[l]) continue;
       span = b->hbc[l] < b->hb0 ? ~size_t(0) : std::max(span, (size_t)(b->hbc[l] - b->hb0) * sizeof(float) + tab(Eb, D));
@@ -832,6 +838,15 @@
     b->addr_span = span;
   }
   total = (c.pos + 255) & ~size_t(255);
+}
+
+int ensure_index_records(chg_engine* eng, chg_batch* b) {
+  if (b->index_records_ready) return CHG_OK;
+  b->index_records_ready = true;
+  if (b->Ed > 0) hipLaunchKernelGGL(k_pair_records, g1(b->Ed), dim3(256), 0, eng->stream, b->p_center, b->p_nbr, b->u_bnode, b->Ed, b->pair_rec);
+  if (b->A > 0) hipLaunchKernelGGL(k_angle_records, g1(b->A), dim3(256), 0, eng->stream, b->a_ctr, b->a_b1c, b->a_b2c, b->A, b->ang_rec);
+  HIP_TRY(eng, hipGetLastError());
+  return CHG_OK;
 }
 
 int ensure_windows(chg_engine* eng, chg_batch* b) {
@@ -864,6 +879,7 @@
 int prepare_windows(chg_engine* eng, chg_batch* b) {
   hipStream_t st = eng->stream;
   WinIndex& w = b->win;
+  TRY(ensure_index_records(eng, b));
   if (b->blk_cap > 0) {
     b->win_built = false; b->win_team = 0;
     if (b->blk_ready) return CHG_OK;
@@ -942,6 +958,8 @@
   mi["win_flag"] = {b->win.flag, 4}; mi["win_q_a"] = {b->win.q_a, A}; mi["win_q_ctr"] = {b->win.q_ctr, A}; mi["win_na"] = {b->win.na, N + 1};
   mi["win_aoff"] = {b->win.aoff, N + 1}; mi["win_q_ab1"] = {b->win.q_ab1, A}; mi["win_q_ab2"] = {b->win.q_ab2, A};
   mi["win_next_atom"] = {b->win.next_atom, A ? N : 0};
+  mi["win_rows"] = {reinterpret_cast<const int*>(b->win.rows), 4 * A}; mi["win_atoms"] = {reinterpret_cast<const int*>(b->win.atoms), A ? 4 * N : 0};
+  mi["pair_rec"] = {reinterpret_cast<const int*>(b->pair_rec), 4 * Ed}; mi["ang_rec"] = {reinterpret_cast<const int*>(b->ang_rec), 4 * A};
   mi["blk_tiles"] = {b->blk_tiles, b->blk_cap ? (size_t)1 : 0}; mi["blk_a"] = {b->blk_a, (size_t)b->blk_cap * TILE_ROWS};
   mi["blk_b1c"] = {b->blk_b1c, (size_t)b->blk_cap * TILE_ROWS}; mi["blk_b2c"] = {b->blk_b2c, (size_t)b->blk_cap * TILE_ROWS};
   mi["blk_ctr"] = {b->blk_ctr, (size_t)b->blk_cap * TILE_ROWS}; mi["blk_desc"] = {b->blk_desc, (size_t)b->blk_cap};
diff --git a/chgnet_amd/csrc/kernels_angle_fa.h b/chgnet_amd/csrc/kernels_angle_fa.h
--- a/chgnet_amd/csrc/kernels_angle_fa.h
+++ b/chgnet_amd/csrc/kernels_angle_fa.h
@@ -36,63 +36,56 @@
   const int wave = __builtin_amdgcn_readfirstlane(tid >> 6);
   float* tab = smem + L::tiles + wave * (FA_NSL * FA_RS);
 
-  int c_cur = w.wave_head[blockIdx.x * WAVES + wave];
-  int n_raw = 0, ab_raw = 0, r_raw = 0, c_nx = -1;
-  if (c_cur >= 0) { n_raw = w.na[c_cur]; ab_raw = w.boff[c_cur]; r_raw = w.aoff[c_cur]; c_nx = w.next_atom[c_cur]; }
+  const int c_first = __builtin_amdgcn_readfirstlane(w.wave_head[blockIdx.x * WAVES + wave]);
+  int4 h_cur = index_load_uniform(w.atoms, max(c_first, 0));
   stage_image<L::tiles / 4, BLOCK>(smem, p.image, tid);
   __syncthreads();
-  if (c_cur < 0) return;
-  int n_nraw = 0, ab_nraw = 0, r_nraw = 0, c_n2 = -1;
-  if (c_nx >= 0) { n_nraw = w.na[c_nx]; ab_nraw = w.boff[c_nx]; r_nraw = w.aoff[c_nx]; c_n2 = w.next_atom[c_nx]; }
+  if (c_first < 0) return;
+  int c_cur = c_first;
+  int4 h_nx = index_load_uniform(w.atoms, max(h_cur.w, 0));
   FaRows rows;
-  int aA, q1A, q2A;
+  int4 recA;
   V64 xn;
   {
-    const int c = __builtin_amdgcn_readfirstlane(c_cur), n = __builtin_amdgcn_readfirstlane(n_raw);
-    const int ab0 = __builtin_amdgcn_readfirstlane(ab_raw), r0 = __builtin_amdgcn_readfirstlane(r_raw);
-    const int bkv = w.abbond[ab0 + min(lane, n - 1)];
-    const int ra = min(r0 + j, r0 + n * (n - 1) - 1);
-    aA = w.q_a[ra]; q1A = w.q_ab1[ra]; q2A = w.q_ab2[ra];
-    fa_request<A32>(rows, p, c, min(n, FA_NSL), bkv, lane);
-    read_dl_g<VT, A32>(p.ang, (unsigned)aA, D, g, xn.t);
+    const int n = h_cur.x, r0 = h_cur.y, ab0 = h_cur.z;
+    const int bkv = index_load<int, A32>(w.abbond, ab0 + min(lane, n - 1));
+    recA = index_load<int4, A32>(w.rows, min(r0 + j, r0 + n * (n - 1) - 1));
+    fa_request<A32>(rows, p, c_cur, min(n, FA_NSL), bkv, lane);
+    read_dl_g<VT, A32>(p.ang, (unsigned)recA.x, D, g, xn.t);
   }
   V64 y_prev;
   CHG_EV(ft) y_prev.t[ft] = zero4();
   int a_prev = 0, nvalid_prev = 0;
 
-  for (int c = __builtin_amdgcn_readfirstlane(c_cur); c >= 0; c = __builtin_amdgcn_readfirstlane(c_cur)) {
-    const int n = __builtin_amdgcn_readfirstlane(n_raw), ab0 = __builtin_amdgcn_readfirstlane(ab_raw);
-    const int r_begin = __builtin_amdgcn_readfirstlane(r_raw), r_end = r_begin + n * (n - 1);
+  for (int c = c_cur; c >= 0; c = c_cur) {
+    const int n = h_cur.x, r_begin = h_cur.y, r_end = r_begin + n * (n - 1);
+    const float inv_group = 1.f / (float)(n - 1);
     __builtin_amdgcn_wave_barrier();
     fa_commit(rows, tab, min(n, FA_NSL), lane);
     __builtin_amdgcn_wave_barrier();
-    const int c_next = __builtin_amdgcn_readfirstlane(c_nx);
-    int bkv_n = 0, aA_n = 0, q1A_n = 0, q2A_n = -1;
-    int n1 = 0, ab1 = 0, rb1 = 0;
-    int n_n2raw = 0, ab_n2raw = 0, r_n2raw = 0, c_n3 = -1;
+    const int c_next = h_cur.w;
+    int bkv_n = 0, n1 = 0;
+    int4 recA_n = make_int4(0, 0, 0, -1);
+    int4 h_n2 = h_nx;
     if (c_next >= 0) {
-      n1 = __builtin_amdgcn_readfirstlane(n_nraw); ab1 = __builtin_amdgcn_readfirstlane(ab_nraw); rb1 = __builtin_amdgcn_readfirstlane(r_nraw);
-      bkv_n = w.abbond[ab1 + min(lane, n1 - 1)];
-      const int ra = min(rb1 + j, rb1 + n1 * (n1 - 1) - 1);
-      aA_n = w.q_a[ra]; q1A_n = w.q_ab1[ra]; q2A_n = w.q_ab2[ra];
-      if (c_n2 >= 0) { n_n2raw = w.na[c_n2]; ab_n2raw = w.boff[c_n2]; r_n2raw = w.aoff[c_n2]; c_n3 = w.next_atom[c_n2]; }
+      n1 = h_nx.x;
+      bkv_n = index_load<int, A32>(w.abbond, h_nx.z + min(lane, n1 - 1));
+      recA_n = index_load<int4, A32>(w.rows, min(h_nx.y + j, h_nx.y + n1 * (n1 - 1) - 1));
+      h_n2 = index_load_uniform(w.atoms, max(h_nx.w, 0));
     }
-    int a_t = aA, q1_t = q1A, q2_t = q2A;
-    int a_n, q1_n, q2_n;
-    {
-      const int rr = min(r_begin + TILE_ROWS + j, r_end - 1);
-      a_n = w.q_a[rr]; q1_n = w.q_ab1[rr]; q2_n = w.q_ab2[rr];
-    }
+    int4 rec_t = recA;
+    int4 rec_n = index_load<int4, A32>(w.rows, min(r_begin + TILE_ROWS + j, r_end - 1));
     for (int row0 = r_begin; row0 < r_end; row0 += TILE_ROWS) {
       const int nvalid = min(TILE_ROWS, r_end - row0);
       asm volatile("" ::: "memory");
       const V64 x = xn;
-      const int a = a_t, r1 = q1_t - ab0, r2 = q2_t < 0 ? -1 : q2_t - ab0;
+      const int a = rec_t.x, r2 = rec_t.w;
+      const int rel = min(row0 - r_begin + j, r_end - r_begin - 1);
+      const int r1 = (int)(((float)rel + 0.5f) * inv_group);
       const bool last = row0 + TILE_ROWS >= r_end;
-      const int a_ld = last ? (c_next >= 0 ? aA_n : a) : a_n;
+      const int a_ld = last ? (c_next >= 0 ? recA_n.x : a) : rec_n.x;
       read_dl_g<VT, A32>(p.ang, (unsigned)a_ld, D, g, xn.t);
-      const int rr2 = min(row0 + 2 * TILE_ROWS + j, r_end - 1);
-      const int a_n2 = w.q_a[rr2], q1_n2 = w.q_ab1[rr2], q2_n2 = w.q_ab2[rr2];
+      const int4 rec_n2 = index_load<int4, A32>(w.rows, min(row0 + 2 * TILE_ROWS + j, r_end - 1));
       f32x4 z[2 * VT];
 #pragma unroll
       for (int fo = 0; fo < 2 * VT; ++fo) z[fo] = zero4();
@@ -100,7 +93,7 @@
       asm volatile("" ::: "memory");
       if (j < nvalid_prev) write_dl_g<VT, A32>(p.out, (unsigned)a_prev, D, g, y_prev.t);
       asm volatile("" ::: "memory");
-      const bool in_lds = r1 < FA_NSL && r2 >= 0 && r2 < FA_NSL;
+      const bool in_lds = r1 < FA_NSL && (unsigned)r2 < (unsigned)FA_NSL;
       if (__builtin_amdgcn_ballot_w64(!in_lds) == 0) {
         const float* t1 = tab + r1 * FA_RS + 4 * g;
         const float* t2 = tab + r2 * FA_RS + 2 * D + 4 * g;
@@ -108,9 +101,8 @@
         for (int fo = 0; fo < 2 * VT; ++fo)
           z[fo] += *reinterpret_cast<const f32x4*>(t1 + 16 * fo) + *reinterpret_cast<const f32x4*>(t2 + 16 * fo);
       } else {
-        const int row = min(row0 + j, r_end - 1);
-        const float* g1 = grow<float, A32>(p.R, (unsigned)w.q_b1c[row], 4 * D, 4 * g);
-        const float* g2 = grow<float, A32>(p.R, (unsigned)w.q_b2c[row], 4 * D, 2 * D + 4 * g);
+        const float* g1 = grow<float, A32>(p.R, (unsigned)rec_t.y, 4 * D, 4 * g);
+        const float* g2 = grow<float, A32>(p.R, (unsigned)rec_t.z, 4 * D, 2 * D + 4 * g);
         const float* gs = grow<float, A32>(p.S, (unsigned)c, 2 * D, 4 * g);
 #pragma unroll
         for (int fo = 0; fo < 2 * VT; ++fo)
@@ -124,11 +116,10 @@
       gated_forward<false, false, false, 1>(zc, zg, nullptr, nullptr, vecs, j, g, st, y);
       CHG_EV(ft) y_prev.t[ft] = y.t[ft] + x.t[ft];
       a_prev = a; nvalid_prev = nvalid;
-      a_t = a_n; q1_t = q1_n; q2_t = q2_n; a_n = a_n2; q1_n = q1_n2; q2_n = q2_n2;
+      rec_t = rec_n; rec_n = rec_n2;
     }
-    c_cur = c_next; n_raw = n_nraw; ab_raw = ab_nraw; r_raw = r_nraw;
-    c_nx = c_n2; n_nraw = n_n2raw; ab_nraw = ab_n2raw; r_nraw = r_n2raw; c_n2 = c_n3;
-    aA = aA_n; q1A = q1A_n; q2A = q2A_n;
+    c_cur = c_next; h_cur = h_nx; h_nx = h_n2;
+    recA = recA_n;
   }
   if (j < nvalid_prev) write_dl_g<VT, A32>(p.out, (unsigned)a_prev, D, g, y_prev.t);
 }
diff --git a/chgnet_amd/csrc/kernels_angle_w.h b/chgnet_amd/csrc/kernels_angle_w.h
--- a/chgnet_amd/csrc/kernels_angle_w.h
+++ b/chgnet_amd/csrc/kernels_angle_w.h
@@ -222,11 +222,6 @@
   return k;
 }
 
-template <class T, bool A32 = false>
-__device__ __forceinline__ T index_load(const T* __restrict__ base, int i) {
-  if constexpr (A32) return *reinterpret_cast<const T*>(reinterpret_cast<const char*>(base) + (unsigned)i * (unsigned)sizeof(T));
-  else return base[i];
-}
 __device__ __forceinline__ int4 index_load_uniform(const int4* base, int i) {
 #if defined(__HIP_DEVICE_COMPILE__)
   typedef const int __attribute__((address_space(4))) * ConstInt;
diff --git a/chgnet_amd/csrc/kernels_conv.h b/chgnet_amd/csrc/kernels_conv.h
--- a/chgnet_amd/csrc/kernels_conv.h
+++ b/chgnet_amd/csrc/kernels_conv.h
@@ -401,6 +401,7 @@
   GatedW gw;
   const float *hb0, *hbc;
   const int* u_bnode;
+  const int4* rec;
   const float *w_bond, *q_bias;
   float* Qout;
   const float* image;
@@ -462,6 +463,11 @@
 static __global__ __launch_bounds__(BLOCK) void k_atomconv_image_rm(AtomConvArgs p, float* out) { atomconv_bwd_stage_rm(out, p, threadIdx.x, BLOCK); }
 
 __device__ __forceinline__ int bond_node(const AtomConvArgs& p, int k) { return p.hbc ? p.u_bnode[k] : -1; }
+static __global__ void k_pair_records(const int* __restrict__ p_center, const int* __restrict__ p_nbr, const int* __restrict__ u_bnode, int n_edges,
+                                      int4* __restrict__ rec) {
+  const int r = blockIdx.x * blockDim.x + threadIdx.x;
+  if (r < n_edges) rec[r] = make_int4(p_center[r], p_nbr[r], u_bnode[r >> 1], 0);
+}
 template <bool A32 = false>
 __device__ __forceinline__ long bond_row_offset(const AtomConvArgs& p, int k, int bn) {
   if constexpr (A32) return (long)(bn >= 0 ? (unsigned)(p.hbc - p.hb0) + (unsigned)bn * D : (unsigned)k * D);
@@ -489,15 +495,16 @@
   V64 wv_nx;
   int c_nx = 0, n_nx = 0, c_n2 = 0, n_n2 = 0;
   int bn_nx = -1, bn_n2 = -1;
+  const bool nodes = p.hbc != nullptr;
   if (ts.count > 0) {
     const int r0 = row_of(0);
-    c_nx = p.e_center[r0]; n_nx = p.e_nbr[r0];
-    bn_nx = bond_node(p, r0 >> 1);
-    gather_issue_ph<A32>(gr, p.P, c_nx, p.P + 2 * D, n_nx, 4 * D, 4 * D, p.hb0, bond_row_offset<A32>(p, r0 >> 1, bn_nx), lane);
+    const int4 q0 = index_load<int4, A32>(p.rec, r0);
+    c_nx = q0.x; n_nx = q0.y; bn_nx = q0.z;
+    gather_issue_ph<A32>(gr, p.P, c_nx, p.P + 2 * D, n_nx, 4 * D, 4 * D, p.hb0, bond_row_offset<A32>(p, r0 >> 1, nodes ? bn_nx : -1), lane);
     read_dl_g<VT, A32>(p.wag, (unsigned)(r0 >> 1), D, g, wv_nx.t);
     const int r1 = row_of(1);
-    c_n2 = p.e_center[r1]; n_n2 = p.e_nbr[r1];
-    bn_n2 = bond_node(p, r1 >> 1);
+    const int4 q1 = index_load<int4, A32>(p.rec, r1);
+    c_n2 = q1.x; n_n2 = q1.y; bn_n2 = q1.z;
   }
   stage_image<ac_fwd_image_floats() / 4, 64 * NW>(smem, p.image, tid);
   __syncthreads();
@@ -505,7 +512,7 @@
     const int row0 = ts.at(v) * tstride;
     const int nvalid = min(TILE_ROWS, p.n_edges - row0);
     const int c = c_nx;
-    const bool node = bn_nx >= 0;
+    const bool node = nodes && bn_nx >= 0;
     const V64 wv = wv_nx;
     gather_commit_h(gr, T, TS, lane);
     __builtin_amdgcn_wave_barrier();
@@ -517,11 +524,12 @@
     c_nx = c_n2; n_nx = n_n2; bn_nx = bn_n2;
     if (v + 1 < ts.count) {
       const int r1 = row_of(v + 1);
-      gather_issue_ph<A32>(gr, p.P, c_nx, p.P + 2 * D, n_nx, 4 * D, 4 * D, p.hb0, bond_row_offset<A32>(p, r1 >> 1, bn_nx), lane);
+      gather_issue_ph<A32>(gr, p.P, c_nx, p.P + 2 * D, n_nx, 4 * D, 4 * D, p.hb0, bond_row_offset<A32>(p, r1 >> 1, nodes ? bn_nx : -1), lane);
       read_dl_g<VT, A32>(p.wag, (unsigned)(r1 >> 1), D, g, wv_nx.t);
-      const int r2 = row_of(v + 2);
-      c_n2 = p.e_center[r2]; n_n2 = p.e_nbr[r2];
-      bn_n2 = bond_node(p, r2 >> 1);
+    }
+    {
+      const int4 q2 = index_load<int4, A32>(p.rec, row_of(v + 2));
+      c_n2 = q2.x; n_n2 = q2.y; bn_n2 = q2.z;
     }
     f32x4 z[2 * VT];
     if (!node) {
@@ -553,26 +561,25 @@
     write_dl<VT>(Trow, g, m.t);
     __builtin_amdgcn_wave_barrier();
     {
+      const int c_back = __builtin_amdgcn_update_dpp(c, c, 0x112 , 0xF, 0xF, false);
+      const unsigned starts = (unsigned)__builtin_amdgcn_ballot_w64(c != c_back && j < nvalid);
       float acc1 = 0.f, acc2 = 0.f;
-      int cur1 = __builtin_amdgcn_readlane(c, 0), cur2 = __builtin_amdgcn_readlane(c, 1);
 #pragma unroll
       for (int b = 0; b < TILE_ROWS / 2; ++b) {
         if (2 * b < nvalid) {
-          const int c1 = __builtin_amdgcn_readlane(c, 2 * b), c2 = __builtin_amdgcn_readlane(c, 2 * b + 1);
-          if (c1 != cur1) {
-            tile_atomic_add(grow<float, A32>(p.agg, (unsigned)cur1, D, lane), acc1);
+          if (b > 0 && (starts & (1u << (2 * b)))) {
+            tile_atomic_add(grow<float, A32>(p.agg, (unsigned)__builtin_amdgcn_readlane(c, max(2 * b - 2, 0)), D, lane), acc1);
             acc1 = 0.f;
-            cur1 = c1;
           }
-          if (c2 != cur2) {
-            tile_atomic_add(grow<float, A32>(p.agg, (unsigned)cur2, D, lane), acc2);
+          if (b > 0 && (starts & (1u << (2 * b + 1)))) {
+            tile_atomic_add(grow<float, A32>(p.agg, (unsigned)__builtin_amdgcn_readlane(c, max(2 * b - 1, 1)), D, lane), acc2);
             acc2 = 0.f;
-            cur2 = c2;
           }
           acc1 += T[(2 * b) * TS + lane];
           acc2 += T[(2 * b + 1) * TS + lane];
         }
       }
+      const int cur1 = __builtin_amdgcn_readlane(c, nvalid - 2), cur2 = __builtin_amdgcn_readlane(c, nvalid - 1);
       tile_atomic_add(grow<float, A32>(p.agg, (unsigned)cur1, D, lane), acc1);
       tile_atomic_add(grow<float, A32>(p.agg, (unsigned)cur2, D, lane), acc2);
     }
@@ -639,9 +646,17 @@
   const TileSeq ts = wave_tile_seq<!TRAIN>(ntiles, NW, wave);
   const int last_row = p.n_edges - 1;
   int c, n, k;
+  auto row_index = [&](int row, int& ctr, int& nbr) {
+    if constexpr (!TRAIN) {
+      const int4 q = index_load<int4, A32>(p.rec, row);
+      ctr = q.x; nbr = q.y;
+    } else {
+      ctr = p.e_center[row]; nbr = p.e_nbr[row];
+    }
+  };
   {
     const int row = max(0, min(ts.at(0) * TILE_ROWS + j, last_row));
-    c = p.e_center[row]; n = p.e_nbr[row]; k = row >> 1;
+    row_index(row, c, n); k = row >> 1;
     GatherRegs gr;
     gather_issue128<A32>(gr, p.P, c, p.P + 2 * D, n, p.Q, k, 4 * D, 4 * D, 2 * D, lane);
     if (TRAIN) atomconv_bwd_stage(smem, p, tid, 64 * NW);
@@ -662,7 +677,7 @@
     int cn, nn, kn;
     {
       const int row = max(0, min(ts.at(v + 1) * TILE_ROWS + j, last_row));
-      cn = p.e_center[row]; nn = p.e_nbr[row]; kn = row >> 1;
+      row_index(row, cn, nn); kn = row >> 1;
     }
     V64 wv, gm;
     read_dl_g<VT, A32>(p.wag, (unsigned)k, D, g, wv.t);
@@ -746,6 +761,7 @@
   const float* ang;
   const float* wbgc;
   const int *a_ctr, *a_b1c, *a_b2c;
+  const int4* rec;
   int n_angles;
   const float* w_ang;
   GatedW gw;
@@ -804,6 +820,11 @@
   }
   stage_gated_vecs(base + L::vecs, gw, HIDDEN, tid);
 }
+static __global__ void k_angle_records(const int* __restrict__ a_ctr, const int* __restrict__ a_b1c, const int* __restrict__ a_b2c, int n_angles,
+                                       int4* __restrict__ rec) {
+  const int a = blockIdx.x * blockDim.x + threadIdx.x;
+  if (a < n_angles) rec[a] = make_int4(a_ctr[a], a_b1c[a], a_b2c[a], 0);
+}
 template <bool HIDDEN, bool BWD>
 __global__ __launch_bounds__(BLOCK) void k_angle_image(const float* w_ang, GatedW gw, float* out) {
   angle_stage<HIDDEN, BWD>(out, w_ang, gw, threadIdx.x, BLOCK);
@@ -830,19 +851,28 @@
   const int tstride = TILE_ROWS;
   auto row_of = [&](int v) { return max(0, min(ts.at(v) * tstride + j, p.n_angles - 1)); };
   constexpr bool PIPE = !BWD;
+  constexpr bool REC = HIDDEN && !BWD && A32;
+  auto row_index = [&](int a, int& ctr, int& b1, int& b2) {
+    if constexpr (REC) {
+      const int4 q = index_load<int4, A32>(p.rec, a);
+      ctr = q.x; b1 = q.y; b2 = q.z;
+    } else {
+      ctr = p.a_ctr[a]; b1 = p.a_b1c[a]; b2 = p.a_b2c[a];
+    }
+  };
   int ctr_nx, b1_nx, b2_nx;
   int ctr_n2 = 0, b1_n2 = 0, b2_n2 = 0;
   GatherRegs gr_p;
   V64 x_p;
   {
     const int a0 = row_of(0);
-    ctr_nx = p.a_ctr[a0]; b1_nx = p.a_b1c[a0]; b2_nx = p.a_b2c[a0];
+    row_index(a0, ctr_nx, b1_nx, b2_nx);
     if (PIPE) {
       gather_issue128<A32>(gr_p, p.R, b1_nx, p.R + 2 * D, b2_nx, p.S, ctr_nx, 4 * D, 4 * D, 2 * D, lane);
       read_dl_g<VT, A32>(p.ang, (unsigned)a0, D, g, x_p.t);
-      if (1 < ts.count) {
+      if (REC || 1 < ts.count) {
         const int a1 = row_of(1);
-        ctr_n2 = p.a_ctr[a1]; b1_n2 = p.a_b1c[a1]; b2_n2 = p.a_b2c[a1];
+        row_index(a1, ctr_n2, b1_n2, b2_n2);
       }
     }
   }
@@ -864,7 +894,7 @@
     }
     if (!PIPE && v + 1 < ts.count) {
       const int a1 = row_of(v + 1);
-      ctr_nx = p.a_ctr[a1]; b1_nx = p.a_b1c[a1]; b2_nx = p.a_b2c[a1];
+      row_index(a1, ctr_nx, b1_nx, b2_nx);
     }
     if (nvalid <= 0) continue;
     const bool valid = j < nvalid;
@@ -883,10 +913,16 @@
         asm volatile("v_mbcnt_lo_u32_b32 %0, -1, 0\n\tv_mbcnt_hi_u32_b32 %0, -1, %0" : "=v"(lane_here));
         read_dl_g<VT, A32>(p.ang, (unsigned)a1, D, lane_here >> 4, x_p.t);
         ctr_nx = ctr_n2; b1_nx = b1_n2; b2_nx = b2_n2;
-        if (v + 2 < ts.count) {
+        if (!REC && v + 2 < ts.count) {
           const int a2 = max(0, min(ts.at(v + 2) * tstride + (lane_here & 15), p.n_angles - 1));
-          ctr_n2 = p.a_ctr[a2]; b1_n2 = p.a_b1c[a2]; b2_n2 = p.a_b2c[a2];
+          row_index(a2, ctr_n2, b1_n2, b2_n2);
         }
+      }
+      if (REC) {
+        int lane_here;
+        asm volatile("v_mbcnt_lo_u32_b32 %0, -1, 0\n\tv_mbcnt_hi_u32_b32 %0, -1, %0" : "=v"(lane_here));
+        const int a2 = max(0, min(ts.at(v + 2) * tstride + (lane_here & 15), p.n_angles - 1));
+        row_index(a2, ctr_n2, b1_n2, b2_n2);
       }
     } else {
       gather_rows64<A32>(T, TS, p.ang, a, lane_t);
@@ -924,7 +960,7 @@
       }
       write_dl<VT>(Trow, g, y.t);
       __builtin_amdgcn_wave_barrier();
-      if (HIDDEN) seg_colsum_atomic<D, A32>(T, TS, valid ? b1 : -1, nvalid, p.out, D, lane_t);
+      if (HIDDEN) seg_colsum_atomic_ballot<D, A32>(T, TS, valid ? b1 : -1, nvalid, p.out, D, lane_t);
       else scatter_rows64<false, A32>(T, TS, p.out, a, nvalid, lane_t);
     } else {
       V64 gy, gzc, gzg;
diff --git a/chgnet_amd/csrc/mfma_tile.h b/chgnet_amd/csrc/mfma_tile.h
--- a/chgnet_amd/csrc/mfma_tile.h
+++ b/chgnet_amd/csrc/mfma_tile.h
@@ -60,6 +60,11 @@
 __device__ __forceinline__ T* grow(float* __restrict__ base, unsigned r, int ld, int c) {
   if constexpr (A32) return reinterpret_cast<T*>(reinterpret_cast<char*>(base) + (r * (unsigned)(4 * ld) + (unsigned)(4 * c)));
   else return reinterpret_cast<T*>(base + (size_t)r * ld + c);
+}
+template <class T, bool A32 = false>
+__device__ __forceinline__ T index_load(const T* __restrict__ base, int i) {
+  if constexpr (A32) return *reinterpret_cast<const T*>(reinterpret_cast<const char*>(base) + (unsigned)i * (unsigned)sizeof(T));
+  else return base[i];
 }
 template <int NT>
 __device__ __forceinline__ void read_dl(const float* row, int g, f32x4 (&x)[NT]) {
@@ -284,6 +289,39 @@
 }
 
 template <int W, bool A32 = false>
+__device__ __forceinline__ void seg_colsum_atomic_ballot(const float* tile, int stride, int key, int nvalid, float* __restrict__ dst,
+                                                         int ldd, int lane) {
+  constexpr int NC = W / 64;
+  const int prev = __builtin_amdgcn_update_dpp(key, key, 0x111 , 0xF, 0xF, false);
+  const unsigned starts = (unsigned)__builtin_amdgcn_ballot_w64(key != prev);
+  float acc[NC];
+#pragma unroll
+  for (int c = 0; c < NC; ++c) acc[c] = 0.f;
+#pragma unroll
+  for (int rr = 0; rr < TILE_ROWS; ++rr) {
+    if (rr > 0 && (starts & (1u << rr))) {
+      const int cur = __builtin_amdgcn_readlane(key, rr > 0 ? rr - 1 : 0);
+      if (cur >= 0) {
+#pragma unroll
+        for (int c = 0; c < NC; ++c) tile_atomic_add(grow<float, A32>(dst, (unsigned)cur, ldd, 64 * c + lane), acc[c]);
+      }
+#pragma unroll
+      for (int c = 0; c < NC; ++c) acc[c] = 0.f;
+    }
+#pragma unroll
+    for (int c = 0; c < NC; ++c) {
+      asm volatile("" : "+v"(acc[c]));
+      acc[c] += tile[rr * stride + 64 * c + lane];
+    }
+  }
+  const int cur = __builtin_amdgcn_readlane(key, TILE_ROWS - 1);
+  if (cur >= 0) {
+#pragma unroll
+    for (int c = 0; c < NC; ++c) tile_atomic_add(grow<float, A32>(dst, (unsigned)cur, ldd, 64 * c + lane), acc[c]);
+  }
+}
+
+template <int W, bool A32 = false>
 __device__ __forceinline__ void row_atomic_add(const float* tile, int stride, int key, int nvalid, float* __restrict__ dst,
                                                int ldd, int lane) {
 #pragma unroll
```

Measured after the change: 40960 structures/s (median of 6 runs). No clear change (+0.1%).
